# zyang1580/SML

Hardware: AMD Instinct MI355X
Metric: SML retrain-period training triples/s (MF + transfer stages), Yelp-shaped synthetic, d=32 (higher is better)
Workload: dtype f32; 1 GPU; yelp_period: users=60000 items=123000 interactions/period=75000 neg=999 d=32 multi_num=10 MF_batch=1024 TR_batch=256 val_eval=True (the reference's 40 validation evaluations per period: 31 computed on the GPU, 9 memoised because the tables did not change in between -- identical numbers); MF stage: the transfer net runs once per DISTINCT row of a batch (the reference gathers one row per occurrence:; parallelism=single GPU

## Files before the change

### include/sml_hip.h

```cpp
#ifndef SML_HIP_H
#define SML_HIP_H

#include <stdint.h>

#ifdef __cplusplus
extern "C" {
#endif

#define SML_OK 0
#define SML_EINVAL (-1)
#define SML_EHIP (-2)
#define SML_ENOMEM (-3)
#define SML_ESTATE (-4)

#define SML_LOSS_BCE 0
#define SML_LOSS_BPR 1
#define SML_LOSS_BPR_NORM 2
#define SML_LOSS_BPR_UNIT 3

typedef struct sml_ctx sml_ctx;

const char* sml_last_error(void);
int sml_version(void);

int sml_ctx_create(sml_ctx** out, int device, int d, int max_batch);
int sml_ctx_destroy(sml_ctx* ctx);
int sml_ctx_set_variant(sml_ctx* ctx, int variant);
int sml_ctx_set_grad_clip(sml_ctx* ctx, float max_norm);
int sml_ctx_set_adaptive(sml_ctx* ctx, float beta);

int64_t sml_theta_net_size(int d);
int64_t sml_theta_offset(int d, int which);
int sml_theta_pack(sml_ctx* ctx, const float* theta, void* stream);

int sml_comm_load(const char* librccl_path);
int sml_comm_unique_id(void* out128);
int sml_comm_init(sml_ctx* ctx, int world, int rank, const void* id128);
int sml_comm_destroy(sml_ctx* ctx);
int sml_comm_allreduce(sml_ctx* ctx, float* buf, int64_t n, void* stream);
int sml_comm_allgather(sml_ctx* ctx, const float* src, float* dst, int64_t n_per_rank, void* stream);

#define SML_MAX_PEERS 8
int sml_peer_region_bytes(sml_ctx* ctx, int world, int64_t rows_cap, int64_t* inbox_bytes, int64_t* flags_bytes);
int sml_peer_alloc(int device, int64_t bytes, void** ptr);
int sml_peer_free(int device, void* ptr);
int sml_peer_mem_kind(void* ptr);
int sml_peer_read(int device, const void* src, void* dst, int64_t bytes, void* stream);
int sml_peer_export(void* ptr, void* handle64);
int sml_peer_open(int device, const void* handle64, void** ptr);
int sml_peer_close(int device, void* ptr);
int sml_peer_attach(sml_ctx* ctx, int world, int rank, void* const* inbox, void* const* flags, int64_t rows_cap,
                    double timeout_s);
int sml_peer_detach(sml_ctx* ctx);
int sml_peer_status(sml_ctx* ctx, int* timeouts);
int sml_peer_allreduce_check(sml_ctx* ctx, const float* src, float* dst, int64_t n, double timeout_s, void* stream);

int sml_transfer_forward(sml_ctx* ctx, const float* theta, int net, const float* x_t,
                         const float* x_hat, float* out, int64_t n_rows, void* stream);

typedef struct {
    float* w_user;
    float* w_item;
    const float* last_user;
    const float* last_item;
    float* m_user; float* v_user;
    float* m_item; float* v_item;
    int32_t* step_user;
    int32_t* step_item;
    int64_t n_user, n_item;
} sml_mf_tables;

typedef int (*sml_mf_hook)(void* user, int64_t batch_index);
typedef struct {
    int world;
    const uint64_t* key_items;
    const uint32_t* val_items;
    float* dx_local;
    float* dx_items_all;
    sml_mf_hook hook;
    void* hook_user;
    float loss_scale;
    int64_t slot_stride;
    const int64_t* item_off;
    int64_t push_rows;
    int lists_unsorted;
} sml_mf_exchange;
// ... 33 lines not shown
    const int64_t* items_all;
    float* dx_local;
    float* dx_items_all;
    sml_mf_hook hook;
    void* hook_user;
    float loss_scale;
} sml_bare_exchange;

int sml_embed_loss_sgd_prepare(sml_ctx* ctx, const int64_t* triples, int64_t n, int batch,
                               int64_t n_user, int64_t n_item, int slot, const sml_bare_exchange* xchg, void* stream);
int64_t sml_index_lists_read(sml_ctx* ctx, int slot, int which, void* host, int64_t bytes);
int sml_embed_loss_sgd_epoch(sml_ctx* ctx, void* w_user, void* w_item, int64_t n_user,
                             int64_t n_item, int dtype_bytes, const int64_t* triples, int64_t n,
                             int batch, float lr, float lam_user, float lam_item, int loss_kind,
                             float* batch_loss, int prepared_slot, const sml_bare_exchange* xchg, void* stream);

typedef struct {
    int world, rank;
    int64_t head_rows, shard_rows;
    void* const* item_shard;
    void* w_item_head;
    const int64_t* items_all;
    float loss_scale;
} sml_bare_shard;
int sml_embed_loss_sgd_epoch_sharded(sml_ctx* ctx, void* w_user, int64_t n_user, int64_t n_item, int dtype_bytes,
                                     const int64_t* triples, int64_t n, int batch, float lr, float lam_user, float lam_item,
                                     int loss_kind, float* batch_loss, const sml_bare_shard* sh, void* stream);

int sml_embed_loss_adam_epoch(sml_ctx* ctx, const sml_mf_tables* t, const int64_t* triples, int64_t n,
                              int batch, float lr, float lam_user, float lam_item, int loss_kind,
                              int64_t* step, float* batch_loss, void* stream);

int sml_mf_forward(sml_ctx* ctx, const float* w_user, const float* w_item, const int64_t* user,
                   const int64_t* item, int64_t n, int norm, float* uemb, float* iemb, float* score,
                   void* stream);

int sml_eval_ranks(sml_ctx* ctx, const float* w_user, const float* w_item, const int64_t* rows,
                   int64_t n, int n_cols, int32_t* rank, void* stream);
int sml_eval_prepare(sml_ctx* ctx, const int64_t* rows, int64_t n, int n_cols, int64_t n_item,
                     int32_t* rows_b, int32_t* bucket_off, void* stream);
int sml_eval_ranks_blocked(sml_ctx* ctx, const float* w_user, const float* w_item, const int32_t* rows_b,
                           const int32_t* bucket_off, int64_t n, int n_cols, int32_t* rank,
                           int max_workgroups, void* stream);
int sml_eval_sliced_slices(sml_ctx* ctx, int64_t n, int n_cols, int64_t n_item);
int64_t sml_eval_sliced_entries(sml_ctx* ctx, int64_t n, int n_cols, int64_t n_item);
int64_t sml_eval_sliced_work_ints(sml_ctx* ctx, int64_t n, int n_cols, int64_t n_item);
int64_t sml_eval_sliced_scratch_bytes(sml_ctx* ctx, int64_t n, int n_cols, int64_t n_item);
int sml_eval_prepare_sliced(sml_ctx* ctx, const int64_t* rows, int64_t n, int n_cols, int64_t n_item,
                            uint32_t* entries, int32_t* seg_off, int32_t* work, void* stream);
int sml_eval_ranks_sliced(sml_ctx* ctx, const float* w_user, const float* w_item, const int64_t* rows,
                          const uint32_t* entries, const int32_t* seg_off, int64_t n, int n_cols, int64_t n_item,
                          void* scratch, int32_t* rank, int max_workgroups, void* stream);
int sml_copy_tables(int n, void* const* dst, const void* const* src, const int64_t* bytes, void* stream);

int sml_stream_create_cu_range(void** stream, int device, int cu_lo, int cu_hi);
int sml_stream_destroy(void* stream);
int sml_stream_wait_stream(void* waiter, void* signaler);
int sml_flag_set(int32_t* flag, int value, void* stream);
int sml_flag_wait(int32_t* flag, int value, double timeout_s, void* stream);
int sml_eval_metrics(sml_ctx* ctx, const int32_t* rank, int64_t n, int topk, float* out, void* stream);

int sml_full_rank(sml_ctx* ctx, const float* w_user, const float* w_item, int64_t n_item,
                  const int64_t* rows, int64_t n, int n_cols,
                  const int64_t* seen_off, const int32_t* seen_items, int32_t* rank, void* stream);
int64_t sml_topk_scratch_bytes(sml_ctx* ctx, int64_t n, int k, int64_t n_item);
int sml_topk_items(sml_ctx* ctx, const float* w_user, const float* w_item, int64_t n_item,
                   const int64_t* users, int64_t n, int k,
                   const int64_t* seen_off, const int32_t* seen_items,
                   void* scratch, int32_t* items, float* scores, void* stream);
int64_t sml_user_rank_scratch_bytes(sml_ctx* ctx, int64_t n, int64_t n_pos, int64_t n_item);
int sml_user_rank(sml_ctx* ctx, const float* w_user, const float* w_item, int64_t n_item,
                  const int64_t* users, int64_t n, const int64_t* pos_off, const int32_t* pos_items, int64_t n_pos,
                  const int64_t* seen_off, const int32_t* seen_items, void* scratch, int32_t* above, int32_t* pos,
                  void* stream);
int sml_full_rank_f16(sml_ctx* ctx, const void* w_user, const void* w_item, int64_t n_item,
                      const int64_t* rows, int64_t n, int n_cols,
                      const int64_t* seen_off, const int32_t* seen_items, int32_t* rank, void* stream);
int sml_topk_items_f16(sml_ctx* ctx, const void* w_user, const void* w_item, int64_t n_item,
                       const int64_t* users, int64_t n, int k,
                       const int64_t* seen_off, const int32_t* seen_items,
                       void* scratch, int32_t* items, float* scores, void* stream);
int sml_user_rank_f16(sml_ctx* ctx, const void* w_user, const void* w_item, int64_t n_item,
                      const int64_t* users, int64_t n, const int64_t* pos_off, const int32_t* pos_items, int64_t n_pos,
                      const int64_t* seen_off, const int32_t* seen_items, void* scratch, int32_t* above, int32_t* pos,
                      void* stream);
int sml_user_metrics(sml_ctx* ctx, const int32_t* pos, const int64_t* pos_off, int64_t n, const int32_t* ks, int n_k,
                     int32_t* hits, float* dcg, float* ap, int32_t* first, void* stream);

int sml_prof_enable(sml_ctx* ctx, int on);
int sml_debug_timeline(long long* buf);
int sml_prof_reset(sml_ctx* ctx);
int sml_prof_pair_overhead(sml_ctx* ctx, int n, void* stream, double* avg_us);
int sml_prof_classes(void);
const char* sml_prof_name(int cls);
int sml_prof_get(sml_ctx* ctx, int cls, int64_t* count, double* total_ms);

int sml_sample_negatives(sml_ctx* ctx, const int64_t* users, int64_t n, const int64_t* item_all, int64_t pop,
                         const int64_t* user_ptr, int64_t n_users, const int64_t* user_items, uint64_t seed,
                         int64_t* negs, int32_t* failed, void* stream);

int sml_device_epoch(sml_ctx* ctx, const int64_t* ui, const void* mat, int elem_bytes, int64_t row_stride, int64_t col, int64_t n,
                     uint64_t seed, int64_t* out3, void* stream);

int64_t sml_rank_weights_scratch_bytes(sml_ctx* ctx, int64_t n);
int sml_rank_weights(sml_ctx* ctx, const float* w_user, const float* w_item, const int64_t* rows, int64_t n, void* scratch,
                     float* score, int32_t* rank, int32_t* order, float* p, void* stream);
// ... 22 lines not shown
```

### sml_amd/_lib.py

```python
import ctypes
import os

import torch

_HERE = os.path.dirname(os.path.abspath(__file__))
LIB_PATH = os.path.join(_HERE, "libsml_hip.so")

c_f32p = ctypes.POINTER(ctypes.c_float)
c_i64p = ctypes.POINTER(ctypes.c_int64)
c_i32p = ctypes.POINTER(ctypes.c_int32)
c_void = ctypes.c_void_p

GRAD_HOOK = ctypes.CFUNCTYPE(ctypes.c_int, ctypes.c_void_p, ctypes.c_void_p, ctypes.c_int64, ctypes.c_int64)
MF_HOOK = ctypes.CFUNCTYPE(ctypes.c_int, ctypes.c_void_p, ctypes.c_int64)

LOSS_BCE, LOSS_BPR, LOSS_BPR_NORM, LOSS_BPR_UNIT = 0, 1, 2, 3


class MFTables(ctypes.Structure):
    _fields_ = [("w_user", c_void), ("w_item", c_void), ("last_user", c_void), ("last_item", c_void),
                ("m_user", c_void), ("v_user", c_void), ("m_item", c_void), ("v_item", c_void),
                ("step_user", c_void), ("step_item", c_void), ("n_user", ctypes.c_int64), ("n_item", ctypes.c_int64)]


class MFExchange(ctypes.Structure):
    _fields_ = [("world", ctypes.c_int), ("key_items", c_void), ("val_items", c_void), ("dx_local", c_void),
                ("dx_items_all", c_void), ("hook", MF_HOOK), ("hook_user", c_void), ("loss_scale", ctypes.c_float),
                ("slot_stride", ctypes.c_int64), ("item_off", c_void), ("push_rows", ctypes.c_int64), ("lists_unsorted", ctypes.c_int)]


class BareExchange(ctypes.Structure):
    _fields_ = [("world", ctypes.c_int), ("items_all", c_void), ("dx_local", c_void), ("dx_items_all", c_void), ("hook", MF_HOOK),
                ("hook_user", c_void), ("loss_scale", ctypes.c_float)]


class BareShard(ctypes.Structure):
    _fields_ = [("world", ctypes.c_int), ("rank", ctypes.c_int), ("head_rows", ctypes.c_int64), ("shard_rows", ctypes.c_int64),
                ("item_shard", ctypes.POINTER(c_void)), ("w_item_head", c_void), ("items_all", c_void), ("loss_scale", ctypes.c_float)]


class BatchPlan(ctypes.Structure):
    _fields_ = [("n_batches", ctypes.c_int64), ("batch_off", c_void), ("batch_off_dev", c_void), ("loss_scale", c_void)]


class TRTables(ctypes.Structure):
    _fields_ = [("last_user", c_void), ("last_item", c_void), ("hat_user", c_void), ("hat_item", c_void),
                ("n_user", ctypes.c_int64), ("n_item", ctypes.c_int64)]


SIGNATURES = {
    "sml_last_error": (ctypes.c_char_p, []),
    "sml_version": (ctypes.c_int, []),
    "sml_ctx_create": (ctypes.c_int, [ctypes.POINTER(c_void), ctypes.c_int, ctypes.c_int, ctypes.c_int]),
    "sml_ctx_set_variant": (ctypes.c_int, [c_void, ctypes.c_int]),
    "sml_ctx_set_grad_clip": (ctypes.c_int, [c_void, ctypes.c_float]),
    "sml_ctx_set_adaptive": (ctypes.c_int, [c_void, ctypes.c_float]),
    "sml_ctx_destroy": (ctypes.c_int, [c_void]),
    "sml_theta_net_size": (ctypes.c_int64, [ctypes.c_int]),
    "sml_theta_offset": (ctypes.c_int64, [ctypes.c_int, ctypes.c_int]),
    "sml_theta_pack": (ctypes.c_int, [c_void, c_void, c_void]),
    "sml_transfer_forward": (ctypes.c_int, [c_void, c_void, ctypes.c_int, c_void, c_void, c_void, ctypes.c_int64, c_void]),
    "sml_mf_stage_epoch": (ctypes.c_int, [c_void, c_void, ctypes.POINTER(MFTables), c_void, ctypes.c_int64, ctypes.c_int,
                                          ctypes.c_float, ctypes.c_float, ctypes.c_int, ctypes.POINTER(ctypes.c_int64),
                                          c_void, ctypes.POINTER(MFExchange), ctypes.POINTER(BatchPlan), c_void]),
    "sml_mf_adam_flush": (ctypes.c_int, [c_void, ctypes.POINTER(MFTables), ctypes.c_float, ctypes.c_int64, c_void]),
    "sml_tr_stage_epoch": (ctypes.c_int, [c_void, c_void, c_void, c_void, c_void, ctypes.POINTER(TRTables), c_void,
                                          ctypes.c_int64, ctypes.c_int, ctypes.c_float, ctypes.c_float, ctypes.c_int,
                                          ctypes.c_float, ctypes.POINTER(ctypes.c_int64), c_void, GRAD_HOOK, c_void,
                                          ctypes.POINTER(BatchPlan), c_void]),
    "sml_run_mf_grad": (ctypes.c_int, [c_void, c_void, c_void, c_void, c_void, c_void, ctypes.c_int, ctypes.c_int, c_void, c_void, c_void,
                                       c_void, c_void]),
    "sml_embed_loss_sgd_epoch": (ctypes.c_int, [c_void, c_void, c_void, ctypes.c_int64, ctypes.c_int64, ctypes.c_int,
                                                c_void, ctypes.c_int64, ctypes.c_int, ctypes.c_float, ctypes.c_float,
                                                ctypes.c_float, ctypes.c_int, c_void, ctypes.c_int, ctypes.POINTER(BareExchange), c_void]),
    "sml_embed_loss_sgd_epoch_sharded": (ctypes.c_int, [c_void, c_void, ctypes.c_int64, ctypes.c_int64, ctypes.c_int, c_void, ctypes.c_int64,
                                                        ctypes.c_int, ctypes.c_float, ctypes.c_float, ctypes.c_float, ctypes.c_int, c_void,
                                                        ctypes.POINTER(BareShard), c_void]),
    "sml_embed_loss_adam_epoch": (ctypes.c_int, [c_void, c_void, c_void, ctypes.c_int64, ctypes.c_int, ctypes.c_float, ctypes.c_float,
                                                 ctypes.c_float, ctypes.c_int, c_void, c_void, c_void]),
    "sml_index_lists_read": (ctypes.c_int64, [c_void, ctypes.c_int, ctypes.c_int, c_void, ctypes.c_int64]),
    "sml_embed_loss_sgd_prepare": (ctypes.c_int, [c_void, c_void, ctypes.c_int64, ctypes.c_int, ctypes.c_int64, ctypes.c_int64,
                                                  ctypes.c_int, ctypes.POINTER(BareExchange), c_void]),
    "sml_mf_forward": (ctypes.c_int, [c_void, c_void, c_void, c_void, c_void, ctypes.c_int64, ctypes.c_int, c_void,
                                      c_void, c_void, c_void]),
    "sml_eval_ranks": (ctypes.c_int, [c_void, c_void, c_void, c_void, ctypes.c_int64, ctypes.c_int, c_void, c_void]),
    "sml_eval_metrics": (ctypes.c_int, [c_void, c_void, ctypes.c_int64, ctypes.c_int, c_void, c_void]),
    "sml_eval_prepare": (ctypes.c_int, [c_void, c_void, ctypes.c_int64, ctypes.c_int, ctypes.c_int64, c_void, c_void, c_void]),
    "sml_eval_ranks_blocked": (ctypes.c_int, [c_void, c_void, c_void, c_void, c_void, ctypes.c_int64, ctypes.c_int, c_void, ctypes.c_int,
                                              c_void]),
    "sml_eval_sliced_slices": (ctypes.c_int, [c_void, ctypes.c_int64, ctypes.c_int, ctypes.c_int64]),
    "sml_eval_sliced_entries": (ctypes.c_int64, [c_void, ctypes.c_int64, ctypes.c_int, ctypes.c_int64]),
    "sml_eval_sliced_work_ints": (ctypes.c_int64, [c_void, ctypes.c_int64, ctypes.c_int, ctypes.c_int64]),
    "sml_eval_sliced_scratch_bytes": (ctypes.c_int64, [c_void, ctypes.c_int64, ctypes.c_int, ctypes.c_int64]),
    "sml_eval_prepare_sliced": (ctypes.c_int, [c_void, c_void, ctypes.c_int64, ctypes.c_int, ctypes.c_int64, c_void, c_void, c_void, c_void]),
    "sml_eval_ranks_sliced": (ctypes.c_int, [c_void, c_void, c_void, c_void, c_void, c_void, ctypes.c_int64, ctypes.c_int, ctypes.c_int64,
                                             c_void, c_void, ctypes.c_int, c_void]),
    "sml_full_rank": (ctypes.c_int, [c_void, c_void, c_void, ctypes.c_int64, c_void, ctypes.c_int64, ctypes.c_int, c_void, c_void,
                                     c_void, c_void]),
    "sml_topk_scratch_bytes": (ctypes.c_int64, [c_void, ctypes.c_int64, ctypes.c_int, ctypes.c_int64]),
    "sml_topk_items": (ctypes.c_int, [c_void, c_void, c_void, ctypes.c_int64, c_void, ctypes.c_int64, ctypes.c_int, c_void, c_void,
                                      c_void, c_void, c_void, c_void]),
    "sml_user_rank_scratch_bytes": (ctypes.c_int64, [c_void, ctypes.c_int64, ctypes.c_int64, ctypes.c_int64]),
    "sml_user_rank": (ctypes.c_int, [c_void, c_void, c_void, ctypes.c_int64, c_void, ctypes.c_int64, c_void, c_void, ctypes.c_int64,
                                     c_void, c_void, c_void, c_void, c_void, c_void]),
    "sml_full_rank_f16": (ctypes.c_int, [c_void, c_void, c_void, ctypes.c_int64, c_void, ctypes.c_int64, ctypes.c_int, c_void, c_void,
                                         c_void, c_void]),
    "sml_topk_items_f16": (ctypes.c_int, [c_void, c_void, c_void, ctypes.c_int64, c_void, ctypes.c_int64, ctypes.c_int, c_void, c_void,
                                          c_void, c_void, c_void, c_void]),
    "sml_user_rank_f16": (ctypes.c_int, [c_void, c_void, c_void, ctypes.c_int64, c_void, ctypes.c_int64, c_void, c_void, ctypes.c_int64,
                                         c_void, c_void, c_void, c_void, c_void, c_void]),
    "sml_user_metrics": (ctypes.c_int, [c_void, c_void, c_void, ctypes.c_int64, c_void, ctypes.c_int, c_void, c_void, c_void, c_void,
                                        c_void]),
    "sml_stream_create_cu_range": (ctypes.c_int, [ctypes.POINTER(c_void), ctypes.c_int, ctypes.c_int, ctypes.c_int]),
    "sml_stream_destroy": (ctypes.c_int, [c_void]),
    "sml_stream_wait_stream": (ctypes.c_int, [c_void, c_void]),
    "sml_copy_tables": (ctypes.c_int, [ctypes.c_int, ctypes.POINTER(c_void), ctypes.POINTER(c_void), ctypes.POINTER(ctypes.c_int64), c_void]),
    "sml_flag_set": (ctypes.c_int, [c_void, ctypes.c_int, c_void]),
    "sml_flag_wait": (ctypes.c_int, [c_void, ctypes.c_int, ctypes.c_double, c_void]),
    "sml_comm_load": (ctypes.c_int, [ctypes.c_char_p]),
    "sml_comm_unique_id": (ctypes.c_int, [c_void]),
    "sml_comm_init": (ctypes.c_int, [c_void, ctypes.c_int, ctypes.c_int, c_void]),
    "sml_comm_destroy": (ctypes.c_int, [c_void]),
    "sml_comm_allreduce": (ctypes.c_int, [c_void, c_void, ctypes.c_int64, c_void]),
    "sml_comm_allgather": (ctypes.c_int, [c_void, c_void, c_void, ctypes.c_int64, c_void]),
    "sml_peer_region_bytes": (ctypes.c_int, [c_void, ctypes.c_int, ctypes.c_int64, ctypes.POINTER(ctypes.c_int64), ctypes.POINTER(ctypes.c_int64)]),
    "sml_peer_alloc": (ctypes.c_int, [ctypes.c_int, ctypes.c_int64, ctypes.POINTER(c_void)]),
    "sml_peer_free": (ctypes.c_int, [ctypes.c_int, c_void]),
    "sml_device_epoch": (ctypes.c_int, [c_void, c_void, c_void, ctypes.c_int, ctypes.c_int64, ctypes.c_int64, ctypes.c_int64,
                                        ctypes.c_uint64, c_void, c_void]),
    "sml_peer_mem_kind": (ctypes.c_int, [c_void]),
    "sml_peer_read": (ctypes.c_int, [ctypes.c_int, c_void, c_void, ctypes.c_int64, c_void]),
    "sml_peer_export": (ctypes.c_int, [c_void, c_void]),
    "sml_peer_open": (ctypes.c_int, [ctypes.c_int, c_void, ctypes.POINTER(c_void)]),
    "sml_peer_close": (ctypes.c_int, [ctypes.c_int, c_void]),
    "sml_peer_attach": (ctypes.c_int, [c_void, ctypes.c_int, ctypes.c_int, ctypes.POINTER(c_void), ctypes.POINTER(c_void), ctypes.c_int64,
                                       ctypes.c_double]),
    "sml_peer_detach": (ctypes.c_int, [c_void]),
    "sml_peer_status": (ctypes.c_int, [c_void, ctypes.POINTER(ctypes.c_int)]),
    "sml_peer_allreduce_check": (ctypes.c_int, [c_void, c_void, c_void, ctypes.c_int64, ctypes.c_double, c_void]),
    "sml_prof_enable": (ctypes.c_int, [c_void, ctypes.c_int]),
    "sml_debug_timeline": (ctypes.c_int, [c_void]),
    "sml_prof_reset": (ctypes.c_int, [c_void]),
    "sml_prof_pair_overhead": (ctypes.c_int, [c_void, ctypes.c_int, c_void, ctypes.POINTER(ctypes.c_double)]),
    "sml_prof_classes": (ctypes.c_int, []),
    "sml_prof_name": (ctypes.c_char_p, [ctypes.c_int]),
    "sml_prof_get": (ctypes.c_int, [c_void, ctypes.c_int, ctypes.POINTER(ctypes.c_int64), ctypes.POINTER(ctypes.c_double)]),
    "sml_sample_negatives": (ctypes.c_int, [c_void, c_void, ctypes.c_int64, c_void, ctypes.c_int64, c_void, ctypes.c_int64, c_void,
                                            ctypes.c_uint64, c_void, c_void, c_void]),
    "sml_host_resolve_negatives": (ctypes.c_int, [c_void, ctypes.c_int64, c_void, ctypes.c_int64, c_void, ctypes.c_int64,
                                                  ctypes.c_int64, c_void, ctypes.POINTER(ctypes.c_int64),
                                                  ctypes.POINTER(ctypes.c_int64)]),
    "sml_host_gather_pairs": (ctypes.c_int, [c_void, ctypes.c_int64, c_void, ctypes.c_int64, c_void]),
    "sml_host_gather_column": (ctypes.c_int, [c_void, ctypes.c_int64, ctypes.c_int64, ctypes.c_int, ctypes.c_int64, c_void, ctypes.c_int64,
                               c_void, ctypes.c_int]),
    "sml_host_resolve_negatives_csr": (ctypes.c_int, [c_void, ctypes.c_int64, c_void, ctypes.c_int64, c_void, ctypes.c_int64, c_void,
                                                      c_void, c_void, c_void]),
    "sml_rank_weights_scratch_bytes": (ctypes.c_int64, [c_void, ctypes.c_int64]),
    "sml_rank_weights": (ctypes.c_int, [c_void, c_void, c_void, c_void, ctypes.c_int64, c_void, c_void, c_void, c_void, c_void,
                                        c_void]),
    "sml_weighted_epoch": (ctypes.c_int, [c_void, c_void, ctypes.c_int64, c_void, c_void, ctypes.c_int64, c_void, ctypes.c_int64,
                                          c_void, ctypes.c_int64, ctypes.c_uint64, c_void, c_void, c_void]),
    "sml_selftest": (ctypes.c_int, [ctypes.c_int]),
}

_lib = None


def load():
    global _lib
# ... 36 lines not shown
```

### sml_amd/csrc/capi.hip

```cpp
#include <hip/hip_runtime.h>
#ifdef SML_TEST_PREP_REFERENCE
#include <hipcub/hipcub.hpp>
#endif
#include <rccl/rccl.h>
#include <dlfcn.h>

#include <cmath>
#include <cstdio>
#include <cstdlib>
#include <cstring>
#include <map>
#include <mutex>
#include <string>
#include <vector>

#include "../../include/sml_hip.h"
#include "sml_kernels.h"

namespace {

thread_local std::string g_err;

int fail(int code, const char* what, const char* detail) {
    g_err = std::string(what) + ": " + (detail ? detail : "");
// ... 121 lines not shown
    Buf<uint32_t> slot_info;
    int64_t slot_stride = 0;
    int64_t dense_stride = 0;
    Buf<SmlRun> dense_rec; Buf<int> dense_n; Buf<SmlTileHdr> tile_hdr; Buf<uint2> tile_ent, tile_spill; Buf<int> spill_cnt;
    bool dense = false; int tiles_cap = 0;
    Buf<int> off_u, off_i, n_sel;
    Buf<uint32_t> hist_u, hist_i, bko_u, bko_i, bkc_u, bkc_i, large, medium;
    Buf<SmlRun> stage_u, stage_i;
    Buf<int> cnt_u, cnt_i;
    Buf<int> rank_viol;
    bool rank_probed = false;
    bool by_hand = false;
    Buf<char> cub_tmp;
    int key_bytes = 8, row_bits_u = 32, row_bits_i = 32;
    int* viol_host = nullptr;
    hipEvent_t viol_ready = nullptr;
    int* max_len_host = nullptr;
    int* lists_host = nullptr;
    int64_t lists_host_nb = 0, lists_nb = 0;
    hipEvent_t ready = nullptr;
    int64_t n = -1; int batch = 0; const void* triples = nullptr; int world = 1;
    void release() {
        key_u.release(); key_u2.release(); key_i.release(); key_i2.release();
        val_u.release(); val_u2.release(); val_i.release(); val_i2.release();
        rec_u.release(); rec_i.release(); runs_u.release(); runs_i.release();
        hist_u.release(); hist_i.release(); bko_u.release(); bko_i.release(); bkc_u.release(); bkc_i.release(); large.release(); medium.release();
        cnt_u.release(); cnt_i.release(); stage_u.release(); stage_i.release(); rank_viol.release();
        dense_rec.release(); dense_n.release(); tile_hdr.release(); tile_ent.release(); tile_spill.release(); spill_cnt.release();
        uniq.release(); slot_info.release(); heads_u.release(); heads_i.release(); hot_list.release(); hot_count.release(); off_u.release(); off_i.release(); n_sel.release();
        cub_tmp.release();
        if (max_len_host) { g_graveyard.park_host(max_len_host); max_len_host = nullptr; }
        if (viol_host) { g_graveyard.park_host(viol_host); viol_host = nullptr; }
        if (viol_ready) { (void)hipEventDestroy(viol_ready); viol_ready = nullptr; }
        if (lists_host) { g_graveyard.park_host(lists_host); lists_host = nullptr; lists_host_nb = 0; }
        if (ready) { (void)hipEventDestroy(ready); ready = nullptr; }
    }
};

struct SchedRetired { SmlSched* dev; SmlSched* host; hipEvent_t done; };

struct sml_ctx {
    int device = 0, d = 32, max_batch = 0;
    int variant = 0;
    bool side = false;
    float clip_max_norm = 0.0f;
    float adaptive_beta = 0.0f;
    Buf<float> clip_sumsq;
    IndexSet ix[2];
    Buf<float> out, dout, dx, xin, z1, a1, a2, dz1, mrep, vrep;
    Buf<float> pk, grad, convg, loss_part;
    Buf<float> pkx;
    Buf<float> cstate;
    int pk_set = 0;
    Buf<int> arrive;
    Buf<int> run_arrive;
    Buf<SmlSched> sched;
    int sched_len = 0;
    float sched_lr = -1.0f;
    std::vector<SchedRetired> sched_retired;
    hipEvent_t sched_ready = nullptr;
    hipStream_t sched_stream = nullptr;
    Buf<int32_t> dummy;
    Buf<SmlRun> rec_x;
    Buf<int32_t> xoff;
    ncclComm_t comm = nullptr;
    int comm_world = 1, comm_rank = 0;
    struct Peer {
        int world = 0, rank = 0;
        char* inbox[SML_MAX_PEERS] = {nullptr};
        unsigned long long* flags[SML_MAX_PEERS] = {nullptr};
        int64_t theta_slot = 0;
        int64_t rows_cap = 0;
        int64_t tick[3] = {0, 0, 0};
        unsigned long long expect[3][2] = {{0, 0}, {0, 0}, {0, 0}};
        bool done_pending = false;
        SmlPeerPoll done_poll;
        long long timeout = 0;
        int* err = nullptr;
    } peer;
    Buf<int> hot_first;
    Buf<float> hot_part;
    Buf<float> head_part;
    Buf<void*> ptr_tab;
    Prof prof;

    void release_all() {
        prof.release();
        out.release(); dout.release(); dx.release(); xin.release(); z1.release(); a1.release(); a2.release(); dz1.release();
        mrep.release(); vrep.release();
        pk.release(); pkx.release(); grad.release(); convg.release(); loss_part.release(); arrive.release(); run_arrive.release(); cstate.release();
        ix[0].release(); ix[1].release();
        sched.release(); dummy.release(); rec_x.release(); xoff.release();
        for (auto& r : sched_retired) { g_graveyard.park(r.dev); g_graveyard.park_host(r.host); (void)hipEventDestroy(r.done); }
        sched_retired.clear();
        if (sched_ready) { (void)hipEventDestroy(sched_ready); sched_ready = nullptr; }
        hot_first.release(); hot_part.release(); head_part.release(); ptr_tab.release();
        if (peer.err) { g_graveyard.park(peer.err); peer.err = nullptr; }
    }
};

namespace {

SmlSched sched_entry(double lr, int64_t k) {
    SmlSched s;
    if (k <= 0) { s.step_size = 0.f; s.bc2_sqrt = 1.f; return s; }
    const double bc1 = 1.0 - std::pow((double)0.9, (double)k);
// ... 70 lines not shown
    c->sched.p = dnew; c->sched.cap = (size_t)len;
    c->sched_len = (int)len;
    c->sched_lr = lr;
    if (!c->sched_ready) HIPCHK(hipEventCreateWithFlags(&c->sched_ready, hipEventDisableTiming));
    HIPCHK(hipEventRecord(c->sched_ready, st));
    c->sched_stream = st;
    return SML_OK;
}

int tiles_of(int rows) { return (rows + SML_R - 1) / SML_R; }
int wg_tiles(int rows, int mt) { const int r = SML_TM * mt; return (rows + r - 1) / r; }

int env_int(const char* name, int dflt) { const char* v = getenv(name); return v && *v ? atoi(v) : dflt; }
int replay_len(const sml_ctx* c, int64_t to) {
    const int on = env_int("SML_REPLAY_CLOSED", 1), k0 = env_int("SML_REPLAY_K0", SML_RP_K0);
    return (on != 0 && to >= k0 && to - SML_RP_N >= 1 && to + 1 < c->sched_len) ? c->sched_len : 0;
}
int fwd_split(int row_tiles) {
    const int forced = env_int("SML_FWD_NS", 0);
    if (forced == 1 || forced == 2 || forced == 4) return forced;
    return row_tiles <= 64 ? 4 : row_tiles <= 128 ? 2 : 1;
}
int bwd_split(int row_tiles) {
    const int forced = env_int("SML_BWD_SPLIT", -1);
    if (forced == 0 || forced == 1) return forced;
    return row_tiles <= 128 ? 1 : 0;
}

int ensure_transfer_ws(sml_ctx* c, int B, bool tr_stage, hipStream_t st) {
    const size_t slots = (size_t)SML_R * (tiles_of(B) + tiles_of(2 * B)), d = (size_t)c->d;
    HIPCHK(c->out.ensure(slots * d * SML_FWD_NS));
    HIPCHK(c->dout.ensure(slots * d));
    HIPCHK(c->xin.ensure(slots * 3 * d));
    HIPCHK(c->z1.ensure(slots * SML_HID));
    if (tr_stage) {
        HIPCHK(c->a1.ensure(slots * SML_C2 * d));
        HIPCHK(c->a2.ensure(slots * SML_HID));
        HIPCHK(c->dz1.ensure(slots * SML_HID));
        HIPCHK(c->convg.ensure((slots / SML_TM + 4) * (d / 16) * SML_CG));
        HIPCHK(c->grad.ensure((size_t)2 * sml_net_size(c->d)));
        if (!c->arrive.p) { HIPCHK(c->arrive.ensure(4)); HIPCHK(hipMemsetAsync(c->arrive.p, 0, 4 * sizeof(int), st)); }
    } else {
        HIPCHK(c->dx.ensure(slots * d));
        HIPCHK(c->mrep.ensure(slots * d)); HIPCHK(c->vrep.ensure(slots * d));
    }
    return SML_OK;
}

int ensure_pk(sml_ctx* c) {
    HIPCHK(c->pk.ensure((size_t)4 * sml_pk_size(c->d)));
    return SML_OK;
}
float* pk_cur(const sml_ctx* c) { return c->pk.p + (size_t)c->pk_set * 2 * sml_pk_size(c->d); }
float* pk_other(const sml_ctx* c) { return c->pk.p + (size_t)(1 - c->pk_set) * 2 * sml_pk_size(c->d); }

int ceil_log2(int64_t x) { int b = 0; while (((int64_t)1 << b) < x) ++b; return b; }

int64_t peer_theta_slot(int d) { return ((int64_t)2 * sml_net_size(d) + 63) / 64 * 64; }
float* peer_theta_at(const sml_ctx* c, int owner, int parity, int src) {
    return reinterpret_cast<float*>(c->peer.inbox[owner]) + ((int64_t)parity * c->peer.world + src) * c->peer.theta_slot;
}
float* peer_rows_at(const sml_ctx* c, int owner, int parity, int src) {
    float* base = reinterpret_cast<float*>(c->peer.inbox[owner]) + (int64_t)2 * c->peer.world * c->peer.theta_slot;
    return base + ((int64_t)parity * c->peer.world + src) * c->peer.rows_cap * c->d;
}
unsigned long long* peer_flag_at(const sml_ctx* c, int owner, int kind, int parity, int src) {
    return c->peer.flags[owner] + ((int64_t)kind * 2 + parity) * c->peer.world + src;
}
void peer_step(sml_ctx* c, int kind, int incr, SmlPeerPush* push, SmlPeerPoll* poll) {
    const int W = c->peer.world, me = c->peer.rank;
    const int parity = (int)(c->peer.tick[kind] & 1);
    c->peer.tick[kind] += 1;
    c->peer.expect[kind][parity] += (unsigned long long)incr;
    memset(push, 0, sizeof(*push)); memset(poll, 0, sizeof(*poll));
    push->world = W;
    for (int q = 0; q < W; ++q) {
        push->dst[q] = kind == 0 ? peer_theta_at(c, q, parity, me) : kind == 1 ? peer_rows_at(c, q, parity, me) : nullptr;
        push->flag[q] = peer_flag_at(c, q, kind, parity, me);
    }
    poll->world = W;
    poll->slot0 = kind == 0 ? peer_theta_at(c, me, parity, 0) : kind == 1 ? peer_rows_at(c, me, parity, 0) : nullptr;
    poll->slot_stride = kind == 0 ? c->peer.theta_slot : c->peer.rows_cap * c->d;
    poll->flag0 = peer_flag_at(c, me, kind, parity, 0);
    poll->expect = c->peer.expect[kind][parity];
    poll->timeout = c->peer.timeout;
    poll->err = c->peer.err;
}

static bool prep_by_hand() {
    const char* e = getenv("SML_PREP");
    return !(e && !strcmp(e, "cub"));
}

int sort_order_check(IndexSet* c) {
    if (c->viol_host && c->viol_ready && hipEventQuery(c->viol_ready) == hipSuccess && *c->viol_host != 0) {
        char msg[320];
        const int w1 = c->viol_host[1], w2 = c->viol_host[2];
        snprintf(msg, sizeof(msg), "a sorted bucket left out of (row, value) order (%d entries; first: occurrence source %d, table %d, batch %d, %s mode, "
                                   "position %d of a %d-entry bucket): the stable ranking failed on this device (SML_PREP_RANK=ballot selects the ballot ranking)",
                 c->viol_host[0], (w1 >> 28) & 7, (w1 >> 27) & 1, w1 & 0x3ffffff, (w1 >> 26) & 1 ? "records" : "compact / dense", w2 >> 12, w2 & 0xfff);
        return fail(SML_ESTATE, "index preparation", msg);
    }
    return SML_OK;
}
int prep_epoch(IndexSet* c, const int64_t* tri, int64_t n, int batch, int pad_tiles, int64_t n_user, int64_t n_item,
               bool dups, hipStream_t st, const sml_batch_plan* plan, int mode = 0, const sml_bare_exchange* bx = nullptr,
// ... 151 lines not shown
}

int sort_epoch_sharded(IndexSet* A, IndexSet* Bset, const int64_t* tri, int64_t n, int batch, int64_t n_user, const sml_bare_shard* sh,
                       int64_t rows_cap, hipStream_t st) {
    if (prep_by_hand()) {
        int rc = prep_epoch(A, tri, n, batch, 0, n_user, 0, true, st, nullptr, 2, nullptr, sh, rows_cap);
        if (!rc && sh->head_rows > 0) rc = prep_epoch(Bset, tri, n, batch, 0, n_user, 0, true, st, nullptr, 3, nullptr, sh, rows_cap);
        return rc;
    }
#ifdef SML_TEST_PREP_REFERENCE
    return sort_epoch_sharded_reference(A, Bset, tri, n, batch, n_user, sh, rows_cap, st);
#else
    return fail(SML_ESTATE, "index preparation", "SML_PREP=cub: the library-sort reference is test infrastructure (tests/build_reference.py), not in this library");
#endif
}

}

extern "C" {

const char* sml_last_error(void) { return g_err.c_str(); }
int sml_version(void) { return 1; }

int64_t sml_theta_net_size(int d) { return d_ok(d) ? sml_net_size(d) : -1; }
int64_t sml_theta_offset(int d, int which) {
    if (!d_ok(d)) return -1;
    switch (which) {
        case 0: return SML_OFF_C1W;
        case 1: return SML_OFF_C1B;
        case 2: return SML_OFF_C2W;
        case 3: return SML_OFF_C2B;
        case 4: return SML_OFF_F1W;
        case 5: return sml_off_f1b(d);
        case 6: return sml_off_f2w(d);
        case 7: return sml_off_f2b(d);
        default: return -1;
    }
}

int sml_ctx_create(sml_ctx** out, int device, int d, int max_batch) {
    if (!out || !d_ok(d) || max_batch <= 0) return fail(SML_EINVAL, "sml_ctx_create", "d must be 32/64/128, max_batch > 0");
    int n_dev = 0;
    HIPCHK(hipGetDeviceCount(&n_dev));
    if (device < 0 || device >= n_dev) return fail(SML_EINVAL, "sml_ctx_create", "no such device");
    sml_ctx* c = new (std::nothrow) sml_ctx();
    if (!c) return fail(SML_ENOMEM, "sml_ctx_create", "host allocation");
    c->device = device; c->d = d; c->max_batch = max_batch;
    *out = c;
    return SML_OK;
}

int sml_ctx_set_variant(sml_ctx* ctx, int variant) {
    if (!ctx || variant < 0 || variant > 3) return fail(SML_EINVAL, "sml_ctx_set_variant", "variant must be 0 or 1 (+ 2: an evaluation-stream context)");
    ctx->variant = variant & 1; ctx->side = (variant & 2) != 0;
    return SML_OK;
}

int sml_ctx_set_adaptive(sml_ctx* ctx, float beta) {
    if (!ctx || !(beta >= 0.0f)) return fail(SML_EINVAL, "sml_ctx_set_adaptive", "beta must be >= 0 (0: off)");
    ctx->adaptive_beta = beta;
    return SML_OK;
}

int sml_ctx_set_grad_clip(sml_ctx* ctx, float max_norm) {
    if (!ctx || !(max_norm >= 0.0f)) return fail(SML_EINVAL, "sml_ctx_set_grad_clip", "max_norm must be >= 0 (0: off)");
    ctx->clip_max_norm = max_norm;
    return SML_OK;
}

static void ctx_destroy_now(sml_ctx* ctx) {
    (void)sml_comm_destroy(ctx);
    { DevGuard g(ctx->device); ctx->release_all(); }
    delete ctx;
}
int sml_ctx_destroy(sml_ctx* ctx) {
    if (!ctx) return SML_OK;
    (void)sml_peer_detach(ctx);
    if (g_graveyard.defer(ctx)) return SML_OK;
    ctx_destroy_now(ctx);
    for (sml_ctx* z : g_graveyard.take_zombies()) ctx_destroy_now(z);
    g_graveyard.reap();
    return SML_OK;
}

int sml_theta_pack(sml_ctx* ctx, const float* theta, void* stream) {
    if (!ctx || !theta) return fail(SML_EINVAL, "sml_theta_pack", "null argument");
    DevGuard g(ctx->device);
    int rc = ensure_pk(ctx); if (rc) return rc;
    hipStream_t st = (hipStream_t)stream;
    ctx->prof.begin(PC_PACK, st); HIPCHK(sml_launch_theta_pack(ctx->d, theta, pk_cur(ctx), st)); ctx->prof.end(st);
    return SML_OK;
}

int sml_transfer_forward(sml_ctx* ctx, const float* theta, int net, const float* x_t, const float* x_hat, float* out,
                         int64_t n_rows, void* stream) {
    if (n_rows == 0) return SML_OK;
    if (!ctx || !theta || !x_t || !x_hat || !out || (net != 0 && net != 1) || n_rows < 0 || n_rows > 0x7fffffff)
        return fail(SML_EINVAL, "sml_transfer_forward", "bad argument");
    DevGuard g(ctx->device);
    hipStream_t st = (hipStream_t)stream;
    int rc = ensure_pk(ctx); if (rc) return rc;
    const size_t bx3 = n_rows > 8192 && env_int("SML_FWD_BX3", 1) != 0 && env_int("SML_FWD_MT", 0) == 0 ? sml_bx3_bytes(ctx->d) : 0;
    if (bx3) {
        HIPCHK(ctx->pkx.ensure(bx3 / sizeof(float) + 4));
        ctx->prof.begin(PC_PACK, st); HIPCHK(sml_launch_theta_pack_bx3(ctx->d, theta, ctx->pkx.p, st)); ctx->prof.end(st);
        SmlFwdArgs a;
        memset(&a, 0, sizeof(a));
        SmlSeg& s = a.seg[0];
        s.theta = theta + (int64_t)net * sml_net_size(ctx->d);
        s.xt_tab = x_t; s.xh_tab = x_hat; s.n_rows = (int)n_rows; s.out = out;
        a.k2 = ctx->variant == 1; a.unit_rows = (ctx->variant == 1 && net == 0);
        a.tiles0 = wg_tiles((int)n_rows, 2);
        const char* pkx_net = reinterpret_cast<const char*>(ctx->pkx.p) + (size_t)net * (bx3 / 2);
        ctx->prof.begin(ctx->side ? PC_FWD_SIDE : PC_FWD, st);
        HIPCHK(sml_launch_fwd_bx3(ctx->d, a, pkx_net, a.tiles0, st, ctx->side));
        ctx->prof.end(st);
        return SML_OK;
    }
    ctx->prof.begin(PC_PACK, st); HIPCHK(sml_launch_theta_pack(ctx->d, theta, pk_cur(ctx), st)); ctx->prof.end(st);
    SmlFwdArgs a;
    memset(&a, 0, sizeof(a));
    SmlSeg& s = a.seg[0];
    s.theta = theta + (int64_t)net * sml_net_size(ctx->d);
    s.pk = pk_cur(ctx) + (int64_t)net * sml_pk_size(ctx->d);
    s.xt_tab = x_t; s.xh_tab = x_hat; s.n_rows = (int)n_rows; s.out = out;
    a.k2 = ctx->variant == 1; a.unit_rows = (ctx->variant == 1 && net == 0);
    const int mt_env = env_int("SML_FWD_MT", 0);
    const int mt = n_rows > 8192 ? ((mt_env == 3 && ctx->d == 32) ? 3 : 2) : 1;
    a.tiles0 = wg_tiles((int)n_rows, mt);
    a.seg[1] = s; a.seg[1].n_rows = 0;
    const bool side = ctx->side && mt == 2 && (ctx->d == 32 || ctx->d == 64);
    ctx->prof.begin(side ? PC_FWD_SIDE : PC_FWD, st); HIPCHK(sml_launch_fwd(ctx->d, mt, 1, a, a.tiles0, st, side)); ctx->prof.end(st);
    return SML_OK;
}

int sml_mf_stage_epoch(sml_ctx* ctx, const float* theta, const sml_mf_tables* t, const int64_t* triples, int64_t n,
                       int batch, float lr, float l2, int loss_kind, int64_t* step, float* batch_loss,
                       const sml_mf_exchange* xchg, const sml_batch_plan* plan, void* stream) {
    if (!ctx || !theta || !t || !step || !batch_loss || batch <= 0 || (plan ? n < 0 : n <= 0) || (n > 0 && !triples))
        return fail(SML_EINVAL, "sml_mf_stage_epoch", "bad argument");
    if (plan && (plan->n_batches <= 0 || !plan->batch_off || !plan->batch_off_dev || plan->batch_off[0] != 0 || plan->batch_off[plan->n_batches] != n))
        return fail(SML_EINVAL, "sml_mf_stage_epoch", "batch plan does not cover the triples");
    if (batch > ctx->max_batch) return fail(SML_EINVAL, "sml_mf_stage_epoch", "batch exceeds ctx max_batch");
    if (n > 0x3fffffff) return fail(SML_EINVAL, "sml_mf_stage_epoch", "epoch too long");
    if (loss_kind < 0 || loss_kind > 3 || (ctx->variant == 1 ? (loss_kind != SML_LOSS_BPR_UNIT && loss_kind != SML_LOSS_BPR_NORM) : loss_kind == SML_LOSS_BPR_UNIT))
        return fail(SML_EINVAL, "sml_mf_stage_epoch", "loss_kind (variant 1 takes SML_LOSS_BPR_UNIT, or SML_LOSS_BPR_NORM for run_MF(norm=True); SML_LOSS_BPR_UNIT goes with variant 1 only)");
    if (xchg && (xchg->world < 1 || !xchg->key_items || !xchg->val_items || !xchg->dx_local || !xchg->dx_items_all))
        return fail(SML_EINVAL, "sml_mf_stage_epoch", "incomplete exchange descriptor");
    const bool mf_peers = xchg && !xchg->hook && ctx->peer.world > 0;
    if (mf_peers && ctx->peer.world != xchg->world) return fail(SML_ESTATE, "sml_mf_stage_epoch", "peer mappings were attached for another world size");
    if (mf_peers && (xchg->slot_stride > 0 ? xchg->slot_stride : (int64_t)2 * batch) != ctx->peer.rows_cap)
        return fail(SML_EINVAL, "sml_mf_stage_epoch", "on the peer path the exchange's slot_stride must equal the rows_cap the inboxes were attached with");
    if (mf_peers && (xchg->push_rows < 0 || xchg->push_rows > ctx->peer.rows_cap || (xchg->push_rows > 0 && xchg->push_rows < 2 * (int64_t)batch)))
        return fail(SML_EINVAL, "sml_mf_stage_epoch", "push_rows must cover a batch's 2*batch item rows and fit a slot");
    if (xchg && !xchg->hook && !mf_peers && (!ctx->comm || ctx->comm_world != xchg->world))
        return fail(SML_ESTATE, "sml_mf_stage_epoch", "exchange without a hook needs sml_peer_attach or sml_comm_init with the same world size");
    DevGuard g(ctx->device);
    hipStream_t st = (hipStream_t)stream;
    const int d = ctx->d;
    const int64_t nb = plan ? plan->n_batches : (n + batch - 1) / batch;
    if (plan) for (int64_t b = 0; b < nb; ++b)
        if (plan->batch_off[b + 1] < plan->batch_off[b] || plan->batch_off[b + 1] - plan->batch_off[b] > batch)
            return fail(SML_EINVAL, "sml_mf_stage_epoch", "a planned batch is longer than `batch`");
    int rc;
    if ((rc = ensure_pk(ctx))) return rc;
    if ((rc = ensure_transfer_ws(ctx, batch, false, st))) return rc;
    if ((rc = ensure_sched(ctx, lr, *step + nb + 1, st))) return rc;
    const int lstride = (wg_tiles(batch, 1) + wg_tiles(2 * batch, 1)) * (d / 16);
    const int64_t out_pstride = (int64_t)SML_R * (tiles_of(batch) + tiles_of(2 * batch)) * d;
    const int fns = fwd_split(wg_tiles(batch, 1) + wg_tiles(2 * batch, 1)), bsplit = bwd_split(wg_tiles(batch, 1) + wg_tiles(2 * batch, 1));
    HIPCHK(ctx->loss_part.ensure((size_t)nb * lstride));
    ctx->prof.begin(PC_PACK, st); HIPCHK(sml_launch_theta_pack(d, theta, pk_cur(ctx), st)); ctx->prof.end(st);
    const bool mf_bx3 = fns == 1 && sml_bx3_bytes(d) > 0 && env_int("SML_MF_BX3", 1) != 0;
    if (mf_bx3) {
        HIPCHK(ctx->pkx.ensure(sml_bx3_bytes(d) / sizeof(float) + 4));
        ctx->prof.begin(PC_PACK, st); HIPCHK(sml_launch_theta_pack_bx3(d, theta, ctx->pkx.p, st)); ctx->prof.end(st);
    }
    const bool can_fuse = !xchg && !bsplit && d <= 64 && ctx->adaptive_beta <= 0.0f && env_int("SML_MF_FUSED_UPDATE", 1) != 0;
    const bool want_dense = can_fuse && fns == 1 && env_int("SML_MF_DISTINCT", 1) != 0;
    ctx->prof.begin(PC_SORT, st); rc = sort_epoch(&ctx->ix[0], triples, n, batch, 1, t->n_user, t->n_item, false, st, plan, nullptr, want_dense);
    const int64_t x_total = !xchg ? 0 : xchg->item_off ? xchg->item_off[nb] : (int64_t)xchg->world * 2 * n;
    const int64_t x_stride = !xchg ? 0 : xchg->slot_stride > 0 ? xchg->slot_stride : (int64_t)2 * batch;
    const bool x_by_hand = xchg && xchg->lists_unsorted != 0;
    if (!rc && xchg && x_total > 0 && x_by_hand) {
        int64_t x_seg = (int64_t)xchg->world * 2 * batch;
        sml_batch_plan px;
        memset(&px, 0, sizeof(px));
        if (xchg->item_off) {
            std::vector<int32_t> off32((size_t)nb + 1);
            x_seg = 1;
            for (int64_t b = 0; b <= nb; ++b) {
                off32[(size_t)b] = (int32_t)xchg->item_off[b];
                if (b && xchg->item_off[b] - xchg->item_off[b - 1] > x_seg) x_seg = xchg->item_off[b] - xchg->item_off[b - 1];
            }
            HIPCHK(ctx->xoff.ensure((size_t)nb + 1));
            HIPCHK(hipMemcpyAsync(ctx->xoff.p, off32.data(), ((size_t)nb + 1) * sizeof(int32_t), hipMemcpyHostToDevice, st));
            px.n_batches = nb; px.batch_off_dev = ctx->xoff.p;
        }
        if (x_seg > 0x3fffffff) return fail(SML_EINVAL, "sml_mf_stage_epoch", "a batch's job-wide item list is too long");
        rc = prep_epoch(&ctx->ix[1], reinterpret_cast<const int64_t*>(xchg->key_items), x_total, (int)x_seg, 0, 1, t->n_item, false, st,
                        xchg->item_off ? &px : nullptr, 4, nullptr, nullptr, (int64_t)xchg->world * x_stride, false, xchg->val_items);
    } else if (!rc && xchg && x_total > 0) {
        HIPCHK(ctx->rec_x.ensure((size_t)x_total));
        HIPCHK(sml_launch_mark_runs(8, xchg->key_items, xchg->val_items, x_total, 32, ctx->rec_x.p, nullptr, nullptr, 0, 0, st));
    }
    ctx->prof.end(st); if (rc) return rc;
    HIPCHK(hipMemsetAsync(ctx->loss_part.p, 0, (size_t)nb * lstride * sizeof(float), st));
    const int64_t ns = sml_net_size(d), ps = sml_pk_size(d);
    float* dx_buf = xchg ? xchg->dx_local : ctx->dx.p;
    const bool dense = want_dense && ctx->ix[0].by_hand && ctx->ix[0].dense;
    const bool fused = can_fuse && !dense && ctx->ix[0].by_hand && ctx->ix[0].slot_stride > 0;
    if (env_int("SML_TRACE", 0))
        fprintf(stderr, "[sml] mf_stage_epoch: form=%s batches=%lld batch=%d d=%d\n", dense ? "distinct-rows" : fused ? "per-occurrence+fused-update" : "per-occurrence+run-update",
                (long long)nb, batch, d);
    if (fused) {
        HIPCHK(ctx->run_arrive.ensure((size_t)3 * ctx->max_batch + 8));
        HIPCHK(hipMemsetAsync(ctx->run_arrive.p, 0, ((size_t)3 * ctx->max_batch + 8) * sizeof(int), st));
    }
    for (int64_t b = 0; b < nb; ++b) {
        const int64_t off0 = plan ? plan->batch_off[b] : b * batch;
        const int B = plan ? (int)(plan->batch_off[b + 1] - off0) : (int)((n - off0) < batch ? (n - off0) : batch);
        const int64_t* tri = triples + off0 * 3;
        const int cur = (int)(*step + 1 + b);
        SmlFwdArgs f;
        memset(&f, 0, sizeof(f));
        for (int s = 0; s < 2; ++s) {
            SmlSeg& sg = f.seg[s];
            sg.theta = theta + s * ns; sg.pk = pk_cur(ctx) + s * ps;
            sg.xt_tab = s ? t->last_item : t->last_user;
            sg.xh_tab = s ? t->w_item : t->w_user;
            sg.m_tab = s ? t->m_item : t->m_user; sg.v_tab = s ? t->v_item : t->v_user;
            sg.last_tab = s ? t->step_item : t->step_user;
            sg.tri = tri; sg.B = B; sg.is_item = s; sg.n_rows = s ? 2 * B : B;
            const int64_t slot0 = s ? (int64_t)SML_R * tiles_of(B) : 0;
            sg.out = ctx->out.p + slot0 * d; sg.z1 = ctx->z1.p + slot0 * SML_HID; sg.xin = ctx->xin.p + slot0 * 3 * d;
            sg.a1 = nullptr;
            sg.mrep = ctx->mrep.p + slot0 * d; sg.vrep = ctx->vrep.p + slot0 * d;
            if (dense) {
                sg.n_rows = SML_TM * wg_tiles(sg.n_rows, 1);
                sg.drec = ctx->ix[0].dense_rec.p + b * ctx->ix[0].dense_stride + slot0;
                sg.hdr = ctx->ix[0].tile_hdr.p + b * ctx->ix[0].tiles_cap + (s ? wg_tiles(B, 1) : 0);
            }
        }
        f.tiles0 = wg_tiles(B, 1); f.cur_step = cur; f.sched = ctx->sched.p; f.out_pstride = out_pstride; f.k2 = ctx->variant == 1;
        f.sched_len = replay_len(ctx, cur - 1);
        const int tiles = f.tiles0 + wg_tiles(2 * B, 1);
        f.tiles_total = tiles;
        ctx->prof.begin(PC_FWD, st);
        if (mf_bx3) HIPCHK(sml_launch_mf_fwd_bx3(d, f, ctx->pkx.p, tiles, st));
        else HIPCHK(sml_launch_fwd(d, 1, fns, f, tiles, st));
        ctx->prof.end(st);
        SmlBwdArgs w;
        memset(&w, 0, sizeof(w));
        for (int s = 0; s < 2; ++s) {
            SmlBwdSeg& sg = w.seg[s];
            const int64_t slot0 = s ? (int64_t)SML_R * tiles_of(B) : 0;
            sg.theta = theta + s * ns; sg.pk = pk_cur(ctx) + s * ps;
            sg.dout = ctx->dout.p + slot0 * d; sg.is_item = s; sg.z1 = ctx->z1.p + slot0 * SML_HID; sg.xin = ctx->xin.p + slot0 * 3 * d;
            sg.dx = dx_buf + slot0 * d; sg.dz1 = nullptr; sg.n_rows = s ? 2 * B : B;
        }
// ... 27 lines not shown
        int bwd_grid = tiles;
        if (push_fused) {
            bwd_grid = wg_tiles(batch, 1) + wg_tiles(2 * batch, 1);
            if (bwd_grid < tiles) bwd_grid = tiles;
            peer_step(ctx, 1, bwd_grid, &push_f, &poll_f);
            w.push = push_f; w.tiles_live = tiles;
        }
        ctx->prof.begin(PC_BWD, st); HIPCHK(sml_launch_bwd(d, bsplit, w, bwd_grid, st)); ctx->prof.end(st);
        if (fused || dense) continue;
        if (ctx->adaptive_beta > 0.0f) {
            ctx->prof.begin(PC_MISC, st);
            HIPCHK(sml_launch_adaptive_users(d, ctx->xin.p, dx_buf, B, ctx->adaptive_beta, w.loss_part, st));
            ctx->prof.end(st);
        }
        SmlRunArgs u;
        memset(&u, 0, sizeof(u));
        u.run_u = ctx->ix[0].rec_u.p + off0; u.n_u = B; u.val_u = ctx->ix[0].val_u2.p;
        u.run_i = ctx->ix[0].rec_i.p + 2 * off0; u.n_i = 2 * B; u.val_i = ctx->ix[0].val_i2.p;
        u.dx = dx_buf; u.dx_i = dx_buf; u.w_user = t->w_user; u.w_item = t->w_item;
        if (xchg) {
            const float* gathered = xchg->dx_items_all;
            if (xchg->hook) {
                if (xchg->hook(xchg->hook_user, b) != 0) return fail(SML_ESTATE, "sml_mf_stage_epoch", "exchange hook failed");
            } else if (mf_peers) {
                const int64_t ioff = (int64_t)SML_R * tiles_of(B);
                SmlPeerPush push; SmlPeerPoll poll;
                const int64_t x_push = xchg->push_rows > 0 ? xchg->push_rows : x_stride;
                ctx->prof.begin(PC_MISC, st);
                if (push_fused) poll = poll_f;
                else {
                    peer_step(ctx, 1, sml_peer_push_blocks(x_push * d), &push, &poll);
                    HIPCHK(sml_launch_peer_push(dx_buf + ioff * d, x_push * d, push, st));
                }
                if (env_int("SML_PEER_WAIT_LAUNCH", 0)) HIPCHK(sml_launch_peer_wait(poll, st));
                else u.wait = poll;
                ctx->prof.end(st);
                gathered = poll.slot0;
            } else {
                const int64_t ioff = (int64_t)SML_R * tiles_of(B);
                NCCLCHK(g_rccl.AllGather(dx_buf + ioff * d, xchg->dx_items_all, (size_t)x_stride * d, ncclFloat, ctx->comm, st));
            }
            const int64_t x0 = xchg->item_off ? xchg->item_off[b] : (int64_t)xchg->world * 2 * b * batch;
            u.run_i = (x_by_hand ? ctx->ix[1].rec_i.p : ctx->rec_x.p) + x0;
            u.val_i = x_by_hand ? ctx->ix[1].val_i2.p : xchg->val_items;
            u.n_i = xchg->item_off ? (int)(xchg->item_off[b + 1] - x0) : xchg->world * 2 * B;
            u.dx_i = gathered;
        }
        u.m_user = t->m_user; u.v_user = t->v_user; u.m_item = t->m_item; u.v_item = t->v_item;
        u.last_user = t->step_user; u.last_item = t->step_item; u.sched = ctx->sched.p; u.cur_step = cur; u.lr = lr; u.sched_len = replay_len(ctx, cur - 1);
        u.rep_x = ctx->xin.p; u.rep_m = ctx->mrep.p; u.rep_v = ctx->vrep.p; u.rep_u = 1; u.rep_i = xchg ? 0 : 1;
        u.rep_x_stride = 3 * d; u.rep_x_off = d;
        ctx->prof.begin(PC_SEG_ADAM, st); HIPCHK(sml_launch_run_adam(d, u, (int64_t)u.n_u + u.n_i, st)); ctx->prof.end(st);
    }
    ctx->prof.begin(PC_MISC, st); HIPCHK(sml_launch_loss_finalize(ctx->loss_part.p, (int)nb, lstride, nullptr, batch_loss, st)); ctx->prof.end(st);
    *step += nb;
    return SML_OK;
}

int sml_mf_adam_flush(sml_ctx* ctx, const sml_mf_tables* t, float lr, int64_t step, void* stream) {
    if (!ctx || !t || step < 0) return fail(SML_EINVAL, "sml_mf_adam_flush", "bad argument");
    if (step == 0) return SML_OK;
    DevGuard g(ctx->device);
    hipStream_t st = (hipStream_t)stream;
    int rc;
    if ((rc = ensure_sched(ctx, lr, step + 1, st))) return rc;
    ctx->prof.begin(PC_FLUSH, st); HIPCHK(sml_launch_adam_flush(ctx->d, t->w_user, t->m_user, t->v_user, t->step_user, t->n_user, ctx->sched.p, (int)step, replay_len(ctx, step), st));
    HIPCHK(sml_launch_adam_flush(ctx->d, t->w_item, t->m_item, t->v_item, t->step_item, t->n_item, ctx->sched.p, (int)step, replay_len(ctx, step), st)); ctx->prof.end(st);
    return SML_OK;
}

int sml_tr_stage_epoch(sml_ctx* ctx, float* theta, float* adam_m, float* adam_v, float* theta_grad,
                       const sml_tr_tables* t, const int64_t* triples, int64_t n, int batch, float lr,
                       float weight_decay, int loss_kind, float loss_scale, int64_t* step, float* batch_loss,
                       sml_grad_hook grad_hook, void* hook_user, const sml_batch_plan* plan, void* stream) {
    if (!ctx || !theta || !adam_m || !adam_v || !t || !step || !batch_loss || batch <= 0 || (plan ? n < 0 : n <= 0) || (n > 0 && !triples))
        return fail(SML_EINVAL, "sml_tr_stage_epoch", "bad argument");
    if (plan && (plan->n_batches <= 0 || !plan->batch_off || plan->batch_off[0] != 0 || plan->batch_off[plan->n_batches] != n))
        return fail(SML_EINVAL, "sml_tr_stage_epoch", "batch plan does not cover the triples");
    if (batch > ctx->max_batch) return fail(SML_EINVAL, "sml_tr_stage_epoch", "batch exceeds ctx max_batch");
    if (loss_kind < 0 || loss_kind > 3 || (ctx->variant == 1 ? (loss_kind != SML_LOSS_BPR_UNIT && loss_kind != SML_LOSS_BPR_NORM) : loss_kind == SML_LOSS_BPR_UNIT))
        return fail(SML_EINVAL, "sml_tr_stage_epoch", "loss_kind (variant 1 takes SML_LOSS_BPR_UNIT, or SML_LOSS_BPR_NORM for run_MF(norm=True); SML_LOSS_BPR_UNIT goes with variant 1 only)");
    DevGuard g(ctx->device);
    hipStream_t st = (hipStream_t)stream;
    const int d = ctx->d;
    const int64_t nb = plan ? plan->n_batches : (n + batch - 1) / batch;
    if (plan) for (int64_t b = 0; b < nb; ++b)
        if (plan->batch_off[b + 1] < plan->batch_off[b] || plan->batch_off[b + 1] - plan->batch_off[b] > batch)
            return fail(SML_EINVAL, "sml_tr_stage_epoch", "a planned batch is longer than `batch`");
    int rc;
    if ((rc = ensure_pk(ctx))) return rc;
    if ((rc = ensure_transfer_ws(ctx, batch, true, st))) return rc;
    const bool clip = ctx->clip_max_norm > 0.0f;
    if (clip) HIPCHK(ctx->clip_sumsq.ensure(4));
    float* grad = theta_grad ? theta_grad : ctx->grad.p;
    const int fns = fwd_split(wg_tiles(batch, 1) + wg_tiles(2 * batch, 1)), bsplit = bwd_split(wg_tiles(batch, 1) + wg_tiles(2 * batch, 1));
    const int cs = bsplit ? d / 16 : 1;
    const bool v2 = env_int("SML_TR_V2", 1) != 0;
    const int lstride = (wg_tiles(batch, 1) + wg_tiles(2 * batch, 1)) * (d / 16 > 4 ? d / 16 : 4);
    const int64_t out_pstride = (int64_t)SML_R * (tiles_of(batch) + tiles_of(2 * batch)) * d;
    HIPCHK(ctx->loss_part.ensure((size_t)nb * lstride));
    ctx->prof.begin(PC_PACK, st); HIPCHK(sml_launch_theta_pack(d, theta, pk_cur(ctx), st)); ctx->prof.end(st);
    HIPCHK(hipMemsetAsync(ctx->loss_part.p, 0, (size_t)nb * lstride * sizeof(float), st));
    HIPCHK(hipMemsetAsync(grad, 0, (size_t)2 * sml_net_size(d) * sizeof(float), st));
    const int64_t ns = sml_net_size(d), ps = sml_pk_size(d);
    const bool fused_path = !clip && !grad_hook && ctx->peer.world <= 0 && ctx->comm == nullptr;
    const bool defer = v2 && fns == 4 && fused_path && !plan && nb > 1 && env_int("SML_TR_DEFER", 1) != 0;
    const bool a2_recompute = v2 && env_int("SML_TR_A2_RECOMPUTE", 1) != 0;
    int prev_split = 0, prev_total = 0;
    if (defer) {
        HIPCHK(ctx->cstate.ensure((size_t)2 * 2 * 3 * SML_CG));
        HIPCHK(sml_launch_conv_state_init(d, theta, adam_m, adam_v, ctx->cstate.p, st));
    }
    for (int64_t b = 0; b < nb; ++b) {
        const int64_t off0 = plan ? plan->batch_off[b] : b * batch;
        const int B = plan ? (int)(plan->batch_off[b + 1] - off0) : (int)((n - off0) < batch ? (n - off0) : batch);
        const int64_t* tri = triples + off0 * 3;
        SmlFwdArgs f;
        memset(&f, 0, sizeof(f));
        if (defer) {
            const SmlSched scp = sched_entry((double)lr, *step + b);
            f.cg_part = b > 0 ? ctx->convg.p : nullptr; f.cg_split = prev_split; f.cg_total = prev_total;
            f.cs_in = ctx->cstate.p + (size_t)(b & 1) * 2 * 3 * SML_CG; f.cs_out = ctx->cstate.p + (size_t)((b + 1) & 1) * 2 * 3 * SML_CG;
            f.cs_theta = theta; f.cs_m = adam_m; f.cs_v = adam_v;
            f.cs_wd = weight_decay; f.cs_step_size = scp.step_size; f.cs_bc2_sqrt = scp.bc2_sqrt;
        }
        for (int s = 0; s < 2; ++s) {
            SmlSeg& sg = f.seg[s];
            sg.theta = theta + s * ns; sg.pk = pk_cur(ctx) + s * ps;
            sg.xt_tab = s ? t->last_item : t->last_user;
            sg.xh_tab = s ? t->hat_item : t->hat_user;
            sg.tri = tri; sg.B = B; sg.is_item = s; sg.n_rows = s ? 2 * B : B;
            const int64_t slot0 = s ? (int64_t)SML_R * tiles_of(B) : 0;
            sg.out = ctx->out.p + slot0 * d; sg.z1 = ctx->z1.p + slot0 * SML_HID; sg.xin = ctx->xin.p + slot0 * 3 * d;
            sg.a1 = ctx->a1.p + slot0 * SML_C2 * d; sg.a2 = a2_recompute ? nullptr : ctx->a2.p + slot0 * SML_HID;
        }
        f.tiles0 = wg_tiles(B, 1); f.cur_step = 0; f.sched = nullptr; f.out_pstride = out_pstride; f.k2 = ctx->variant == 1;
        const int tiles = f.tiles0 + wg_tiles(2 * B, 1);
        f.tiles_total = tiles;
        ctx->prof.begin(PC_FWD, st); HIPCHK(sml_launch_fwd(d, 1, fns, f, tiles, st)); ctx->prof.end(st);
        SmlBwdArgs w;
        memset(&w, 0, sizeof(w));
        SmlWgArgs wg;
        memset(&wg, 0, sizeof(wg));
        for (int s = 0; s < 2; ++s) {
            SmlBwdSeg& sg = w.seg[s];
            const int64_t slot0 = s ? (int64_t)SML_R * tiles_of(B) : 0;
            sg.theta = theta + s * ns; sg.pk = pk_cur(ctx) + s * ps;
            sg.dout = ctx->dout.p + slot0 * d; sg.is_item = s; sg.z1 = ctx->z1.p + slot0 * SML_HID; sg.xin = ctx->xin.p + slot0 * 3 * d;
            sg.dx = nullptr; sg.dz1 = ctx->dz1.p + slot0 * SML_HID; sg.n_rows = s ? 2 * B : B;
            SmlWgSeg& q = wg.seg[s];
            q.dz1 = sg.dz1; q.a1 = ctx->a1.p + slot0 * SML_C2 * d; q.dout = sg.dout; q.a2 = a2_recompute ? sg.z1 : ctx->a2.p + slot0 * SML_HID;
            const bool fused_only = !clip && !grad_hook && (ctx->comm == nullptr || ctx->peer.world > 0) && theta_grad == nullptr;
            q.grad = fused_only ? nullptr : grad + s * ns; q.n_rows = sg.n_rows;
            q.theta_net = sg.theta; q.pk_net = sg.pk; q.xin = sg.xin;
        }
        w.tiles0 = f.tiles0; w.l2 = 0.0f; w.convg_part = ctx->convg.p;
        w.out_all = ctx->out.p; w.B = B; w.ioff = SML_R * tiles_of(B); w.kind = loss_kind;
        w.scale = (plan && plan->loss_scale) ? plan->loss_scale[b] : loss_scale; w.loss_part = ctx->loss_part.p + b * lstride;
// ... 2 lines not shown
        if (v2) HIPCHK(sml_launch_tr_bwd_head(d, w, tiles, st)); else HIPCHK(sml_launch_bwd(d, bsplit, w, tiles, st));
        ctx->prof.end(st);
        const SmlSched sc = sched_entry((double)lr, *step + 1 + b);
        const int wcs = v2 ? 1 : cs;
        auto launch_wgrad = [&](const SmlWgArgs& g) { return v2 ? sml_launch_tr_wgrad2(d, g, st) : sml_launch_wgrad(d, g, st); };
        wg.convg_part = ctx->convg.p; wg.tiles0 = f.tiles0 * wcs; wg.tiles_total = tiles * wcs;
        wg.n_tail = tiles * (d / 16) > 0 ? tiles * (d / 16) : 1; wg.convg_out = ctx->convg.p; wg.arrive = ctx->arrive.p;
        wg.defer_conv = (defer && b + 1 < nb) ? 1 : 0; wg.gelu_b = a2_recompute ? 1 : 0;
        prev_split = f.tiles0 * (d / 16); prev_total = tiles * (d / 16);
        const bool peers = !grad_hook && ctx->peer.world > 0;
        const bool native = !grad_hook && !peers && ctx->comm != nullptr;
        if (peers) {
            SmlThetaAdamArgs ad;
            memset(&ad, 0, sizeof(ad));
            peer_step(ctx, 0, v2 ? sml_wgrad2_pushers(d) : sml_wgrad_grid(d), &wg.peer, &ad.peer);
            ctx->prof.begin(PC_WGRAD, st); HIPCHK(launch_wgrad(wg)); ctx->prof.end(st);
            ad.theta = theta; ad.m = adam_m; ad.v = adam_v; ad.grad = grad; ad.pk = pk_cur(ctx);
            ad.weight_decay = weight_decay; ad.step_size = sc.step_size; ad.bc2_sqrt = sc.bc2_sqrt;
            static const bool poll_in_adam = env_int("SML_PEER_POLL_IN_ADAM", 1) != 0;
            ctx->prof.begin(PC_THETA_ADAM, st);
            if (clip) {
                HIPCHK(sml_launch_peer_sum(grad, 2 * ns, ad.peer, st, (int)ns));
                HIPCHK(sml_launch_grad_sumsq(grad, 2 * ns, ctx->clip_sumsq.p, st));
                ad.peer.world = 0;
                ad.clip_sumsq = ctx->clip_sumsq.p; ad.clip_max_norm = ctx->clip_max_norm;
            } else if (!poll_in_adam) { HIPCHK(sml_launch_peer_wait(ad.peer, st)); ad.peer.waited = 1; }
            HIPCHK(sml_launch_theta_adam(d, ad, st));
            ctx->prof.end(st);
        } else if (!grad_hook && !native && !clip) {
            wg.theta = theta; wg.m = adam_m; wg.v = adam_v; wg.pk = v2 ? pk_other(ctx) : pk_cur(ctx);
            wg.weight_decay = weight_decay; wg.step_size = sc.step_size; wg.bc2_sqrt = sc.bc2_sqrt;
            ctx->prof.begin(PC_WGRAD, st); HIPCHK(launch_wgrad(wg)); ctx->prof.end(st);
            if (v2) ctx->pk_set ^= 1;
        } else {
            ctx->prof.begin(PC_WGRAD, st); HIPCHK(launch_wgrad(wg)); ctx->prof.end(st);
            SmlThetaAdamArgs ad;
            memset(&ad, 0, sizeof(ad));
            ad.theta = theta; ad.m = adam_m; ad.v = adam_v; ad.grad = grad; ad.pk = pk_cur(ctx);
            ad.weight_decay = weight_decay; ad.step_size = sc.step_size; ad.bc2_sqrt = sc.bc2_sqrt;
            if (native) {
                NCCLCHK(g_rccl.AllReduce(grad, grad, (size_t)(2 * ns), ncclFloat, ncclSum, ctx->comm, st));
            } else if (grad_hook) {
                const int hr = grad_hook(hook_user, grad, 2 * ns, b);
                if (hr != 0) return fail(SML_ESTATE, "sml_tr_stage_epoch", "grad_hook failed");
            }
            ctx->prof.begin(PC_THETA_ADAM, st);
            if (clip) {
                HIPCHK(sml_launch_grad_sumsq(grad, 2 * ns, ctx->clip_sumsq.p, st));
                ad.clip_sumsq = ctx->clip_sumsq.p; ad.clip_max_norm = ctx->clip_max_norm;
            }
            HIPCHK(sml_launch_theta_adam(d, ad, st)); ctx->prof.end(st);
        }
    }
    ctx->prof.begin(PC_MISC, st); HIPCHK(sml_launch_loss_finalize(ctx->loss_part.p, (int)nb, lstride, nullptr, batch_loss, st)); ctx->prof.end(st);
    *step += nb;
    return SML_OK;
}

int sml_run_mf_grad(sml_ctx* ctx, const float* theta, const float* user_last, const float* user_hat, const float* item_last,
                    const float* item_hat, int B, int loss_kind, float* loss, float* d_user_hat, float* d_item_hat,
                    float* theta_grad, void* stream) {
    if (!ctx || !theta || !user_last || !user_hat || !item_last || !item_hat || !loss || B <= 0)
        return fail(SML_EINVAL, "sml_run_mf_grad", "bad argument");
    if (B > ctx->max_batch) return fail(SML_EINVAL, "sml_run_mf_grad", "batch exceeds ctx max_batch");
    if (loss_kind < 0 || loss_kind > 3 || (ctx->variant == 1 ? (loss_kind != SML_LOSS_BPR_UNIT && loss_kind != SML_LOSS_BPR_NORM) : loss_kind == SML_LOSS_BPR_UNIT))
        return fail(SML_EINVAL, "sml_run_mf_grad", "loss_kind (variant 1 takes SML_LOSS_BPR_UNIT, or SML_LOSS_BPR_NORM for run_MF(norm=True); SML_LOSS_BPR_UNIT goes with variant 1 only)");
    DevGuard g(ctx->device);
    hipStream_t st = (hipStream_t)stream;
    const int d = ctx->d;
    int rc;
    if ((rc = ensure_pk(ctx))) return rc;
    if ((rc = ensure_transfer_ws(ctx, B, true, st))) return rc;
    if ((rc = ensure_transfer_ws(ctx, B, false, st))) return rc;
    const int64_t ns = sml_net_size(d), ps = sml_pk_size(d);
    const int tiles0 = wg_tiles(B, 1), tiles = tiles0 + wg_tiles(2 * B, 1);
    const int fns = fwd_split(tiles);
    const int lstride = tiles * (d / 16 > 4 ? d / 16 : 4);
    const int64_t out_pstride = (int64_t)SML_R * (tiles_of(B) + tiles_of(2 * B)) * d;
    HIPCHK(ctx->loss_part.ensure((size_t)2 * lstride));
    HIPCHK(hipMemsetAsync(ctx->loss_part.p, 0, (size_t)2 * lstride * sizeof(float), st));
    HIPCHK(sml_launch_theta_pack(d, theta, pk_cur(ctx), st));
    SmlFwdArgs f;
    memset(&f, 0, sizeof(f));
    SmlBwdArgs w;
    memset(&w, 0, sizeof(w));
    SmlWgArgs wg;
    memset(&wg, 0, sizeof(wg));
    float* grad = theta_grad ? theta_grad : ctx->grad.p;
    for (int s = 0; s < 2; ++s) {
        const int64_t slot0 = s ? (int64_t)SML_R * tiles_of(B) : 0;
        SmlSeg& sg = f.seg[s];
        sg.theta = theta + s * ns; sg.pk = pk_cur(ctx) + s * ps;
        sg.xt_tab = s ? item_last : user_last; sg.xh_tab = s ? item_hat : user_hat;
        sg.tri = nullptr; sg.B = B; sg.is_item = s; sg.n_rows = s ? 2 * B : B;
        sg.out = ctx->out.p + slot0 * d; sg.z1 = ctx->z1.p + slot0 * SML_HID; sg.xin = ctx->xin.p + slot0 * 3 * d;
        sg.a1 = ctx->a1.p + slot0 * SML_C2 * d; sg.a2 = ctx->a2.p + slot0 * SML_HID;
        SmlBwdSeg& bg = w.seg[s];
        bg.theta = sg.theta; bg.pk = sg.pk; bg.dout = ctx->dout.p + slot0 * d; bg.is_item = s; bg.z1 = sg.z1; bg.xin = sg.xin;
        bg.dx = ctx->dx.p + slot0 * d; bg.dz1 = ctx->dz1.p + slot0 * SML_HID; bg.n_rows = sg.n_rows;
        SmlWgSeg& q = wg.seg[s];
        q.dz1 = bg.dz1; q.a1 = sg.a1; q.dout = bg.dout; q.a2 = sg.a2; q.grad = grad + s * ns; q.n_rows = sg.n_rows;
        q.theta_net = sg.theta; q.pk_net = sg.pk; q.xin = sg.xin;
    }
    f.tiles0 = tiles0; f.out_pstride = out_pstride; f.k2 = ctx->variant == 1; f.tiles_total = tiles;
    HIPCHK(sml_launch_fwd(d, 1, fns, f, tiles, st));
    w.tiles0 = tiles0; w.l2 = 0.0f; w.out_all = ctx->out.p; w.B = B; w.ioff = SML_R * tiles_of(B); w.kind = loss_kind; w.scale = 1.0f;
    w.out_np = fns; w.out_pstride = out_pstride; w.tiles_total = tiles;
    if (d_user_hat || d_item_hat || !theta_grad) {
        w.convg_part = nullptr; w.loss_part = ctx->loss_part.p;
        SmlBwdArgs wx = w;
        wx.seg[0].dz1 = nullptr; wx.seg[1].dz1 = nullptr;
        HIPCHK(sml_launch_bwd(d, bwd_split(tiles), wx, tiles, st));
        if (d_user_hat) HIPCHK(hipMemcpyAsync(d_user_hat, ctx->dx.p, (size_t)B * d * sizeof(float), hipMemcpyDeviceToDevice, st));
        if (d_item_hat) HIPCHK(hipMemcpyAsync(d_item_hat, ctx->dx.p + (size_t)SML_R * tiles_of(B) * d, (size_t)2 * B * d * sizeof(float),
                                              hipMemcpyDeviceToDevice, st));
        HIPCHK(sml_launch_loss_finalize(ctx->loss_part.p, 1, lstride, nullptr, loss, st));
    }
    if (theta_grad) {
        w.convg_part = ctx->convg.p; w.loss_part = ctx->loss_part.p + lstride;
        w.seg[0].dx = nullptr; w.seg[1].dx = nullptr;
        HIPCHK(sml_launch_tr_bwd_head(d, w, tiles, st));
        wg.convg_part = ctx->convg.p; wg.tiles0 = tiles0; wg.tiles_total = tiles;
        wg.n_tail = tiles * (d / 16); wg.convg_out = ctx->convg.p; wg.arrive = ctx->arrive.p;
        HIPCHK(hipMemsetAsync(grad, 0, (size_t)2 * ns * sizeof(float), st));
        HIPCHK(sml_launch_tr_wgrad2(d, wg, st));
        if (!(d_user_hat || d_item_hat)) HIPCHK(sml_launch_loss_finalize(ctx->loss_part.p + lstride, 1, lstride, nullptr, loss, st));
    }
    return SML_OK;
}

int sml_embed_loss_sgd_prepare(sml_ctx* ctx, const int64_t* triples, int64_t n, int batch, int64_t n_user,
                               int64_t n_item, int slot, const sml_bare_exchange* xchg, void* stream) {
    if (!ctx || !triples || n <= 0 || batch <= 0 || (slot != 0 && slot != 1))
        return fail(SML_EINVAL, "sml_embed_loss_sgd_prepare", "bad argument");
// ... 19 lines not shown
        case 4: case 5: {
            if (!X->by_hand) return 0;
            std::vector<int> raw((size_t)nb * SML_PREP_CNT_STRIDE), cnt((size_t)nb);
            HIPCHK(hipMemcpy(raw.data(), which == 4 ? X->cnt_u.p : X->cnt_i.p, raw.size() * sizeof(int), hipMemcpyDeviceToHost));
            for (int64_t b = 0; b < nb; ++b) cnt[(size_t)b] = raw[(size_t)b * SML_PREP_CNT_STRIDE];
            const int64_t nbytes = nb * 4 < bytes ? nb * 4 : bytes;
            memcpy(host, cnt.data(), (size_t)nbytes);
            return nbytes;
        }
        case 6: src = X->val_u2.p; have = X->n * 4; break;
        case 7: src = X->val_i2.p; have = 2 * X->n * 4; break;
        case 8: src = X->uniq.p; have = 3 * nb * X->batch; break;
        case 9: src = X->hot_list.p; have = X->hot_cap ? nb * X->hot_cap * 12 : 0; break;
        case 10: src = X->hot_count.p; have = X->hot_cap ? nb * 4 : 0; break;
        case 11: HIPCHK(hipMemcpy(two, X->n_sel.p + 2, 4, hipMemcpyDeviceToHost)); memcpy(host, two, bytes < 8 ? bytes : 8); return bytes < 8 ? bytes : 8;
        default: return fail(SML_EINVAL, "sml_index_lists_read", "which");
    }
    const int64_t nbytes = have < bytes ? have : bytes;
    if (nbytes > 0 && src) HIPCHK(hipMemcpy(host, src, (size_t)nbytes, hipMemcpyDeviceToHost));
    return src ? nbytes : 0;
}

int sml_embed_loss_sgd_epoch(sml_ctx* ctx, void* w_user, void* w_item, int64_t n_user, int64_t n_item, int dtype_bytes,
                             const int64_t* triples, int64_t n, int batch, float lr, float lam_user, float lam_item,
                             int loss_kind, float* batch_loss, int prepared_slot, const sml_bare_exchange* xchg, void* stream) {
    if (!ctx || !w_user || !w_item || !triples || !batch_loss || n <= 0 || batch <= 0 || n_user <= 0 || n_item <= 0)
        return fail(SML_EINVAL, "sml_embed_loss_sgd_epoch", "bad argument");
    if (xchg && (xchg->world < 1 || !xchg->items_all || !xchg->dx_items_all || !xchg->dx_local))
        return fail(SML_EINVAL, "sml_embed_loss_sgd_epoch", "incomplete exchange descriptor");
    if (xchg && !xchg->hook && (!ctx->comm || ctx->comm_world != xchg->world))
        return fail(SML_ESTATE, "sml_embed_loss_sgd_epoch", "exchange without a hook needs sml_comm_init with the same world size");
    if (dtype_bytes != 4 && dtype_bytes != 2) return fail(SML_EINVAL, "sml_embed_loss_sgd_epoch", "dtype_bytes must be 4 or 2");
    if (loss_kind != SML_LOSS_BCE && loss_kind != SML_LOSS_BPR) return fail(SML_EINVAL, "sml_embed_loss_sgd_epoch", "loss_kind");
    if (batch > ctx->max_batch) return fail(SML_EINVAL, "sml_embed_loss_sgd_epoch", "batch exceeds ctx max_batch");
    if (n > 0x3fffffff) return fail(SML_EINVAL, "sml_embed_loss_sgd_epoch", "epoch too long");
    if (prepared_slot < -1 || prepared_slot > 1) return fail(SML_EINVAL, "sml_embed_loss_sgd_epoch", "prepared_slot");
    DevGuard g(ctx->device);
    hipStream_t st = (hipStream_t)stream;
    const int d = ctx->d;
    const int64_t nb = (n + batch - 1) / batch;
    int rc;
    HIPCHK(ctx->dx.ensure((size_t)3 * batch * d));
    float* const dxb = xchg ? xchg->dx_local : ctx->dx.p;
    const int lpr = d * dtype_bytes / 16;
    const int lstride = (int)(((int64_t)batch * lpr + 255) / 256);
    HIPCHK(ctx->loss_part.ensure((size_t)nb * lstride));
    IndexSet* X = &ctx->ix[prepared_slot < 0 ? 0 : prepared_slot];
    if (prepared_slot < 0) {
        ctx->prof.begin(PC_SORT, st); rc = sort_epoch(X, triples, n, batch, 0, n_user, n_item, true, st, nullptr, xchg); ctx->prof.end(st);
        if (rc) return rc;
    } else if (X->n != n || X->batch != batch || X->triples != triples || X->world != (xchg ? xchg->world : 1)) {
        return fail(SML_ESTATE, "sml_embed_loss_sgd_epoch", "index set was prepared for other triples");
    }
    HIPCHK(hipMemsetAsync(ctx->loss_part.p, 0, (size_t)nb * lstride * sizeof(float), st));
    const int hot_cap = X->hot_cap;
    const bool known = hipEventQuery(X->ready) == hipSuccess;
    if ((rc = sort_order_check(X))) return rc;
    const bool hot = hot_cap > 0 && (!known || *X->max_len_host > SML_HOT);
    const int world = xchg ? xchg->world : 1;
    const int hot_chunks = (int)(((int64_t)batch + (int64_t)world * 2 * batch) / SML_HOT_CHUNK) + hot_cap;
    if (hot) {
        HIPCHK(ctx->hot_first.ensure((size_t)hot_cap));
        HIPCHK(ctx->hot_part.ensure((size_t)hot_chunks * d));
    }
    for (int64_t b = 0; b < nb; ++b) {
        const int B = (int)((n - b * batch) < batch ? (n - b * batch) : batch);
        SmlBareArgs a;
        memset(&a, 0, sizeof(a));
        a.w_user = w_user; a.w_item = w_item; a.tri = triples + b * batch * 3; a.B = B; a.dx = dxb;
        a.loss_part = ctx->loss_part.p + b * lstride; a.kind = loss_kind; a.lam_user = lam_user; a.lam_item = lam_item;
        a.uniq = X->uniq.p + (size_t)3 * b * batch; a.lr = lr; a.scale = xchg ? xchg->loss_scale : 1.0f;
        ctx->prof.begin(PC_BARE_GRAD, st); HIPCHK(sml_launch_bare_grad(d, dtype_bytes, a, nullptr, st)); ctx->prof.end(st);
        if (xchg) {
            if (xchg->hook) {
                if (xchg->hook(xchg->hook_user, b) != 0) return fail(SML_ESTATE, "sml_embed_loss_sgd_epoch", "exchange hook failed");
            } else {
                NCCLCHK(g_rccl.AllGather(dxb + (size_t)B * d, xchg->dx_items_all, (size_t)2 * batch * d, ncclFloat, ctx->comm, st));
            }
        }
        SmlRunArgs u;
        memset(&u, 0, sizeof(u));
        u.run_u = X->runs_u.p; u.run_i = X->runs_i.p; u.off_u = X->off_u.p; u.off_i = X->off_i.p; u.batch_index = (int)b;
        u.val_u = X->val_u2.p; u.val_i = X->val_i2.p;
        if (X->by_hand) { u.cnt_u = X->cnt_u.p; u.cnt_i = X->cnt_i.p; }
        int64_t max_rec = xchg ? (int64_t)B / 2 + (int64_t)world * 2 * B : (int64_t)3 * B / 2;
        if (known && X->by_hand && !xchg && X->lists_nb == nb && env_int("SML_A3_KNOWN_LISTS", 1)) {
            const int* h = X->lists_host;
            const int ou = h[b], oi = h[(nb + 1) + b];
            const int cu = h[2 * (nb + 1) + b * SML_PREP_CNT_STRIDE], ci = h[2 * (nb + 1) + nb * SML_PREP_CNT_STRIDE + b * SML_PREP_CNT_STRIDE];
            u.run_u = X->runs_u.p + ou; u.n_u = cu; u.run_i = X->runs_i.p + oi; u.n_i = ci;
            u.off_u = u.off_i = nullptr; u.cnt_u = u.cnt_i = nullptr; u.known = 1;
            max_rec = (int64_t)cu + ci;
        }
        u.dx = dxb; u.dx_i = xchg ? xchg->dx_items_all : dxb; u.w_user = w_user; u.w_item = w_item; u.lr = lr;
        if (hot) {
            u.hot_list = X->hot_list.p + (size_t)b * hot_cap * 3; u.hot_count = X->hot_count.p + b; u.hot_first = ctx->hot_first.p;
            u.hot_part = ctx->hot_part.p; u.hot_cap = hot_cap; u.hot_blocks = hot_chunks < 512 ? hot_chunks : 512;
        }
        ctx->prof.begin(PC_SEG_SGD, st); HIPCHK(sml_launch_run_sgd(d, dtype_bytes, u, max_rec, st)); ctx->prof.end(st);
        if (hot) { ctx->prof.begin(PC_PAIR_LOSS, st); HIPCHK(sml_launch_hot_apply(d, dtype_bytes, u, st)); ctx->prof.end(st); }
    }
    ctx->prof.begin(PC_MISC, st); HIPCHK(sml_launch_loss_finalize(ctx->loss_part.p, (int)nb, lstride, nullptr, batch_loss, st)); ctx->prof.end(st);
    return SML_OK;
}

int sml_embed_loss_sgd_epoch_sharded(sml_ctx* ctx, void* w_user, int64_t n_user, int64_t n_item, int dtype_bytes,
                                     const int64_t* triples, int64_t n, int batch, float lr, float lam_user, float lam_item,
                                     int loss_kind, float* batch_loss, const sml_bare_shard* sh, void* stream) {
    if (!ctx || !w_user || !triples || !batch_loss || !sh || n <= 0 || batch <= 0 || n_user <= 0 || n_item <= 0)
        return fail(SML_EINVAL, "sml_embed_loss_sgd_epoch_sharded", "bad argument");
    if (dtype_bytes != 4 && dtype_bytes != 2) return fail(SML_EINVAL, "sml_embed_loss_sgd_epoch_sharded", "dtype_bytes must be 4 or 2");
    if (loss_kind != SML_LOSS_BCE && loss_kind != SML_LOSS_BPR) return fail(SML_EINVAL, "sml_embed_loss_sgd_epoch_sharded", "loss_kind");
    if (batch > ctx->max_batch) return fail(SML_EINVAL, "sml_embed_loss_sgd_epoch_sharded", "batch exceeds ctx max_batch");
    const int W = sh->world;
    if (ctx->peer.world <= 0 || ctx->peer.world != W || ctx->peer.rank != sh->rank)
        return fail(SML_ESTATE, "sml_embed_loss_sgd_epoch_sharded", "needs sml_peer_attach with the same world / rank");
    if (!sh->item_shard || !sh->items_all || sh->head_rows < 0 || sh->shard_rows <= 0 || (sh->head_rows > 0 && !sh->w_item_head))
        return fail(SML_EINVAL, "sml_embed_loss_sgd_epoch_sharded", "incomplete shard descriptor");
    for (int q = 0; q < W; ++q) if (!sh->item_shard[q]) return fail(SML_EINVAL, "sml_embed_loss_sgd_epoch_sharded", "every rank's shard pointer is needed");
    if (sh->head_rows + (int64_t)W * sh->shard_rows < n_item) return fail(SML_EINVAL, "sml_embed_loss_sgd_epoch_sharded", "head + shards do not cover the item table");
    if (ctx->peer.rows_cap < 2 * (int64_t)batch) return fail(SML_EINVAL, "sml_embed_loss_sgd_epoch_sharded", "the inboxes' rows_cap must hold a batch's 2*batch gradient rows");
    if (sh->head_rows * ctx->d > 2 * (int64_t)sml_net_size(ctx->d) || (sh->head_rows * ctx->d) % 4)
        return fail(SML_EINVAL, "sml_embed_loss_sgd_epoch_sharded", "the dense head partial must fit a theta slot (head_rows * d <= 2 * net size)");
    DevGuard g(ctx->device);
    hipStream_t st = (hipStream_t)stream;
    const int d = ctx->d, me = sh->rank;
    const int64_t nb = (n + batch - 1) / batch, H = sh->head_rows;
    int rc;
    HIPCHK(ctx->dx.ensure((size_t)3 * batch * d));
    const int lpr = d * dtype_bytes / 16;
    const int lstride = (int)(((int64_t)batch * lpr + 255) / 256);
    HIPCHK(ctx->loss_part.ensure((size_t)nb * lstride));
    if (H > 0) HIPCHK(ctx->head_part.ensure((size_t)H * d));
    HIPCHK(ctx->ptr_tab.ensure(16));
    ctx->prof.begin(PC_SORT, st);
    rc = sort_epoch_sharded(&ctx->ix[0], &ctx->ix[1], triples, n, batch, n_user, sh, ctx->peer.rows_cap, st);
    ctx->prof.end(st);
    if (rc) return rc;
    void* inboxes[8];
    for (int q = 0; q < 8; ++q) inboxes[q] = q < W ? ctx->peer.inbox[q] : nullptr;
    HIPCHK(sml_launch_set_ptr_tab(ctx->ptr_tab.p, sh->item_shard, W, st));
    HIPCHK(sml_launch_set_ptr_tab(ctx->ptr_tab.p + 8, inboxes, W, st));
    HIPCHK(hipMemsetAsync(ctx->loss_part.p, 0, (size_t)nb * lstride * sizeof(float), st));
    IndexSet* A = &ctx->ix[0];
    IndexSet* Bs = &ctx->ix[1];
    for (int64_t b = 0; b < nb; ++b) {
        const int B = (int)((n - b * batch) < batch ? (n - b * batch) : batch);
        if (ctx->peer.done_pending) { ctx->prof.begin(PC_MISC, st); HIPCHK(sml_launch_peer_wait(ctx->peer.done_poll, st)); ctx->prof.end(st); }
        SmlBareArgs a;
        memset(&a, 0, sizeof(a));
        SmlPeerPoll rows_poll;
        int n_blocks = (int)(((int64_t)B * lpr + 255) / 256);
        peer_step(ctx, 1, n_blocks, &a.peer, &rows_poll);
        a.w_user = w_user; a.w_item = sh->w_item_head; a.tri = triples + b * batch * 3; a.B = B; a.dx = ctx->dx.p;
        a.loss_part = ctx->loss_part.p + b * lstride; a.kind = loss_kind; a.lam_user = lam_user; a.lam_item = lam_item;
        a.uniq = A->uniq.p + (size_t)3 * b * batch; a.lr = lr; a.scale = sh->loss_scale;
        a.shard_tab = reinterpret_cast<const void* const*>(ctx->ptr_tab.p);
        a.inbox_tab = reinterpret_cast<float* const*>(ctx->ptr_tab.p + 8);
        a.head_rows = H; a.shard_rows = sh->shard_rows;
        a.push_off = (long long)(a.peer.dst[me] - reinterpret_cast<float*>(ctx->peer.inbox[me]));
        ctx->prof.begin(PC_BARE_GRAD, st); HIPCHK(sml_launch_bare_grad(d, dtype_bytes, a, nullptr, st)); ctx->prof.end(st);
        ctx->prof.begin(PC_MISC, st); HIPCHK(sml_launch_peer_wait(rows_poll, st)); ctx->prof.end(st);
        SmlRunArgs u;
        memset(&u, 0, sizeof(u));
        u.run_u = A->runs_u.p; u.run_i = A->runs_i.p; u.off_u = A->off_u.p; u.off_i = A->off_i.p; u.batch_index = (int)b;
        u.val_u = A->val_u2.p; u.val_i = A->val_i2.p;
        if (A->by_hand) { u.cnt_u = A->cnt_u.p; u.cnt_i = A->cnt_i.p; }
        u.dx = ctx->dx.p; u.dx_i = rows_poll.slot0; u.w_user = w_user; u.w_item = sh->item_shard[me]; u.lr = lr;
        ctx->prof.begin(PC_SEG_SGD, st); HIPCHK(sml_launch_run_sgd(d, dtype_bytes, u, (int64_t)B / 2 + (int64_t)W * 2 * B, st)); ctx->prof.end(st);
        {
            SmlPeerPush done_push;
            peer_step(ctx, 2, 1, &done_push, &ctx->peer.done_poll);
            ctx->peer.done_pending = true;
            ctx->prof.begin(PC_MISC, st); HIPCHK(sml_launch_peer_signal(done_push, st)); ctx->prof.end(st);
        }
        if (H > 0) {
            HIPCHK(hipMemsetAsync(ctx->head_part.p, 0, (size_t)H * d * sizeof(float), st));
            SmlRunArgs hgt;
            memset(&hgt, 0, sizeof(hgt));
            hgt.run_u = Bs->runs_i.p; hgt.run_i = Bs->runs_i.p; hgt.off_u = Bs->off_u.p; hgt.off_i = Bs->off_i.p; hgt.batch_index = (int)b;
            hgt.val_u = Bs->val_i2.p; hgt.val_i = Bs->val_i2.p;
            if (Bs->by_hand) { hgt.cnt_u = Bs->cnt_u.p; hgt.cnt_i = Bs->cnt_i.p; }
            hgt.dx = ctx->dx.p; hgt.dx_i = ctx->dx.p; hgt.w_user = ctx->head_part.p; hgt.w_item = ctx->head_part.p;
            hgt.lr = -1.0f;
            ctx->prof.begin(PC_SEG_SGD, st); HIPCHK(sml_launch_run_sgd(d, 4, hgt, (int64_t)2 * B, st)); ctx->prof.end(st);
            SmlPeerPush hp; SmlPeerPoll hq;
            peer_step(ctx, 0, sml_peer_push_blocks(H * d), &hp, &hq);
            ctx->prof.begin(PC_MISC, st);
            HIPCHK(sml_launch_peer_push(ctx->head_part.p, H * d, hp, st));
            HIPCHK(sml_launch_head_apply(d, dtype_bytes, sh->w_item_head, H, lr, hq, st));
            ctx->prof.end(st);
        }
    }
    ctx->prof.begin(PC_MISC, st); HIPCHK(sml_launch_loss_finalize(ctx->loss_part.p, (int)nb, lstride, nullptr, batch_loss, st)); ctx->prof.end(st);
    return SML_OK;
}

int sml_embed_loss_adam_epoch(sml_ctx* ctx, const sml_mf_tables* t, const int64_t* triples, int64_t n, int batch, float lr,
                              float lam_user, float lam_item, int loss_kind, int64_t* step, float* batch_loss, void* stream) {
    if (!ctx || !t || !t->w_user || !t->w_item || !t->m_user || !t->v_user || !t->m_item || !t->v_item || !t->step_user ||
        !t->step_item || !triples || !step || !batch_loss || n <= 0 || batch <= 0)
        return fail(SML_EINVAL, "sml_embed_loss_adam_epoch", "bad argument");
    if (loss_kind != SML_LOSS_BCE && loss_kind != SML_LOSS_BPR) return fail(SML_EINVAL, "sml_embed_loss_adam_epoch", "loss_kind");
    if (batch > ctx->max_batch) return fail(SML_EINVAL, "sml_embed_loss_adam_epoch", "batch exceeds ctx max_batch");
    if (n > 0x3fffffff) return fail(SML_EINVAL, "sml_embed_loss_adam_epoch", "epoch too long");
    DevGuard g(ctx->device);
    hipStream_t st = (hipStream_t)stream;
    const int d = ctx->d;
    const int64_t nb = (n + batch - 1) / batch;
    int rc;
    if ((rc = ensure_sched(ctx, lr, *step + nb + 1, st))) return rc;
    HIPCHK(ctx->dx.ensure((size_t)3 * batch * d));
    HIPCHK(ctx->xin.ensure((size_t)3 * batch * d)); HIPCHK(ctx->mrep.ensure((size_t)3 * batch * d)); HIPCHK(ctx->vrep.ensure((size_t)3 * batch * d));
    const int lstride = (int)(((int64_t)batch * (d / 4) + 255) / 256);
    HIPCHK(ctx->loss_part.ensure((size_t)nb * lstride));
    ctx->prof.begin(PC_SORT, st); rc = sort_epoch(&ctx->ix[0], triples, n, batch, 0, t->n_user, t->n_item, false, st); ctx->prof.end(st);
    if (rc) return rc;
    HIPCHK(hipMemsetAsync(ctx->loss_part.p, 0, (size_t)nb * lstride * sizeof(float), st));
    for (int64_t b = 0; b < nb; ++b) {
        const int B = (int)((n - b * batch) < batch ? (n - b * batch) : batch);
        const int cur = (int)(*step + 1 + b);
        SmlBareArgs a;
        memset(&a, 0, sizeof(a));
        a.w_user = t->w_user; a.w_item = t->w_item; a.tri = triples + b * batch * 3; a.B = B; a.dx = ctx->dx.p;
        a.loss_part = ctx->loss_part.p + b * lstride; a.kind = loss_kind; a.lam_user = lam_user; a.lam_item = lam_item;
        a.m_user = t->m_user; a.v_user = t->v_user; a.m_item = t->m_item; a.v_item = t->v_item;
        a.last_user = t->step_user; a.last_item = t->step_item; a.sched = ctx->sched.p; a.cur_step = cur;
        a.xrep = ctx->xin.p; a.mrep = ctx->mrep.p; a.vrep = ctx->vrep.p; a.scale = 1.0f;
        ctx->prof.begin(PC_BARE_GRAD, st); HIPCHK(sml_launch_bare_grad(d, 4, a, nullptr, st)); ctx->prof.end(st);
        SmlRunArgs u;
        memset(&u, 0, sizeof(u));
        u.run_u = ctx->ix[0].rec_u.p + b * batch; u.n_u = B; u.val_u = ctx->ix[0].val_u2.p;
        u.run_i = ctx->ix[0].rec_i.p + 2 * b * batch; u.n_i = 2 * B; u.val_i = ctx->ix[0].val_i2.p;
        u.dx = ctx->dx.p; u.dx_i = ctx->dx.p; u.w_user = t->w_user; u.w_item = t->w_item;
        u.m_user = t->m_user; u.v_user = t->v_user; u.m_item = t->m_item; u.v_item = t->v_item;
        u.last_user = t->step_user; u.last_item = t->step_item; u.sched = ctx->sched.p; u.cur_step = cur; u.lr = lr; u.sched_len = replay_len(ctx, cur - 1);
        u.rep_x = ctx->xin.p; u.rep_m = ctx->mrep.p; u.rep_v = ctx->vrep.p; u.rep_u = 1; u.rep_i = 1; u.rep_x_stride = d; u.rep_x_off = 0;
        ctx->prof.begin(PC_SEG_ADAM, st); HIPCHK(sml_launch_run_adam(d, u, (int64_t)3 * B, st)); ctx->prof.end(st);
    }
    ctx->prof.begin(PC_MISC, st); HIPCHK(sml_launch_loss_finalize(ctx->loss_part.p, (int)nb, lstride, nullptr, batch_loss, st)); ctx->prof.end(st);
    *step += nb;
    return SML_OK;
}

int sml_mf_forward(sml_ctx* ctx, const float* w_user, const float* w_item, const int64_t* user, const int64_t* item,
                   int64_t n, int norm, float* uemb, float* iemb, float* score, void* stream) {
    if (!ctx || !w_user || !w_item || !user || !item || !uemb || !iemb || !score || n < 0)
        return fail(SML_EINVAL, "sml_mf_forward", "bad argument");
    if (n == 0) return SML_OK;
    DevGuard g(ctx->device);
    HIPCHK(sml_launch_mf_forward(ctx->d, w_user, w_item, user, item, n, norm, uemb, iemb, score, (hipStream_t)stream));
    return SML_OK;
}

int sml_eval_ranks(sml_ctx* ctx, const float* w_user, const float* w_item, const int64_t* rows, int64_t n, int n_cols,
                   int32_t* rank, void* stream) {
    if (ctx && n == 0) return SML_OK;
    if (!ctx || !w_user || !w_item || !rows || !rank || n < 0 || n_cols < 2)
        return fail(SML_EINVAL, "sml_eval_ranks", "bad argument");
    DevGuard g(ctx->device);
    hipStream_t st = (hipStream_t)stream;
    ctx->prof.begin(PC_EVAL_RANKS, st); HIPCHK(sml_launch_eval_ranks(ctx->d, w_user, w_item, rows, n, n_cols, rank, st)); ctx->prof.end(st);
    return SML_OK;
}

int sml_eval_prepare(sml_ctx* ctx, const int64_t* rows, int64_t n, int n_cols, int64_t n_item, int32_t* rows_b,
                     int32_t* bucket_off, void* stream) {
    if (ctx && n == 0 && n_cols >= 2 && n_item > 0) return SML_OK;
    if (!ctx || !rows || !rows_b || !bucket_off || n < 0 || n_cols < 2 || n_item <= 0 || n_item > 0x7fffffff)
        return fail(SML_EINVAL, "sml_eval_prepare", "bad argument");
    if ((uint64_t)n_item * (uint64_t)ctx->d * 4ull > 0x100000000ull)
// ... 530 lines not shown
    return SML_OK;
}

int sml_host_gather_pairs(const int64_t* ui, int64_t n_rows, const int64_t* order, int64_t n, int64_t* out3) {
    if (!ui || !order || !out3 || n < 0 || n_rows < 0) return fail(SML_EINVAL, "sml_host_gather_pairs", "bad argument");
    for (int64_t e = 0; e < n; ++e) {
        if (e + 16 < n) __builtin_prefetch(ui + 2 * order[e + 16]);
        const int64_t r = order[e];
        if (r < 0 || r >= n_rows) return fail(SML_EINVAL, "sml_host_gather_pairs", "index outside the data");
        out3[3 * e] = ui[2 * r]; out3[3 * e + 1] = ui[2 * r + 1];
    }
    return SML_OK;
}
int sml_host_gather_column(const void* mat, int64_t n_rows, int64_t row_stride_bytes, int elem_bytes, int64_t col,
                           const int64_t* order, int64_t n, int64_t* out3, int out_col) {
    if (!mat || !order || !out3 || n < 0 || (elem_bytes != 4 && elem_bytes != 8) || out_col < 0 || out_col > 2 || col < 0)
        return fail(SML_EINVAL, "sml_host_gather_column", "bad argument");
    const char* base = reinterpret_cast<const char*>(mat) + col * elem_bytes;
    for (int64_t e = 0; e < n; ++e) {
        if (e + 16 < n) __builtin_prefetch(base + order[e + 16] * row_stride_bytes);
        const int64_t r = order[e];
        if (r < 0 || r >= n_rows) return fail(SML_EINVAL, "sml_host_gather_column", "index outside the data");
        const char* p = base + r * row_stride_bytes;
        out3[3 * e + out_col] = elem_bytes == 8 ? *reinterpret_cast<const int64_t*>(p) : (int64_t)*reinterpret_cast<const int32_t*>(p);
    }
    return SML_OK;
}

int sml_stream_create_cu_range(void** stream, int device, int cu_lo, int cu_hi) {
    if (!stream) return fail(SML_EINVAL, "sml_stream_create_cu_range", "null stream pointer");
    DevGuard g(device);
    hipDeviceProp_t prop;
    HIPCHK(hipGetDeviceProperties(&prop, device));
    const int n_cu = prop.multiProcessorCount;
    if (cu_lo < 0 || cu_hi > n_cu || cu_lo >= cu_hi) return fail(SML_EINVAL, "sml_stream_create_cu_range", "range outside the device's CUs");
    std::vector<uint32_t> mask((size_t)(n_cu + 31) / 32, 0u);
    for (int b = cu_lo; b < cu_hi; ++b) mask[(size_t)b / 32] |= 1u << (b % 32);
    hipStream_t st = nullptr;
    HIPCHK(hipExtStreamCreateWithCUMask(&st, (uint32_t)mask.size(), mask.data()));
    *stream = st;
    return SML_OK;
}
int sml_stream_wait_stream(void* waiter, void* signaler) {
    static const unsigned flags = getenv("SML_EVENT_FLAGS") ? (unsigned)strtoul(getenv("SML_EVENT_FLAGS"), nullptr, 0)
                                                            : (hipEventDisableTiming | hipEventDisableSystemFence);
    hipEvent_t ev;
    HIPCHK(hipEventCreateWithFlags(&ev, flags));
    hipError_t e = hipEventRecord(ev, (hipStream_t)signaler);
    if (e == hipSuccess) e = hipStreamWaitEvent((hipStream_t)waiter, ev, 0);
    (void)hipEventDestroy(ev);
    if (e != hipSuccess) return fail(SML_EHIP, "sml_stream_wait_stream", hipGetErrorString(e));
    return SML_OK;
}
int sml_copy_tables(int n, void* const* dst, const void* const* src, const int64_t* bytes, void* stream) {
    if (n < 0 || n > 4 || (n && (!dst || !src || !bytes))) return fail(SML_EINVAL, "sml_copy_tables", "1..4 copies per call");
    long long b[4] = {0, 0, 0, 0};
    for (int q = 0; q < n; ++q) {
        if (bytes[q] == 0) continue;
        if (!dst[q] || !src[q] || bytes[q] < 0 || bytes[q] % 16 || ((uintptr_t)dst[q] | (uintptr_t)src[q]) % 16)
            return fail(SML_EINVAL, "sml_copy_tables", "pointers and sizes must be multiples of 16 bytes");
        b[q] = bytes[q];
    }
    HIPCHK(sml_launch_copy_tables(n, dst, src, b, (hipStream_t)stream));
    return SML_OK;
}
int sml_debug_timeline(long long* buf) { return sml_debug_set_timeline(buf) == hipSuccess ? 0 : -1; }
int sml_flag_set(int32_t* flag, int value, void* stream) {
    if (!flag || value < 0) return fail(SML_EINVAL, "sml_flag_set", "bad argument");
    HIPCHK(sml_launch_flag_set(flag, value, (hipStream_t)stream));
    return SML_OK;
}
int sml_flag_wait(int32_t* flag, int value, double timeout_s, void* stream) {
    if (!flag || value < 0 || !(timeout_s > 0)) return fail(SML_EINVAL, "sml_flag_wait", "bad argument");
    HIPCHK(sml_launch_flag_wait(flag, value, (long long)(timeout_s * 1e8), (hipStream_t)stream));
    return SML_OK;
}
int sml_stream_destroy(void* stream) {
    if (stream) HIPCHK(hipStreamDestroy((hipStream_t)stream));
    return SML_OK;
}

int sml_selftest(int device) {
    DevGuard g(device);
    const int M = 16, K = 32;
    std::vector<float> A(M * K), W(M * K), ref(M * M, 0.f), got(M * M, 0.f);
    for (int i = 0; i < M * K; ++i) {
        A[i] = (float)((i * 37 + 11) % 23) - 11.0f;
        W[i] = (float)((i * 53 + 5) % 19) - 9.0f + (float)(i / K);
    }
    for (int r = 0; r < M; ++r)
        for (int c = 0; c < M; ++c) {
            float s = 0.f;
            for (int k = 0; k < K; ++k) s += A[r * K + k] * W[c * K + k];
            ref[r * M + c] = s;
        }
    float *dA = nullptr, *dW = nullptr, *dP = nullptr, *dO = nullptr;
    HIPCHK(hipMalloc((void**)&dA, A.size() * 4)); HIPCHK(hipMalloc((void**)&dW, W.size() * 4));
    HIPCHK(hipMalloc((void**)&dP, 512 * 4)); HIPCHK(hipMalloc((void**)&dO, got.size() * 4));
    HIPCHK(hipMemcpy(dA, A.data(), A.size() * 4, hipMemcpyHostToDevice));
    HIPCHK(hipMemcpy(dW, W.data(), W.size() * 4, hipMemcpyHostToDevice));
    HIPCHK(sml_launch_selftest(dA, dW, dP, dO, nullptr));
    HIPCHK(hipDeviceSynchronize());
    HIPCHK(hipMemcpy(got.data(), dO, got.size() * 4, hipMemcpyDeviceToHost));
    (void)hipFree(dA); (void)hipFree(dW); (void)hipFree(dP); (void)hipFree(dO);
    for (int i = 0; i < M * M; ++i)
        if (got[i] != ref[i]) {
            char buf[128];
            snprintf(buf, sizeof(buf), "element (%d,%d): got %g want %g", i / M, i % M, got[i], ref[i]);
            return fail(SML_ESTATE, "sml_selftest: MFMA lane map mismatch", buf);
        }
    return SML_OK;
}

}
```

### sml_amd/csrc/mf_kernels.hip

```cpp
#include <hip/hip_fp16.h>
#include "sml_dev.h"
#include "sml_kernels.h"
#include "../../include/sml_hip.h"

#ifndef SML_NT
#define SML_NT 7
#endif
namespace {

template <typename T> struct RowVec;
template <> struct RowVec<float> {
    static constexpr int VEC = 4;
    __device__ static void load(const float* p, float (&x)[4]) {
        const f32x4 v = *reinterpret_cast<const f32x4*>(p);
        x[0] = v[0]; x[1] = v[1]; x[2] = v[2]; x[3] = v[3];
    }
    __device__ static void store(float* p, const float (&x)[4]) {
        f32x4 v; v[0] = x[0]; v[1] = x[1]; v[2] = x[2]; v[3] = x[3];
        *reinterpret_cast<f32x4*>(p) = v;
    }
    __device__ static void load_nt(const float* p, float (&x)[4]) {
        const f32x4 v = __builtin_nontemporal_load(reinterpret_cast<const f32x4*>(p));
        x[0] = v[0]; x[1] = v[1]; x[2] = v[2]; x[3] = v[3];
    }
// ... 68 lines not shown
    }
}
template <int LPR>
__device__ __forceinline__ float eval8_reduce(float (&a)[8], int sub) {
    static_assert(LPR == 8 || LPR == 16, "eight-at-a-time path: d = 32 or 64");
    butterfly_split<LPR / 2, 8>(a, sub);
    butterfly_split<LPR / 4, 4>(a, sub);
    butterfly_split<LPR / 8, 2>(a, sub);
    float v = a[0];
    if constexpr (LPR == 16) v += lane_xor<1>(v);
    return v;
}
template <int LPR>
__device__ __forceinline__ int eval8_index(int sub) {
    return ((sub & (LPR / 2)) ? 4 : 0) + ((sub & (LPR / 4)) ? 2 : 0) + ((sub & (LPR / 8)) ? 1 : 0);
}

__device__ __forceinline__ float dot4(const float (&a)[4], const float (&b)[4]) {
    return __fmaf_rn(a[3], b[3], __fmaf_rn(a[2], b[2], __fmaf_rn(a[1], b[1], __fmul_rn(a[0], b[0]))));
}

__device__ __forceinline__ float block_sum256(float v, float* sh4) {
#pragma unroll
    for (int off = 32; off >= 1; off >>= 1) v += __shfl_xor(v, off, 64);
    if ((threadIdx.x & 63) == 0) sh4[threadIdx.x >> 6] = v;
    __syncthreads();
    return sh4[0] + sh4[1] + sh4[2] + sh4[3];
}

template <int D>
__global__ __launch_bounds__(1024) void k_adaptive_users(const float* __restrict__ xin, float* __restrict__ dx, int B, float beta,
                                                         float* __restrict__ loss_slot) {
    constexpr int LPR = D / 4;
    __shared__ float part[16];
    const int grp = threadIdx.x / LPR, sub = threadIdx.x % LPR;
    float acc = 0.0f;
    for (int t = grp; t < B; t += 1024 / LPR) {
        float x[4], g[4];
        RowVec<float>::load(xin + ((int64_t)t * 3 + 1) * D + sub * 4, x);
        const float nrm = sqrtf(group_sum<LPR>(x[0] * x[0] + x[1] * x[1] + x[2] * x[2] + x[3] * x[3]));
        RowVec<float>::load(dx + (int64_t)t * D + sub * 4, g);
#pragma unroll
        for (int e = 0; e < 4; ++e) g[e] += 2.0f * beta * x[e] / nrm;
        RowVec<float>::store(dx + (int64_t)t * D + sub * 4, g);
        if (sub == 0) acc += beta * nrm;
    }
#pragma unroll
    for (int off = 32; off > 0; off >>= 1) acc += __shfl_xor(acc, off, 64);
    if ((threadIdx.x & 63) == 0) part[threadIdx.x >> 6] = acc;
    __syncthreads();
    if (threadIdx.x == 0) { float s2 = 0.0f; for (int w = 0; w < 16; ++w) s2 += part[w]; *loss_slot += s2; }
}

__global__ __launch_bounds__(256) void k_loss_finalize(const float* __restrict__ part, int n_batches, int stride,
                                                      float* __restrict__ out) {
    __shared__ float sh4[4];
    const int b = blockIdx.x;
    if (b >= n_batches) return;
    const float* p = part + (int64_t)b * stride;
    float s = 0.0f;
    int i = threadIdx.x;
    for (; i + 7 * 256 < stride; i += 8 * 256) {
        float x[8];
#pragma unroll
        for (int u = 0; u < 8; ++u) x[u] = p[i + u * 256];
#pragma unroll
        for (int u = 0; u < 8; ++u) s += x[u];
    }
    for (; i < stride; i += 256) s += p[i];
    const float tot = block_sum256(s, sh4);
    if (threadIdx.x == 0) out[b] = tot;
}

template <int D, typename T, bool LAZY, bool SH = false>
__global__ __launch_bounds__(256) void k_bare_grad(const int64_t* __restrict__ p_tri, const uint8_t* __restrict__ p_uniq, int p_B, SmlBareArgs a) {
    constexpr int VEC = RowVec<T>::VEC;
    constexpr int LPR = D / VEC;
    __shared__ float sh4[4];
    __shared__ SmlSched swin[LAZY ? SML_SW : 1];
    if constexpr (LAZY) {
        sched_window_load(swin, a.sched, a.cur_step - 1, threadIdx.x);
        __syncthreads();
    }
    const int gid = blockIdx.x * 256 + threadIdx.x;
    const int t = gid / LPR, sub = gid % LPR;
    float contrib = 0.0f;
    if (t < p_B) {
        const int64_t iu = p_tri[(int64_t)t * 3], ii = p_tri[(int64_t)t * 3 + 1], in = p_tri[(int64_t)t * 3 + 2];
        uint8_t mk_u = 0, mk_i = 0, mk_n = 0;
        if (!LAZY && p_uniq != nullptr) { mk_u = p_uniq[t]; mk_i = p_uniq[p_B + t]; mk_n = p_uniq[2 * p_B + t]; }
        __builtin_amdgcn_sched_barrier(0);
        float u[VEC], it[VEC], ng[VEC];
        if (SML_NT & 1) RowVec<T>::load_nt(reinterpret_cast<const T*>(a.w_user) + iu * D + sub * VEC, u);
        else RowVec<T>::load(reinterpret_cast<const T*>(a.w_user) + iu * D + sub * VEC, u);
        int qi = -1, qn = -1;
        auto item_row = [&](int64_t row, int& q) -> const T* {
            if constexpr (SH) {
                if (row >= a.head_rows) {
                    const int64_t r = row - a.head_rows;
                    q = (int)(r / a.shard_rows);
                    return reinterpret_cast<const T*>(a.shard_tab[q]) + (r - (int64_t)q * a.shard_rows) * D;
                }
            }
            return reinterpret_cast<const T*>(a.w_item) + row * D;
        };
        if constexpr (SH) {
            f32x4 raw[2];
            peer_load16x2(raw, reinterpret_cast<const float*>(item_row(ii, qi) + sub * VEC), reinterpret_cast<const float*>(item_row(in, qn) + sub * VEC));
            RowVec<T>::decode(raw[0], it);
            RowVec<T>::decode(raw[1], ng);
        } else {
            RowVec<T>::load(item_row(ii, qi) + sub * VEC, it);
            RowVec<T>::load(item_row(in, qn) + sub * VEC, ng);
        }
        if constexpr (LAZY) {
            static_assert(!LAZY || VEC == 4, "lazy Adam runs on fp32 tables");
            float m[3][4], v[3][4];
            RowVec<float>::load(a.m_user + iu * D + sub * 4, m[0]); RowVec<float>::load(a.v_user + iu * D + sub * 4, v[0]);
            RowVec<float>::load(a.m_item + ii * D + sub * 4, m[1]); RowVec<float>::load(a.v_item + ii * D + sub * 4, v[1]);
            RowVec<float>::load(a.m_item + in * D + sub * 4, m[2]); RowVec<float>::load(a.v_item + in * D + sub * 4, v[2]);
            const int fu = a.last_user[iu], fi = a.last_item[ii], fn = a.last_item[in];
#pragma unroll
// ... 400 lines not shown
            RowVec<float>::store((is_item ? a.m_item : a.m_user) + row * D + sub * 4, m);
            RowVec<float>::store((is_item ? a.v_item : a.v_user) + row * D + sub * 4, v);
            if (sub == 0) (is_item ? a.last_item : a.last_user)[row] = a.cur_step;
        }
    }
}

template <int D, typename T>
__global__ __launch_bounds__(256) void k_hot_apply(SmlRunArgs a) {
    constexpr int VEC = RowVec<T>::VEC;
    constexpr int LPR = D / VEC;
    constexpr int G = 64 / LPR;
    const int lane = threadIdx.x & 63, grp = lane / LPR, sub = lane % LPR;
    const int h = (blockIdx.x * 256 + threadIdx.x) >> 6;
    const int nh = min(*a.hot_count, a.hot_cap);
    if (h >= nh) return;
    const uint32_t packed = a.hot_list[3 * h];
    const int is_item = packed >> 31, len = (int)a.hot_list[3 * h + 1];
    const int first = a.hot_first[h], nchunks = (len + SML_HOT_CHUNK - 1) / SML_HOT_CHUNK;
    const int64_t row = a.hot_list[3 * h + 2];
    T* w = reinterpret_cast<T*>(is_item ? a.w_item : a.w_user);
    float p[VEC];
    if (grp == 0) RowVec<T>::load(w + row * D + sub * VEC, p);
    float g[VEC];
#pragma unroll
    for (int k = 0; k < VEC; ++k) g[k] = 0.0f;
    for (int c0 = grp; c0 < nchunks; c0 += 8 * G) {
        float x[8][VEC];
#pragma unroll
        for (int j = 0; j < 8; ++j)
            if (c0 + j * G < nchunks) {
                const float* src = a.hot_part + (int64_t)(first + c0 + j * G) * D + sub * VEC;
#pragma unroll
                for (int hh = 0; hh < VEC / 4; ++hh) RowVec<float>::load(src + hh * 4, reinterpret_cast<float(&)[4]>(x[j][hh * 4]));
            }
#pragma unroll
        for (int j = 0; j < 8; ++j)
            if (c0 + j * G < nchunks) {
#pragma unroll
                for (int k = 0; k < VEC; ++k) g[k] += x[j][k];
            }
    }
#pragma unroll
    for (int off = LPR; off < 64; off <<= 1)
#pragma unroll
        for (int k = 0; k < VEC; ++k) g[k] += __shfl_xor(g[k], off, 64);
    if (grp != 0) return;
#pragma unroll
    for (int k = 0; k < VEC; ++k) p[k] -= a.lr * g[k];
    RowVec<T>::store(w + row * D + sub * VEC, p);
}

template <int D>
__global__ __launch_bounds__(256) void k_adam_flush(float* __restrict__ w, float* __restrict__ mt, float* __restrict__ vt,
                                                    int32_t* __restrict__ last, int64_t rows,
                                                    const SmlSched* __restrict__ sched, int cur_step, int sched_len) {
    constexpr int LPR = D / 4;
    __shared__ SmlSched swin[SML_SW];
    __shared__ SmlReplayEnt rtab[SML_RP_N];
    sched_window_load(swin, sched, cur_step, threadIdx.x);
    const bool closed = sched_len > 0;
    if (closed) replay_table_build(rtab, sched, sched_len, cur_step, threadIdx.x);
    __syncthreads();
    const SmlReplayEnt* tab = closed ? rtab : nullptr;
    const int64_t total = rows * LPR;
    for (int64_t gid = (int64_t)blockIdx.x * 256 + threadIdx.x; gid < total; gid += (int64_t)gridDim.x * 256) {
        const int64_t row = gid / LPR;
        const int sub = (int)(gid % LPR);
        const int from = last[row];
        if (from < 0 || from >= cur_step) continue;
        float p[4], m[4], v[4];
        RowVec<float>::load(w + row * D + sub * 4, p);
        RowVec<float>::load(mt + row * D + sub * 4, m);
        RowVec<float>::load(vt + row * D + sub * 4, v);
        adam_replay_t4(p, m, v, from, cur_step, sched, swin, cur_step, tab);
        RowVec<float>::store(w + row * D + sub * 4, p);
        RowVec<float>::store(mt + row * D + sub * 4, m);
        RowVec<float>::store(vt + row * D + sub * 4, v);
        if (sub == 0) last[row] = cur_step;
    }
}

template <int D>
__global__ __launch_bounds__(256) void k_mf_forward(const float* __restrict__ wu, const float* __restrict__ wi,
                                                    const int64_t* __restrict__ user, const int64_t* __restrict__ item,
                                                    int64_t n, int norm, float* __restrict__ uemb,
                                                    float* __restrict__ iemb, float* __restrict__ score) {
    constexpr int LPR = D / 4;
    const int64_t gid = (int64_t)blockIdx.x * 256 + threadIdx.x;
    const int64_t t = gid / LPR;
    const int sub = (int)(gid % LPR);
    if (t >= n) return;
    float u[4], it[4];
    RowVec<float>::load(wu + user[t] * D + sub * 4, u);
    RowVec<float>::load(wi + item[t] * D + sub * 4, it);
    float s = mf_dot<LPR>(u, it), uu = 0.f;
#pragma unroll
    for (int k = 0; k < 4; ++k) uu += u[k] * u[k];
    if (norm) s = s / sqrtf(group_sum<LPR>(uu));
    RowVec<float>::store(uemb + t * D + sub * 4, u);
    RowVec<float>::store(iemb + t * D + sub * 4, it);
    if (sub == 0) score[t] = s;
}

template <int D>
__global__ __launch_bounds__(256) void k_eval_ranks(const float* __restrict__ wu, const float* __restrict__ wi,
                                                    const int64_t* __restrict__ rows, int64_t n, int n_cols,
                                                    int32_t* __restrict__ rank) {
    constexpr int LPR = D / 4;
    constexpr int G = 64 / LPR;
    const int lane = threadIdx.x & 63;
    const int64_t r = (int64_t)blockIdx.x * 4 + (threadIdx.x >> 6);
    if (r >= n) return;
    const int grp = lane / LPR, sub = lane % LPR;
    const int64_t* R = rows + r * n_cols;
    float u[4], x[4];
    RowVec<float>::load(wu + R[0] * D + sub * 4, u);
    RowVec<float>::load(wi + R[1] * D + sub * 4, x);
    const float s0 = eval_group_sum<LPR>(dot4(u, x));
    int cnt = 0;
    int c = 2;
    if constexpr (LPR <= 16) {
        for (; c + 8 * G <= n_cols; c += 8 * G) {
            const int cb = c + grp * 8;
            float y[8][4], a[8];
#pragma unroll
            for (int e = 0; e < 8; ++e) RowVec<float>::load(wi + R[cb + e] * D + sub * 4, y[e]);
#pragma unroll
            for (int e = 0; e < 8; ++e) a[e] = dot4(u, y[e]);
            const float sc = eval8_reduce<LPR>(a, sub);
            cnt += ((sub & (LPR / 8 - 1)) == 0 && sc > s0) ? 1 : 0;
        }
    }
// ... 402 lines not shown
    } while (x >= n);
    return x;
}
template <typename E>
__global__ __launch_bounds__(256) void k_device_epoch(const int64_t* __restrict__ ui, const E* __restrict__ mat, int64_t stride, int64_t col,
                                                      int64_t n, int hb, uint64_t seed, int64_t* __restrict__ out3) {
    const int64_t e = (int64_t)blockIdx.x * 256 + threadIdx.x;
    if (e >= n) return;
    const int64_t r = (int64_t)feistel_perm((uint64_t)e, (uint64_t)n, hb, seed);
    out3[3 * e] = ui[2 * r];
    out3[3 * e + 1] = ui[2 * r + 1];
    if (mat != nullptr) out3[3 * e + 2] = (int64_t)mat[r * stride + col];
}
__global__ __launch_bounds__(1024) void k_eval_metrics(const int32_t* __restrict__ rank, int64_t n, int topk,
                                                       float* __restrict__ out) {
    __shared__ float sh[2][16];
    float hits = 0.f, nd = 0.f;
    for (int64_t i = threadIdx.x; i < n; i += 1024) {
        const int rk = rank[i];
        if (rk < topk) { hits += 1.0f; nd += 1.0f / log2f((float)rk + 2.0f); }
    }
#pragma unroll
    for (int off = 32; off >= 1; off >>= 1) { hits += __shfl_xor(hits, off, 64); nd += __shfl_xor(nd, off, 64); }
    if ((threadIdx.x & 63) == 0) { sh[0][threadIdx.x >> 6] = hits; sh[1][threadIdx.x >> 6] = nd; }
    __syncthreads();
    if (threadIdx.x == 0) {
        float h = 0.f, d = 0.f;
        for (int w = 0; w < 16; ++w) { h += sh[0][w]; d += sh[1][w]; }
        out[0] = h; out[1] = d;
    }
}

#ifdef SML_TEST_PREP_REFERENCE
#define SML_PREP_REF_DEVICE_PART
#include "../../tests/csrc/prep_cub_kernels.inc"
#undef SML_PREP_REF_DEVICE_PART
#endif
}

#define SML_DISPATCH_D(d, ...)              \
    switch (d) {                             \
        case 32: { constexpr int DD = 32; __VA_ARGS__; } break;   \
        case 64: { constexpr int DD = 64; __VA_ARGS__; } break;   \
        case 128: { constexpr int DD = 128; __VA_ARGS__; } break; \
        default: return hipErrorInvalidValue; \
    }

hipError_t sml_launch_adaptive_users(int d, const float* xin, float* dx, int B, float beta, float* loss_slot, hipStream_t st) {
    if (B <= 0) return hipSuccess;
    SML_DISPATCH_D(d, k_adaptive_users<DD><<<dim3(1), dim3(1024), 0, st>>>(xin, dx, B, beta, loss_slot));
    return hipGetLastError();
}
hipError_t sml_launch_loss_finalize(const float* part, int n_batches, int stride, const int*, float* out, hipStream_t st) {
    k_loss_finalize<<<dim3(n_batches), dim3(256), 0, st>>>(part, n_batches, stride, out);
    return hipGetLastError();
}
hipError_t sml_launch_bare_grad(int d, int dtype_bytes, const SmlBareArgs& a, int* n_blocks, hipStream_t st) {
    const int lpr = d * dtype_bytes / 16;
    const int nb = (int)(((int64_t)a.B * lpr + 255) / 256);
    if (n_blocks) *n_blocks = nb;
    if (a.sched != nullptr) {
        if (dtype_bytes != 4) return hipErrorInvalidValue;
        SML_DISPATCH_D(d, k_bare_grad<DD, float, true><<<dim3(nb), dim3(256), 0, st>>>(a.tri, a.uniq, a.B, a));
    } else if (a.shard_tab != nullptr) {
        if (dtype_bytes == 4) { SML_DISPATCH_D(d, k_bare_grad<DD, float, false, true><<<dim3(nb), dim3(256), 0, st>>>(a.tri, a.uniq, a.B, a)); }
        else if (dtype_bytes == 2) { SML_DISPATCH_D(d, k_bare_grad<DD, __half, false, true><<<dim3(nb), dim3(256), 0, st>>>(a.tri, a.uniq, a.B, a)); }
        else return hipErrorInvalidValue;
    } else if (dtype_bytes == 4) {
        SML_DISPATCH_D(d, k_bare_grad<DD, float, false><<<dim3(nb), dim3(256), 0, st>>>(a.tri, a.uniq, a.B, a));
    } else if (dtype_bytes == 2) {
        SML_DISPATCH_D(d, k_bare_grad<DD, __half, false><<<dim3(nb), dim3(256), 0, st>>>(a.tri, a.uniq, a.B, a));
    } else return hipErrorInvalidValue;
    return hipGetLastError();
}
hipError_t sml_launch_head_apply(int d, int dtype_bytes, void* w_head, long long head_rows, float lr, const SmlPeerPoll& p, hipStream_t st) {
    if (head_rows <= 0) return hipSuccess;
    const int lpr = d * dtype_bytes / 16;
    const unsigned nb = (unsigned)((head_rows * lpr + 255) / 256);
    if (dtype_bytes == 4) { SML_DISPATCH_D(d, k_head_apply<DD, float><<<dim3(nb), dim3(256), 0, st>>>((float*)w_head, head_rows, lr, p)); }
    else if (dtype_bytes == 2) { SML_DISPATCH_D(d, k_head_apply<DD, __half><<<dim3(nb), dim3(256), 0, st>>>((__half*)w_head, head_rows, lr, p)); }
    else return hipErrorInvalidValue;
    return hipGetLastError();
}
struct SmlPtr8 { void* p[8]; };
__global__ void k_set_ptr_tab(void** dst, SmlPtr8 v) { if (threadIdx.x < 8) dst[threadIdx.x] = v.p[threadIdx.x]; }
hipError_t sml_launch_set_ptr_tab(void** dst, void* const* src, int n, hipStream_t st) {
    SmlPtr8 v;
    for (int q = 0; q < 8; ++q) v.p[q] = q < n ? src[q] : nullptr;
    k_set_ptr_tab<<<dim3(1), dim3(64), 0, st>>>(dst, v);
    return hipGetLastError();
}
hipError_t sml_launch_peer_signal(const SmlPeerPush& p, hipStream_t st) {
    k_peer_signal<<<dim3(1), dim3(64), 0, st>>>(p);
    return hipGetLastError();
}
hipError_t sml_launch_mark_runs(int key_bytes, const void* keys, const uint32_t* vals, int64_t n, int row_bits, SmlRun* rec,
                                uint8_t* flag_dup, uint8_t* uniq, int64_t uniq_stride, int64_t uniq_item_base, hipStream_t st) {
    if (n <= 0) return hipSuccess;
    const dim3 grid((unsigned)((n + 255) / 256));
    if (key_bytes == 4) k_mark_runs<uint32_t><<<grid, dim3(256), 0, st>>>((const uint32_t*)keys, vals, n, row_bits, rec, flag_dup, uniq, uniq_stride, uniq_item_base);
    else k_mark_runs<uint64_t><<<grid, dim3(256), 0, st>>>((const uint64_t*)keys, vals, n, row_bits, rec, flag_dup, uniq, uniq_stride, uniq_item_base);
    return hipGetLastError();
}
static int run_grid(int64_t records, int lpr, int cap_blocks) {
    int64_t nb = (records * lpr + 255) / 256;
    if (nb < 1) nb = 1;
    return (int)(nb > cap_blocks ? cap_blocks : nb);
}
hipError_t sml_launch_run_adam(int d, const SmlRunArgs& a, int64_t max_records, hipStream_t st) {
    const int nb = run_grid(max_records, d / 4, 4096);
    SML_DISPATCH_D(d, k_run_update<DD, float, 1, false><<<dim3(nb), dim3(256), 0, st>>>(a.run_u, a.run_i, a.off_u, a.off_i, a.n_u, a.n_i, a.batch_index, a.known, a.hot_blocks, a));
    return hipGetLastError();
}
hipError_t sml_launch_run_sgd(int d, int dtype_bytes, const SmlRunArgs& a, int64_t max_records, hipStream_t st) {
    const int nb = run_grid(max_records, d * dtype_bytes / 16, 4096) + a.hot_blocks;
    const bool hotb = a.hot_blocks > 0;
    if (dtype_bytes == 4) {
        if (hotb) { SML_DISPATCH_D(d, k_run_update<DD, float, 0, true><<<dim3(nb), dim3(256), 0, st>>>(a.run_u, a.run_i, a.off_u, a.off_i, a.n_u, a.n_i, a.batch_index, a.known, a.hot_blocks, a)); }
        else { SML_DISPATCH_D(d, k_run_update<DD, float, 0, false><<<dim3(nb), dim3(256), 0, st>>>(a.run_u, a.run_i, a.off_u, a.off_i, a.n_u, a.n_i, a.batch_index, a.known, a.hot_blocks, a)); }
    } else if (dtype_bytes == 2) {
        if (hotb) { SML_DISPATCH_D(d, k_run_update<DD, __half, 0, true><<<dim3(nb), dim3(256), 0, st>>>(a.run_u, a.run_i, a.off_u, a.off_i, a.n_u, a.n_i, a.batch_index, a.known, a.hot_blocks, a)); }
        else { SML_DISPATCH_D(d, k_run_update<DD, __half, 0, false><<<dim3(nb), dim3(256), 0, st>>>(a.run_u, a.run_i, a.off_u, a.off_i, a.n_u, a.n_i, a.batch_index, a.known, a.hot_blocks, a)); }
    } else return hipErrorInvalidValue;
    return hipGetLastError();
}
hipError_t sml_launch_hot_apply(int d, int dtype_bytes, const SmlRunArgs& a, hipStream_t st) {
    const int nb_apply = (a.hot_cap + 3) / 4;
    if (dtype_bytes == 4) {
        SML_DISPATCH_D(d, k_hot_apply<DD, float><<<dim3(nb_apply), dim3(256), 0, st>>>(a));
    } else if (dtype_bytes == 2) {
        SML_DISPATCH_D(d, k_hot_apply<DD, __half><<<dim3(nb_apply), dim3(256), 0, st>>>(a));
    } else return hipErrorInvalidValue;
    return hipGetLastError();
}
hipError_t sml_launch_adam_flush(int d, float* w, float* m, float* v, int32_t* last, int64_t rows,
                                 const SmlSched* sched, int cur_step, int sched_len, hipStream_t st) {
    const int lpr = d / 4;
    int64_t nb = (rows * lpr + 255) / 256;
    if (sched_len > 0 && nb > 2048) nb = 2048;
    SML_DISPATCH_D(d, k_adam_flush<DD><<<dim3((unsigned)nb), dim3(256), 0, st>>>(w, m, v, last, rows, sched, cur_step, sched_len));
    return hipGetLastError();
}
hipError_t sml_launch_mf_forward(int d, const float* wu, const float* wi, const int64_t* user, const int64_t* item,
                                 int64_t n, int norm, float* uemb, float* iemb, float* score, hipStream_t st) {
    const int lpr = d / 4;
    const int64_t nb = (n * lpr + 255) / 256;
    SML_DISPATCH_D(d, k_mf_forward<DD><<<dim3((unsigned)nb), dim3(256), 0, st>>>(wu, wi, user, item, n, norm, uemb, iemb, score));
    return hipGetLastError();
}
hipError_t sml_launch_eval_ranks(int d, const float* wu, const float* wi, const int64_t* rows, int64_t n, int n_cols,
                                 int32_t* rank, hipStream_t st) {
    const int64_t nb = (n + 3) / 4;
    SML_DISPATCH_D(d, k_eval_ranks<DD><<<dim3((unsigned)nb), dim3(256), 0, st>>>(wu, wi, rows, n, n_cols, rank));
    return hipGetLastError();
}
hipError_t sml_launch_eval_bucketize(const int64_t* rows, int64_t n, int n_cols, int64_t n_item, int32_t* rows_out,
                                     int32_t* bucket_off, hipStream_t st) {
    k_eval_bucketize<<<dim3((unsigned)((n + 3) / 4)), dim3(256), 0, st>>>(rows, n, n_cols, n_item, rows_out, bucket_off);
    return hipGetLastError();
}
struct SmlCopyJobs { f32x4* dst[4]; const f32x4* src[4]; long long n16[4]; int n_jobs; };
__global__ __launch_bounds__(256) void k_copy_tables(SmlCopyJobs j) {
    const long long stride = (long long)gridDim.x * 256;
    for (int q = 0; q < j.n_jobs; ++q) {
        f32x4* __restrict__ d = j.dst[q];
        const f32x4* __restrict__ s = j.src[q];
        for (long long i = (long long)blockIdx.x * 256 + threadIdx.x; i < j.n16[q]; i += stride)
            __builtin_nontemporal_store(__builtin_nontemporal_load(s + i), d + i);
    }
}
hipError_t sml_launch_copy_tables(int n_jobs, void* const* dst, const void* const* src, const long long* bytes, hipStream_t st) {
    SmlCopyJobs j;
    long long most = 0;
    j.n_jobs = n_jobs;
    for (int q = 0; q < 4; ++q) {
        j.dst[q] = q < n_jobs ? reinterpret_cast<f32x4*>(dst[q]) : nullptr;
        j.src[q] = q < n_jobs ? reinterpret_cast<const f32x4*>(src[q]) : nullptr;
        j.n16[q] = q < n_jobs ? bytes[q] / 16 : 0;
        if (j.n16[q] > most) most = j.n16[q];
    }
    if (most == 0) return hipSuccess;
    long long nb = (most + 1023) / 1024;
    if (nb > 4096) nb = 4096;
    k_copy_tables<<<dim3((unsigned)nb), dim3(256), 0, st>>>(j);
    return hipGetLastError();
}

__global__ void k_flag_set(int* flag, int value) {
    __hip_atomic_store(flag, value, __ATOMIC_RELAXED, __HIP_MEMORY_SCOPE_SYSTEM);
}
__global__ void k_flag_wait(int* flag, int value, long long timeout) {
    if (threadIdx.x != 0) return;
    const long long t0 = wall_clock64();
    for (;;) {
        const int v = __hip_atomic_load(flag, __ATOMIC_RELAXED, __HIP_MEMORY_SCOPE_SYSTEM);
        if (v >= value) return;
        if (wall_clock64() - t0 > timeout) { __hip_atomic_fetch_add(flag + 1, 1, __ATOMIC_RELAXED, __HIP_MEMORY_SCOPE_SYSTEM); return; }
        __builtin_amdgcn_s_sleep(32);
    }
}
__global__ __launch_bounds__(256) void k_peer_push(const f32x4* __restrict__ src, long long n16, SmlPeerPush p) {
    const long long stride = (long long)gridDim.x * 256;
    for (long long i = (long long)blockIdx.x * 256 + threadIdx.x; i < n16; i += stride) {
        const f32x4 v = src[i];
        for (int q = 0; q < p.world; ++q) peer_store16(p.dst[q] + 4 * i, v);
    }
    peer_signal(p);
}
__global__ __launch_bounds__(64) void k_peer_wait(SmlPeerPoll p) { peer_wait(p); }
__global__ __launch_bounds__(256) void k_peer_sum(float* __restrict__ dst, long long n, SmlPeerPoll p, int theta_net) {
    peer_wait(p);
    const long long i = (long long)blockIdx.x * 256 + threadIdx.x;
    if (i >= n) return;
    float g = peer_load(p.slot0 + i);
    for (int q = 1; q < p.world; ++q) g += peer_load(p.slot0 + q * p.slot_stride + i);
    if (theta_net > 0) { const int off = (int)(i % theta_net); if (off < SML_OFF_F1W && !conv_slot_used_host(off)) g = 0.0f; }
    dst[i] = g;
}
__global__ __launch_bounds__(256) void k_peer_read(const float* __restrict__ src, f32x4* __restrict__ dst, long long n16) {
    const long long stride = (long long)gridDim.x * 256 * 2;
    for (long long i = ((long long)blockIdx.x * 256 + threadIdx.x) * 2; i < n16; i += stride) {
        f32x4 v[2];
        const long long j = i + 1 < n16 ? i + 1 : i;
        peer_load16x2(v, src + 4 * i, src + 4 * j);
        dst[i] = v[0];
        if (j != i) dst[j] = v[1];
    }
}
hipError_t sml_launch_peer_read(const void* src, void* dst, long long n16, hipStream_t st) {
    long long nb = (n16 + 511) / 512;
    nb = nb < 1 ? 1 : nb > 1024 ? 1024 : nb;
    k_peer_read<<<dim3((unsigned)nb), dim3(256), 0, st>>>(reinterpret_cast<const float*>(src), reinterpret_cast<f32x4*>(dst), n16);
    return hipGetLastError();
}
int sml_peer_push_blocks(long long n_floats) {
    long long nb = (n_floats / 4 + 1023) / 1024;
    return (int)(nb < 1 ? 1 : nb > 256 ? 256 : nb);
// ... 96 lines not shown
```

### sml_amd/csrc/sml_kernels.h

```cpp
#pragma once
#include <hip/hip_runtime.h>
#include <stdint.h>
#include "sml_dev.h"

#define SML_RUN_INL 4
struct __attribute__((aligned(16))) SmlRun { uint32_t row, pos, len, pad; uint32_t slot[SML_RUN_INL]; };

#define SML_TILE_ENT 256
struct __attribute__((aligned(16))) SmlTileHdr {
    uint32_t count;
    uint32_t nrows;
    uint32_t spill;
    uint32_t pad;
    unsigned short len[16];
};

struct SmlSeg {
    const float* theta;
    const float* pk;
    const float* xt_tab;
    const float* xh_tab;
    const float* m_tab;
    const float* v_tab;
    const int32_t* last_tab;
// ... 84 lines not shown
struct SmlWgSeg {
    const float* dz1; const float* a1; const float* dout; const float* a2;
    float* grad;
    int n_rows;
    const float* theta_net; const float* pk_net; const float* xin;
};
struct SmlWgArgs {
    SmlWgSeg seg[2];
    float* theta; float* m; float* v; float* pk;
    const float* convg_part; int tiles0, tiles_total;
    float weight_decay, step_size, bc2_sqrt;
    SmlPeerPush peer;
    int n_tail; float* convg_out; int* arrive;
    int defer_conv;
    int gelu_b;
};

struct SmlThetaAdamArgs {
    float* theta; float* m; float* v; float* grad; float* pk;
    float weight_decay, step_size, bc2_sqrt;
    SmlPeerPoll peer;
    const float* clip_sumsq; float clip_max_norm;
};
hipError_t sml_launch_grad_sumsq(const float* grad, int64_t n, float* out, hipStream_t st);
hipError_t sml_launch_conv_state_init(int d, const float* theta, const float* m, const float* v, float* cs, hipStream_t st);

hipError_t sml_launch_fwd(int d, int mt, int ns, const SmlFwdArgs& a, int tiles_total, hipStream_t st, bool side = false);
hipError_t sml_launch_bwd(int d, int split, const SmlBwdArgs& a, int tiles_total, hipStream_t st);
hipError_t sml_launch_wgrad(int d, const SmlWgArgs& a, hipStream_t st);
hipError_t sml_launch_tr_bwd_head(int d, const SmlBwdArgs& a, int tiles_total, hipStream_t st);
hipError_t sml_launch_tr_wgrad2(int d, const SmlWgArgs& a, hipStream_t st);
int sml_wgrad2_pushers(int d);
hipError_t sml_launch_theta_adam(int d, const SmlThetaAdamArgs& a, hipStream_t st);
hipError_t sml_launch_theta_pack(int d, const float* theta, float* pk, hipStream_t st);
size_t sml_bx3_bytes(int d);
hipError_t sml_launch_theta_pack_bx3(int d, const float* theta, void* pkx, hipStream_t st);
hipError_t sml_launch_mf_fwd_bx3(int d, const SmlFwdArgs& a, const void* pkx, int tiles, hipStream_t st);
hipError_t sml_launch_fwd_bx3(int d, const SmlFwdArgs& a, const void* pkx_net, int tiles, hipStream_t st, bool side);
int sml_wgrad_grid(int d);
int sml_peer_push_blocks(long long n_floats);
hipError_t sml_launch_peer_push(const float* src, long long n_floats, const SmlPeerPush& p, hipStream_t st);
hipError_t sml_launch_peer_wait(const SmlPeerPoll& p, hipStream_t st);
hipError_t sml_launch_peer_sum(float* dst, long long n_floats, const SmlPeerPoll& p, hipStream_t st, int theta_net = 0);
hipError_t sml_launch_peer_read(const void* src, void* dst, long long n16, hipStream_t st);
hipError_t sml_launch_selftest(const float* A, const float* W, float* pk, float* out, hipStream_t st);

struct SmlShardKeys {
    int mode;
    int rank; long long head_rows, shard_rows, rows_cap;
};
hipError_t sml_launch_adaptive_users(int d, const float* xin, float* dx, int B, float beta, float* loss_slot, hipStream_t st);
hipError_t sml_launch_loss_finalize(const float* part, int n_batches, int stride, const int* counts,
                                    float* out, hipStream_t st);


struct SmlRunArgs {
    const SmlRun* run_u; int n_u;
    const SmlRun* run_i; int n_i;
    const int* off_u; const int* off_i; int batch_index;
    const int* cnt_u; const int* cnt_i;
    int known;
    const uint32_t* val_u; const uint32_t* val_i;
    const float* dx;
    const float* dx_i;
    void* w_user; void* w_item;
    float* m_user; float* v_user; float* m_item; float* v_item;
    int32_t* last_user; int32_t* last_item;
    const SmlSched* sched; int cur_step;
    int sched_len;
    const float* rep_x; const float* rep_m; const float* rep_v; int rep_u, rep_i;
    int rep_x_stride, rep_x_off;
    float lr;
    SmlPeerPoll wait;
    const uint32_t* hot_list;
    const int* hot_count;
    int hot_blocks;
    int* hot_first;
    float* hot_part;
    int hot_cap;
};
#define SML_HOT 128
#define SML_HOT_CHUNK 512
#define SML_HOT_MAXCAP 8192
#define SML_PREP_CNT_STRIDE 32
#define SML_PREP_IPT 4
#define SML_PREP_TT (1024 * SML_PREP_IPT)
#define SML_PREP_MAXBK 1024
#define SML_PREP_CG 8
#define SML_PREP_SMALL 2048
#define SML_PREP_CROWS 2048
#define SML_PREP_CCAP 1536
#define SML_PREP_CDUP 1024
struct SmlPrepTable {
    int nbk, lb;
    int hb;
    int vb;
    int npass, pbits;
    int wave;
    int ntile;
    int lmul;
    int allruns;
    int rshift;
    void* ent; void* ent2;
    uint32_t* hist;
    uint2* bk;
    uint32_t* brc;
    SmlRun* runs_tmp;
    uint32_t* vals;
    SmlRun* runs;
    int* run_off; int* run_cnt;
};
struct SmlPrepArgs {
    const int64_t* tri; int64_t n; int batch; int nb; int tpb;
    const int* boff;
    int pad_tiles;
    int records;
    int mode, has_users, nis;
    const int64_t* items_all; int64_t val_q;
    const uint64_t* x_keys; const uint32_t* x_vals;
    int64_t head_rows, shard_rows; int shard_rank;
    SmlPrepTable t[2];
    uint8_t* uniq; int64_t uniq_stride;
    uint32_t* slot_info; int64_t slot_stride;
    int dense; SmlRun* dense_rec; int* dense_n; int64_t dense_stride;
    SmlTileHdr* tile_hdr; uint2* tile_ent; uint2* tile_spill; int* spill_cnt; int tiles_cap;
    uint32_t* hot_list; int* hot_count; int hot_cap; int* max_len;
    uint32_t* medium; int* n_medium;
    uint32_t* large; int* n_large; int large_cap;
    const int* rank_viol;
    int* order_viol;
    int vals_ascend;
};
hipError_t sml_launch_rank_probe(int* viol, hipStream_t st);
hipError_t sml_launch_prep(const SmlPrepArgs& a, int ent_bytes, hipStream_t st);
hipError_t sml_launch_hot_apply(int d, int dtype_bytes, const SmlRunArgs& a, hipStream_t st);
hipError_t sml_launch_run_adam(int d, const SmlRunArgs& a, int64_t max_records, hipStream_t st);
hipError_t sml_launch_run_sgd(int d, int dtype_bytes, const SmlRunArgs& a, int64_t max_records, hipStream_t st);
hipError_t sml_launch_adam_flush(int d, float* w, float* m, float* v, int32_t* last, int64_t rows,
                                 const SmlSched* sched, int cur_step, int sched_len, hipStream_t st);
hipError_t sml_launch_mark_runs(int key_bytes, const void* keys, const uint32_t* vals, int64_t n, int row_bits, SmlRun* rec,
                                uint8_t* flag_dup, uint8_t* uniq, int64_t uniq_stride, int64_t uniq_item_base, hipStream_t st);
hipError_t sml_launch_mark_unique(int key_bytes, const void* keys, const uint32_t* vals, int64_t n, int row_bits, uint8_t* uniq,
                                  int64_t uniq_stride, hipStream_t st);
hipError_t sml_launch_make_runs(int key_bytes, const void* keys, const uint32_t* vals, int64_t n, int row_bits, const uint32_t* heads,
                                const int* n_heads, int64_t max_heads, SmlRun* runs, int* max_len, int64_t seg, int is_item,
                                uint32_t* hot_list, int* hot_count, int hot_cap, hipStream_t st);
hipError_t sml_launch_batch_offsets(const SmlRun* runs, const int* n_sel, int nb, int64_t seg, int* off, hipStream_t st);
hipError_t sml_launch_build_item_keys_x(int key_bytes, const int64_t* items_all, int world, int64_t n, int batch, int row_bits_i,
                                        void* key_i, uint32_t* val_i, hipStream_t st);
hipError_t sml_launch_build_item_keys_sh(int key_bytes, const int64_t* items_all, int world, int64_t n, int batch, int row_bits_i,
                                         const SmlShardKeys& sk, void* key_i, uint32_t* val_i, hipStream_t st);
hipError_t sml_launch_head_apply(int d, int dtype_bytes, void* w_head, long long head_rows, float lr, const SmlPeerPoll& p, hipStream_t st);
hipError_t sml_launch_peer_signal(const SmlPeerPush& p, hipStream_t st);
hipError_t sml_launch_set_ptr_tab(void** dst, void* const* src, int n, hipStream_t st);
hipError_t sml_launch_zero_item_marks(uint8_t* uniq, int64_t n, int batch, hipStream_t st);
hipError_t sml_launch_build_keys(int key_bytes, const int64_t* tri, int64_t n, int batch, int pad_tiles, int row_bits_u,
                                 int row_bits_i, void* key_u, uint32_t* val_u, void* key_i, uint32_t* val_i, const int* boff,
                                 int nb, hipStream_t st);

struct SmlBareArgs {
    void* w_user; void* w_item;
    const uint8_t* uniq;
    float lr;
    const int64_t* tri; int B;
    float* dx;
    float* loss_part;
    int kind; float lam_user, lam_item;
    float scale;
    const float* m_user; const float* v_user; const float* m_item; const float* v_item;
    const int32_t* last_user; const int32_t* last_item;
    const SmlSched* sched; int cur_step;
    float* xrep; float* mrep; float* vrep;
    const void* const* shard_tab; float* const* inbox_tab;
    long long head_rows, shard_rows, push_off;
    SmlPeerPush peer;
};

hipError_t sml_launch_bare_grad(int d, int dtype_bytes, const SmlBareArgs& a, int* n_blocks, hipStream_t st);
hipError_t sml_launch_mf_forward(int d, const float* wu, const float* wi, const int64_t* user, const int64_t* item,
                                 int64_t n, int norm, float* uemb, float* iemb, float* score, hipStream_t st);
hipError_t sml_launch_eval_ranks(int d, const float* wu, const float* wi, const int64_t* rows, int64_t n,
                                 int n_cols, int32_t* rank, hipStream_t st);
hipError_t sml_launch_eval_bucketize(const int64_t* rows, int64_t n, int n_cols, int64_t n_item, int32_t* rows_out,
                                     int32_t* bucket_off, hipStream_t st);
hipError_t sml_launch_copy_tables(int n_jobs, void* const* dst, const void* const* src, const long long* bytes, hipStream_t st);
hipError_t sml_debug_set_timeline(long long* buf);
hipError_t sml_launch_flag_set(int* flag, int value, hipStream_t st);
hipError_t sml_launch_flag_wait(int* flag, int value, long long timeout_ticks, hipStream_t st);
hipError_t sml_launch_eval_ranks_bucketed(int d, const float* wu, const float* wi, const int32_t* rows_b,
                                          const int32_t* bucket_off, int64_t n, int n_cols, int32_t* rank, int max_blocks,
                                          hipStream_t st);
int sml_evs_slices(int d, int64_t n_item);
hipError_t sml_launch_evs_prepare(const int64_t* rows, int64_t n, int n_cols, int ns, int32_t* whist, int32_t* mbcnt, int32_t* seg_off,
                                  uint32_t* entries, hipStream_t st);
hipError_t sml_launch_evs_ranks(int d, const float* wu, const float* wi, const int64_t* rows, const uint32_t* entries, const int32_t* seg_off,
                                int64_t n, int n_cols, int64_t n_item, int ns, float* ug, float* s0, uint16_t* partial, int32_t* rank,
                                int max_blocks, hipStream_t st);
hipError_t sml_launch_sample_negatives(const int64_t* users, int64_t n, const int64_t* item_all, int64_t pop, const int64_t* user_ptr,
                                       int64_t n_users, const int64_t* user_items, uint64_t seed, int64_t* negs, int* failed,
                                       hipStream_t st);
hipError_t sml_launch_device_epoch(const int64_t* ui, const void* mat, int elem_bytes, int64_t stride, int64_t col, int64_t n, uint64_t seed,
                                   int64_t* out3, hipStream_t st);
hipError_t sml_launch_eval_metrics(const int32_t* rank, int64_t n, int topk, float* out, hipStream_t st);
bool sml_retrieval_supports(int d, int elem_bytes);
hipError_t sml_launch_full_rank(int d, int elem_bytes, const void* wu, const void* wi, int64_t n_item, const int64_t* rows, int64_t n,
                                int n_cols, const int64_t* seen_off, const int32_t* seen_items, int32_t* rank, hipStream_t st);
int64_t sml_topk_scratch_size(int64_t n, int k, int64_t n_item);
hipError_t sml_launch_topk(int d, int elem_bytes, const void* wu, const void* wi, int64_t n_item, const int64_t* users, int64_t n,
                           int k, const int64_t* seen_off, const int32_t* seen_items, void* scratch, int32_t* items, float* scores,
                           hipStream_t st);
int64_t sml_user_rank_scratch_size(int64_t n_pos);
hipError_t sml_launch_user_rank(int d, int elem_bytes, const void* wu, const void* wi, int64_t n_item, const int64_t* users, int64_t n,
                                const int64_t* pos_off, const int32_t* pos_items, int64_t n_pos, const int64_t* seen_off,
                                const int32_t* seen_items, void* scratch, int32_t* above, int32_t* pos, hipStream_t st);
hipError_t sml_launch_user_metrics(const int32_t* pos, const int64_t* pos_off, int64_t n, const int32_t* ks, int n_k,
                                   int32_t* hits, float* dcg, float* ap, int32_t* first, hipStream_t st);
int64_t sml_rank_weights_scratch_size(int64_t n);
hipError_t sml_launch_rank_weights(int d, const float* wu, const float* wi, const int64_t* rows, int64_t n, void* scratch,
                                   float* score, int32_t* rank, int32_t* order, float* p, hipStream_t st);
hipError_t sml_launch_weighted_epoch(const int64_t* rows, int64_t n, const int32_t* order, const int64_t* item_all, int64_t pop,
                                     const int64_t* user_ptr, int64_t n_users, const int64_t* user_items, int64_t n_out,
                                     uint64_t seed, int64_t* out3, int* failed, hipStream_t st);
```

### sml_amd/engine.py

```python
import ctypes

import numpy as np
import torch

from . import _lib
from ._lib import check

NET_PARAM_ORDER = ("conv1.weight", "conv1.bias", "conv2.weight", "conv2.bias",
                   "fc1.weight", "fc1.bias", "fc2.weight", "fc2.bias")


def _ptr(t):
    return ctypes.c_void_p(t.data_ptr()) if t is not None else ctypes.c_void_p(0)


class HipEngine(object):
    def __init__(self, device, d, max_batch=4096, lib=None):
        self.lib = _lib.load() if lib is None else lib
        if not torch.cuda.is_available():
            raise RuntimeError("HipEngine needs a GPU (torch.cuda.is_available() is False); there is no CPU path")
        self.device = torch.device(device)
        if self.device.type != "cuda":
            raise RuntimeError("HipEngine device must be a cuda (HIP) device, got %s" % device)
        if self.device.index is None:
# ... 37 lines not shown
                self.lib.sml_peer_close(self.device.index, ctypes.c_void_p(p))

    def __del__(self):
        try:
            self.close()
        except Exception:
            pass

    def _stream(self):
        return ctypes.c_void_p(torch.cuda.current_stream(self.device).cuda_stream)

    def _dev(self, t, dtype):
        if isinstance(t, np.ndarray):
            t = torch.from_numpy(np.ascontiguousarray(t))
            if t.dtype != dtype:
                t = t.to(dtype)
            return t.pin_memory().to(device=self.device, non_blocking=True)
        t = t.to(device=self.device, dtype=dtype)
        return t if t.is_contiguous() else t.contiguous()

    def _table(self, t):
        if t.device != self.device or t.dtype != torch.float32 or not t.is_contiguous() or t.shape[-1] != self.d:
            raise ValueError("expected a contiguous fp32 [rows,%d] tensor on %s, got %s %s on %s"
                             % (self.d, self.device, tuple(t.shape), t.dtype, t.device))
        return t

    def adopt(self, transfer):
        key = id(transfer)
        ent = self._flat.get(key)
        if ent is not None and ent[2] is transfer:
            flat, views = ent[0], ent[1]
            if all(p.data_ptr() == flat.data_ptr() + 4 * off for (p, off, _) in views):
                return flat
        flat = torch.zeros(2 * self.net_size, device=self.device, dtype=torch.float32)
        views = []
        for ni, net in enumerate((transfer.user_transfer, transfer.item_transfer)):
            named = dict(net.named_parameters())
            for w, name in enumerate(NET_PARAM_ORDER):
                p = named[name]
                off = ni * self.net_size + self.offsets[w]
                n = p.numel()
                if name == "conv1.weight" and p.shape[2] == 2:
                    block = flat[off:off + 30].view(10, 3)
                    block[:, :2].copy_(p.data.reshape(10, 2).to(self.device, torch.float32))
                    p.data = block[:, :2].view(10, 1, 2, 1)
                    views.append((p, off, n))
                    continue
                flat[off:off + n].copy_(p.data.reshape(-1).to(self.device, torch.float32))
                p.data = flat[off:off + n].view(p.shape)
                views.append((p, off, n))
        if len(self._flat) >= 8:
            self._flat.pop(next(iter(self._flat)))
        self._flat[key] = (flat, views, transfer)
        return flat

    def load_optimizer_state(self, mfbase=None, mf_state=None, transfer=None, tr_state=None):
        if mf_state is not None:
            self._mf_tables(mfbase, None, None)
            s = self.mf_state
            for key, src in (("m_u", "m_user"), ("v_u", "v_user"), ("m_i", "m_item"), ("v_i", "v_item")):
                s[key].copy_(torch.as_tensor(mf_state[src]).to(self.device, torch.float32))
            self.mf_step = int(mf_state["step"])
            s["s_u"].fill_(self.mf_step)
            s["s_i"].fill_(self.mf_step)
        if tr_state is not None:
            theta = self._select(transfer)
            if self.tr_state is None or self.tr_state[0].shape != theta.shape:
                self.tr_state = (torch.zeros_like(theta), torch.zeros_like(theta), torch.zeros_like(theta))
            names = {id(p): n for n, p in transfer.named_parameters()}
            for flat, src in ((self.tr_state[0], tr_state["m"]), (self.tr_state[1], tr_state["v"])):
                flat.zero_()
                for p, off, n in self._flat[id(transfer)][1]:
                    t = torch.as_tensor(src[names[id(p)]]).to(self.device, torch.float32)
                    if p.dim() == 4 and p.shape[2] == 2 and p.shape[0] == 10:
                        flat[off:off + 30].view(10, 3)[:, :2].copy_(t.reshape(10, 2))
                    else:
                        flat[off:off + n].copy_(t.reshape(-1))
            self.tr_step = int(tr_state["step"])

    def _select(self, transfer):
        variant = 1 if int(getattr(transfer.user_transfer, "kernel", 3)) == 2 else 0
        if variant != getattr(self, "_variant", 0):
            check(self.lib.sml_ctx_set_variant(self._ctx, variant), "sml_ctx_set_variant")
            self._variant = variant
        return self.adopt(transfer)

    def transfer_forward(self, transfer, x_t, x_hat, which):
        net = {"user": 0, "item": 1}.get(which)
        if net is None:
            raise TypeError("convtransfer has not this type")
        theta = self._select(transfer)
        x_t = self._table(self._dev(x_t, torch.float32))
        x_hat = self._table(self._dev(x_hat.detach(), torch.float32))
        out = torch.empty_like(x_t)
        check(self.lib.sml_transfer_forward(self._ctx, _ptr(theta), net, _ptr(x_t), _ptr(x_hat), _ptr(out),
                                            x_t.shape[0], self._stream()), "sml_transfer_forward")
        return out

    def updata(self, transfer, last_user, hat_user, last_item, hat_item, out_user, out_item):
        theta = self._select(transfer)
        for net, (xt, xh, out) in enumerate(((last_user, hat_user, out_user), (last_item, hat_item, out_item))):
            xt, xh, out = self._table(xt), self._table(xh), self._table(out)
            if out.data_ptr() in (xt.data_ptr(), xh.data_ptr()):
                raise ValueError("updata output may not alias its inputs")
            check(self.lib.sml_transfer_forward(self._ctx, _ptr(theta), net, _ptr(xt), _ptr(xh), _ptr(out),
                                                xt.shape[0], self._stream()), "sml_transfer_forward")

# ... 576 lines not shown
        st = HipEngine._MASKED.get(key)
        if st is None:
            h = ctypes.c_void_p()
            check(self.lib.sml_stream_create_cu_range(ctypes.byref(h), key[0], key[1], key[2]), "sml_stream_create_cu_range")
            st = HipEngine._MASKED[key] = torch.cuda.ExternalStream(h.value, device=self.device)
        return st

    def training_stream(self):
        if self._side_cus() <= 0:
            return None
        if getattr(self, "_train", None) is None:
            self._train = self._masked_stream(0, self._n_cus() - self._side_cus())
        return self._train

    def partition(self):
        import contextlib, os

        @contextlib.contextmanager
        def scope():
            ts = self.training_stream() if os.environ.get("SML_TRAIN_PARTITION", "1") != "0" else None
            if ts is None:
                yield
                return
            outer = torch.cuda.current_stream(self.device)
            ts.wait_stream(outer)
            with torch.cuda.stream(ts):
                yield
            outer.wait_stream(ts)
        return scope()

    def _side_eval_cap(self):
        if self.SIDE_EVAL_WORKGROUPS > 0:
            return self.SIDE_EVAL_WORKGROUPS
        return 4 * self._side_cus() if self._side_cus() > 0 else 256

    def _side_stream(self):
        if getattr(self, "_side", None) is None:
            if self._side_cus() > 0:
                n = self._n_cus()
                self._side = self._masked_stream(n - self._side_cus(), n)
                return self._side
            prio = 0
            try:
                lo, _hi = torch.cuda.Stream.priority_range()
                prio = int(lo)
            except Exception:
                prio = 0
            try:
                self._side = torch.cuda.Stream(device=self.device, priority=prio)
            except Exception:
                self._side = torch.cuda.Stream(device=self.device)
        return self._side

    def copy_tables(self, pairs):
        pairs = list(pairs)
        for k in range(0, len(pairs), 4):
            chunk = pairs[k:k + 4]
            n = len(chunk)
            dst, src, nbytes = (ctypes.c_void_p * n)(), (ctypes.c_void_p * n)(), (ctypes.c_int64 * n)()
            for q, (d, s) in enumerate(chunk):
                if d.shape != s.shape or d.dtype != s.dtype or not (d.is_contiguous() and s.is_contiguous()) \
                        or (d.numel() * d.element_size()) % 16 or d.data_ptr() % 16 or s.data_ptr() % 16 or d.numel() == 0:
                    d.copy_(s)
                    dst[q], src[q], nbytes[q] = None, None, 0
                    continue
                dst[q], src[q], nbytes[q] = d.data_ptr(), s.data_ptr(), d.numel() * d.element_size()
            check(self.lib.sml_copy_tables(n, dst, src, nbytes, self._stream()), "sml_copy_tables")

    def _snap_slot(self, cur):
        ring = self.__dict__.setdefault("_snap", [])
        k = self.__dict__.get("_snap_next", 0) % self.SNAPSHOTS
        self._snap_next = k + 1
        while len(ring) <= k:
            ring.append(dict(ev=None))
        slot = ring[k]
        if slot["ev"] is not None:
            cur.wait_event(slot["ev"])
        return slot

    @staticmethod
    def _snap_buf(slot, key, like):
        if slot.get(key) is None or slot[key].shape != like.shape:
            slot[key] = torch.empty_like(like)
        return slot[key]

    def _side_order(self, cur, side):
        mode = __import__("os").environ.get("SML_SIDE_SYNC", "flag")
        if mode == "event":
            check(self.lib.sml_stream_wait_stream(ctypes.c_void_p(side.cuda_stream), ctypes.c_void_p(cur.cuda_stream)),
                  "sml_stream_wait_stream")
            return
        if getattr(self, "_sync_flag", None) is None:
            self._sync_flag = torch.zeros(2, device=self.device, dtype=torch.int32)
            self._sync_seq = 0
            self._sync_seen = 0
        self._sync_seq += 1
        check(self.lib.sml_flag_set(_ptr(self._sync_flag), self._sync_seq, ctypes.c_void_p(cur.cuda_stream)), "sml_flag_set")
        check(self.lib.sml_flag_wait(_ptr(self._sync_flag), self._sync_seq, self._flag_timeout(),
                                     ctypes.c_void_p(side.cuda_stream)), "sml_flag_wait")

    def eval_submit(self, user_tab, item_tab, rows):
        wu, wi = self._table(user_tab), self._table(item_tab)
        rows = self._dev(rows, torch.int64)
        side = self._side_stream()
        cur = torch.cuda.current_stream(self.device)
        slot = self._snap_slot(cur)
        su, si = self._snap_buf(slot, "u", wu), self._snap_buf(slot, "i", wi)
        self.copy_tables([(su, wu), (si, wi)])
        self._side_order(cur, side)
        with torch.cuda.stream(side):
            ranks = self.eval_ranks(su, si, rows, max_workgroups=self._side_eval_cap())
            ev = torch.cuda.Event()
            ev.record(side)
        slot["ev"] = ev
        rows.record_stream(side)
        return dict(ranks=ranks, event=ev, n=rows.shape[0])

    TRANSFERRED_MAX_BYTES = int(__import__("os").environ.get("SML_TRANSFERRED_MAX_BYTES", str(24 << 30)))

    def can_submit_transferred(self, user_tab, item_tab):
        if __import__("os").environ.get("SML_EVAL_TRANSFERRED", "1") == "0":
            return False
        per_slot = 3 * (user_tab.numel() + item_tab.numel()) * 4
        return per_slot * self.SNAPSHOTS <= self.TRANSFERRED_MAX_BYTES

    def _side_ctx(self):
        if getattr(self, "_side_ctx_h", None) is None:
            h = ctypes.c_void_p()
            check(self.lib.sml_ctx_create(ctypes.byref(h), self.device.index or 0, self.d, 1024), "sml_ctx_create")
            self._side_ctx_h, self._side_variant = h, -1
        if self._side_variant != getattr(self, "_variant", 0):
            check(self.lib.sml_ctx_set_variant(self._side_ctx_h, getattr(self, "_variant", 0) | 2), "sml_ctx_set_variant")
            self._side_variant = getattr(self, "_variant", 0)
        return self._side_ctx_h

    def eval_submit_transferred(self, transfer, last_user, hat_user, last_item, hat_item, rows):
        theta = self._select(transfer)
        tabs = [self._table(t) for t in (last_user, hat_user, last_item, hat_item)]
        rows = self._dev(rows, torch.int64)
        side = self._side_stream()
        cur = torch.cuda.current_stream(self.device)
        slot = self._snap_slot(cur)
        snaps = [self._snap_buf(slot, k, t) for k, t in zip(("lu", "hu", "li", "hi"), tabs)]
        su, si = self._snap_buf(slot, "u", tabs[0]), self._snap_buf(slot, "i", tabs[2])
        sth = self._snap_buf(slot, "theta", theta)
        self.copy_tables(list(zip(snaps, tabs)))
        sth.copy_(theta)
        self._side_order(cur, side)
        ctx = self._side_ctx()
        with torch.cuda.stream(side):
            for net, (xt, xh, out) in enumerate(((snaps[0], snaps[1], su), (snaps[2], snaps[3], si))):
                check(self.lib.sml_transfer_forward(ctx, _ptr(sth), net, _ptr(xt), _ptr(xh), _ptr(out), xt.shape[0],
                                                    self._stream()), "sml_transfer_forward")
            ranks = self.eval_ranks(su, si, rows, max_workgroups=self._side_eval_cap())
            ev = torch.cuda.Event()
            ev.record(side)
        slot["ev"] = ev
        rows.record_stream(side)
        return dict(ranks=ranks, event=ev, n=rows.shape[0])

    def eval_metrics_submit(self, handle, topk):
        side = self._side_stream()
        with torch.cuda.stream(side):
            out = torch.empty(2, device=self.device, dtype=torch.float32)
            check(self.lib.sml_eval_metrics(self._ctx, _ptr(handle["ranks"]), handle["n"], int(topk), _ptr(out),
                                            self._stream()), "sml_eval_metrics")
            ev = torch.cuda.Event()
            ev.record(side)
        return (out, ev)

    @staticmethod
    def _flag_timeout():
        import os
        return float(os.environ.get("SML_FLAG_TIMEOUT_S", "300"))

    def side_sync_check(self, block=True):
        flag = getattr(self, "_sync_flag", None)
        if flag is None:
            return
        side = self._side_stream()
        if block:
            with torch.cuda.stream(side):
                n = int(flag[1].item())
        else:
            n = self._sync_seen
            pend = getattr(self, "_sync_pending", None)
            if pend is not None and pend[1].query():
                n = int(pend[0][0])
                self._sync_pending = pend = None
            if pend is None:
                host = getattr(self, "_sync_host", None)
                if host is None:
                    host = self._sync_host = torch.zeros(1, dtype=torch.int32).pin_memory()
                with torch.cuda.stream(side):
                    host.copy_(flag[1:2], non_blocking=True)
                    ev = torch.cuda.Event()
                    ev.record(side)
                self._sync_pending = (host, ev)
        if n > self._sync_seen:
            new, self._sync_seen = n - self._sync_seen, n
            raise RuntimeError("%d side-stream evaluation(s) gave up waiting for their table snapshot (sml_flag_wait "
                               "timeout, SML_FLAG_TIMEOUT_S=%g): their results are not trustworthy" % (new, self._flag_timeout()))

    def eval_result(self, pending, check=True):
        out, ev = pending[0], pending[1]
        ev.synchronize()
# ... 194 lines not shown
```

### sml_amd/period.py

```python
import numpy as np
import torch

from . import synth


class Hyper(object):

    def __init__(self, **kw):
        self.multi_num = 10
        self.MF_epochs = 1
        self.TR_epochs = 1
        self.MF_batch_size = 1024
        self.TR_batch_size = 256
        self.MF_lr = 0.01
        self.l2 = 1e-6
        self.TR_lr = 0.001
        self.TR_l2 = 1e-4
        self.topK = 20
        self.__dict__.update(kw)


class PeriodState(object):

    def __init__(self, mfbase, transfer):
        self.MFbase = mfbase
        self.transfer = transfer
        wu, wi = mfbase.user_laten.weight.data, mfbase.item_laten.weight.data
        self.last_user, self.last_item = torch.zeros_like(wu), torch.zeros_like(wi)
        self.hat_user, self.hat_item = wu.clone(), wi.clone()
        self.prev_hat_user, self.prev_hat_item = wu.clone(), wi.clone()


class PeriodPlan(object):

    def __init__(self, val_rows, mf_triples, tr_triples):
        self.val_rows = val_rows
        self.mf_triples = mf_triples
        self.tr_triples = tr_triples

    def n_train_triples(self):
        return sum(t.shape[0] for ph in self.mf_triples for t in ph) + \
               sum(t.shape[0] for ph in self.tr_triples for t in ph)


def synth_plan(seed, n_inter, n_user, n_item, neg, hp, device, user_lo=0, user_hi=None, with_val=True):
    rng = np.random.RandomState(seed)
    user_hi = n_user if user_hi is None else user_hi
    span = user_hi - user_lo

    def period(n):
        train, test = synth.sample_period(rng, n, span, n_item, neg=neg)
        train[:, 0] += user_lo
        test[:, 0] += user_lo
        return train, test

    _, set_t = period(n_inter)
    set_tt, val = period(n_inter)
    mf, tr = [], []
    for ph in range(hp.multi_num):
        eps = []
        for ep in range(hp.MF_epochs):
            order = rng.permutation(n_inter)
            col = 2 + rng.randint(0, neg)
            eps.append(torch.from_numpy(np.ascontiguousarray(set_t[order][:, [0, 1, col]])).to(device))
        mf.append(eps)
        eps = []
        items = np.unique(set_tt[:, 1])
        for ep in range(hp.TR_epochs):
            order = rng.permutation(n_inter)
            negs = items[rng.randint(0, items.shape[0], size=n_inter)]
            tri = np.concatenate([set_tt[order], negs[:, None]], axis=1)
            eps.append(torch.from_numpy(np.ascontiguousarray(tri)).to(device))
        tr.append(eps)
    val_rows = torch.from_numpy(val).to(device) if with_val else None
    return PeriodPlan(val_rows, mf, tr)


class RoutedEpoch(object):

    def __init__(self, route, d, device, with_exchange):
        self.local_tri = torch.from_numpy(route.local_tri).to(device)
        self.cap, self.plan = route.cap, route.plan
        self.exchange = route.exchange(d) if with_exchange else None
        self.n_global = route.n


def route_plan(dctx, plan, hp, n_user_global, d, device, mean_loss=True):
    mf = [[RoutedEpoch(dctx.route_epoch(t.cpu().numpy(), hp.MF_batch_size, n_user_global, mean_loss), d, device, True) for t in ph]
          for ph in plan.mf_triples]
    tr = [[RoutedEpoch(dctx.route_epoch(t.cpu().numpy(), hp.TR_batch_size, n_user_global, mean_loss), d, device, False) for t in ph]
          for ph in plan.tr_triples]
    val = None
    if plan.val_rows is not None:
        val = torch.from_numpy(dctx.route_rows(plan.val_rows.cpu().numpy(), n_user_global)).to(device)
    out = PeriodPlan(val, mf, tr)
    out.n_global_triples = sum(e.n_global for ph in mf for e in ph) + sum(e.n_global for ph in tr for e in ph)
    return out


def run_period(engine, st, plan, hp, record=None, overlap=True, exchanges=None):
    mf, net = st.MFbase, st.transfer
    wu, wi = mf.user_laten.weight.data, mf.item_laten.weight.data
    state = {"version": 0, "cached": None}
    notes = []

    def evaluate(tag):
        if plan.val_rows is None:
            return
        if state["cached"] is None or state["cached"][0] != state["version"]:
            if overlap and hasattr(engine, "eval_submit"):
                pending = engine.eval_metrics_submit(engine.eval_submit(wu, wi, plan.val_rows), hp.topK)
                box = {}

                def res(pending=pending, box=box):
                    if "v" not in box:
                        box["v"] = engine.eval_result(pending)
                    return box["v"]
            else:
                val = engine.eval_metrics(engine.eval_ranks(wu, wi, plan.val_rows), hp.topK)

                def res(val=val):
                    return val
            state["cached"] = (state["version"], res)
        notes.append((tag, state["cached"][1]))

    def updata():
        engine.updata(net, st.last_user, st.hat_user, st.last_item, st.hat_item, wu, wi)
        state["version"] += 1

    transferred_ok = (overlap and plan.val_rows is not None and hasattr(engine, "eval_submit_transferred")
                      and engine.can_submit_transferred(wu, wi))

    def evaluate_transferred(tag):
        pending = engine.eval_metrics_submit(
            engine.eval_submit_transferred(net, st.last_user, st.hat_user, st.last_item, st.hat_item, plan.val_rows), hp.topK)
        box = {}

        def res(pending=pending, box=box):
            if "v" not in box:
                box["v"] = engine.eval_result(pending)
            return box["v"]
        notes.append((tag, res))

    copy = engine.copy_tables if hasattr(engine, "copy_tables") else (lambda pairs: [d.copy_(s) for d, s in pairs])
    copy([(st.last_user, wu), (st.last_item, wi)])
    mf_loss = tr_loss = None
    for ph in range(hp.multi_num):
        evaluate("before MF")
        for tri in plan.mf_triples[ph]:
            if isinstance(tri, RoutedEpoch):
                mf_loss = engine.mf_stage_epoch(mf, net, st.last_user, st.last_item, tri.local_tri, tri.cap,
                                                hp.MF_lr, hp.l2, norm=False, bce=True, plan=tri.plan, exchange=tri.exchange)
            else:
                ex = exchanges.get(id(tri)) if exchanges else None
                mf_loss = engine.mf_stage_epoch(mf, net, st.last_user, st.last_item, tri, hp.MF_batch_size,
                                                hp.MF_lr, hp.l2, norm=False, bce=True, exchange=ex)
            engine.mf_flush(mf)
            state["version"] += 1
            evaluate("MF epoch")
        copy([(st.prev_hat_user, st.hat_user), (st.prev_hat_item, st.hat_item)])
        copy([(st.hat_user, wu), (st.hat_item, wi)])
        n_tr = len(plan.tr_triples[ph])
        if transferred_ok and n_tr > 0:
            evaluate_transferred("before TR")
        else:
            updata()
            evaluate("before TR")
        for k_tr, tri in enumerate(plan.tr_triples[ph]):
            if isinstance(tri, RoutedEpoch):
                tr_loss = engine.tr_stage_epoch(net, st.last_user, st.last_item, st.hat_user, st.hat_item, tri.local_tri,
                                                tri.cap, hp.TR_lr, hp.TR_l2, bce=True, plan=tri.plan)
            else:
                tr_loss = engine.tr_stage_epoch(net, st.last_user, st.last_item, st.hat_user, st.hat_item, tri,
                                                hp.TR_batch_size, hp.TR_lr, hp.TR_l2, bce=True)
            if plan.val_rows is not None:
                if transferred_ok and k_tr + 1 < n_tr:
                    evaluate_transferred("TR epoch")
                else:
                    updata()
                    evaluate("TR epoch")
    updata()
    if record is not None and plan.val_rows is not None:
        n = plan.val_rows.shape[0]
        for tag, res in notes:
            hits, ndcg = res()
            record.append((tag, hits / n, ndcg / n))
    elif plan.val_rows is not None and overlap and hasattr(engine, "side_sync_check"):
        engine.side_sync_check(block=False)
    return mf_loss, tr_loss
```

Measured before the change: 16.05 million triples/s.

## Cut per-epoch launches: cache theta packs, fold loss zeroing, merge flush and copies

Adds a theta-version scope so repeated theta_pack and bx3 pack launches are skipped while theta is unchanged within a period. The loss-partial buffer is now zeroed by the finalize kernel instead of a separate memset, and the TR grad memset is skipped on the fused path. Other merges: the two Adam flushes become one two-table kernel, the two hat-table copy calls become one launch of four copies, and copy_tables can signal a flag from the copy kernel (off by default). The aim is fewer small kernel launches and memsets per epoch. The risks are stale packs if a theta write misses the version bump, and a read/write hazard in the merged copy, where hat_user is both a source and a destination.

```diff
diff --git a/include/sml_hip.h b/include/sml_hip.h
--- a/include/sml_hip.h
+++ b/include/sml_hip.h
@@ -32,6 +32,7 @@
 int64_t sml_theta_net_size(int d);
 int64_t sml_theta_offset(int d, int which);
 int sml_theta_pack(sml_ctx* ctx, const float* theta, void* stream);
+int sml_ctx_theta_scope(sml_ctx* ctx, int on);
 
 int sml_comm_load(const char* librccl_path);
 int sml_comm_unique_id(void* out128);
@@ -171,6 +172,8 @@
                           const uint32_t* entries, const int32_t* seg_off, int64_t n, int n_cols, int64_t n_item,
                           void* scratch, int32_t* rank, int max_workgroups, void* stream);
 int sml_copy_tables(int n, void* const* dst, const void* const* src, const int64_t* bytes, void* stream);
+int sml_copy_tables_signal(int n, void* const* dst, const void* const* src, const int64_t* bytes, int32_t* flag, int value,
+                           void* stream);
 
 int sml_stream_create_cu_range(void** stream, int device, int cu_lo, int cu_hi);
 int sml_stream_destroy(void* stream);
diff --git a/sml_amd/_lib.py b/sml_amd/_lib.py
--- a/sml_amd/_lib.py
+++ b/sml_amd/_lib.py
@@ -59,6 +59,7 @@
     "sml_theta_net_size": (ctypes.c_int64, [ctypes.c_int]),
     "sml_theta_offset": (ctypes.c_int64, [ctypes.c_int, ctypes.c_int]),
     "sml_theta_pack": (ctypes.c_int, [c_void, c_void, c_void]),
+    "sml_ctx_theta_scope": (ctypes.c_int, [c_void, ctypes.c_int]),
     "sml_transfer_forward": (ctypes.c_int, [c_void, c_void, ctypes.c_int, c_void, c_void, c_void, ctypes.c_int64, c_void]),
     "sml_mf_stage_epoch": (ctypes.c_int, [c_void, c_void, ctypes.POINTER(MFTables), c_void, ctypes.c_int64, ctypes.c_int,
                                           ctypes.c_float, ctypes.c_float, ctypes.c_int, ctypes.POINTER(ctypes.c_int64),
@@ -115,6 +116,8 @@
     "sml_stream_destroy": (ctypes.c_int, [c_void]),
     "sml_stream_wait_stream": (ctypes.c_int, [c_void, c_void]),
     "sml_copy_tables": (ctypes.c_int, [ctypes.c_int, ctypes.POINTER(c_void), ctypes.POINTER(c_void), ctypes.POINTER(ctypes.c_int64), c_void]),
+    "sml_copy_tables_signal": (ctypes.c_int, [ctypes.c_int, ctypes.POINTER(c_void), ctypes.POINTER(c_void), ctypes.POINTER(ctypes.c_int64), c_void,
+                                              ctypes.c_int, c_void]),
     "sml_flag_set": (ctypes.c_int, [c_void, ctypes.c_int, c_void]),
     "sml_flag_wait": (ctypes.c_int, [c_void, ctypes.c_int, ctypes.c_double, c_void]),
     "sml_comm_load": (ctypes.c_int, [ctypes.c_char_p]),
diff --git a/sml_amd/csrc/capi.hip b/sml_amd/csrc/capi.hip
--- a/sml_amd/csrc/capi.hip
+++ b/sml_amd/csrc/capi.hip
@@ -197,6 +197,11 @@
     Buf<float> pkx;
     Buf<float> cstate;
     int pk_set = 0;
+    bool theta_scope = false;
+    uint64_t theta_ver = 1;
+    const float* pk_theta = nullptr;  uint64_t pk_ver = 0;
+    const float* pkx_theta = nullptr; uint64_t pkx_ver = 0;
+    const float* loss_clean_p = nullptr; size_t loss_clean_cap = 0;
     Buf<int> arrive;
     Buf<int> run_arrive;
     Buf<SmlSched> sched;
@@ -373,6 +378,36 @@
     return SML_OK;
 }
 float* pk_cur(const sml_ctx* c) { return c->pk.p + (size_t)c->pk_set * 2 * sml_pk_size(c->d); }
+bool hk_on(const char* name) { return env_int(name, 1) != 0; }
+int pack_pk(sml_ctx* c, const float* theta, hipStream_t st, bool force = false) {
+    if (!force && c->theta_scope && hk_on("SML_HK_PACK_ONCE") && c->pk_theta == theta && c->pk_ver == c->theta_ver) return SML_OK;
+    c->prof.begin(PC_PACK, st); HIPCHK(sml_launch_theta_pack(c->d, theta, pk_cur(c), st)); c->prof.end(st);
+    c->pk_theta = theta; c->pk_ver = c->theta_ver;
+    return SML_OK;
+}
+int pack_pkx(sml_ctx* c, const float* theta, hipStream_t st) {
+    const size_t had = c->pkx.cap;
+    HIPCHK(c->pkx.ensure(sml_bx3_bytes(c->d) / sizeof(float) + 4));
+    if (had == c->pkx.cap && c->theta_scope && hk_on("SML_HK_PACK_ONCE") && c->pkx_theta == theta && c->pkx_ver == c->theta_ver) return SML_OK;
+    c->prof.begin(PC_PACK, st); HIPCHK(sml_launch_theta_pack_bx3(c->d, theta, c->pkx.p, st)); c->prof.end(st);
+    c->pkx_theta = theta; c->pkx_ver = c->theta_ver;
+    return SML_OK;
+}
+int loss_part_begin(sml_ctx* c, size_t need, bool fold, hipStream_t st) {
+    HIPCHK(c->loss_part.ensure(need));
+    const bool clean = fold && c->loss_clean_p == c->loss_part.p && c->loss_clean_cap == c->loss_part.cap;
+    c->loss_clean_p = nullptr;
+    if (!clean) HIPCHK(hipMemsetAsync(c->loss_part.p, 0, (fold ? c->loss_part.cap : need) * sizeof(float), st));
+    return SML_OK;
+}
+int loss_part_end(sml_ctx* c, int nb, int lstride, bool fold, float* batch_loss, hipStream_t st) {
+    c->prof.begin(PC_MISC, st);
+    if (fold) HIPCHK(sml_launch_loss_finalize_zero(c->loss_part.p, nb, lstride, batch_loss, st));
+    else HIPCHK(sml_launch_loss_finalize(c->loss_part.p, nb, lstride, nullptr, batch_loss, st));
+    c->prof.end(st);
+    if (fold) { c->loss_clean_p = c->loss_part.p; c->loss_clean_cap = c->loss_part.cap; }
+    return SML_OK;
+}
 float* pk_other(const sml_ctx* c) { return c->pk.p + (size_t)(1 - c->pk_set) * 2 * sml_pk_size(c->d); }
 
 int ceil_log2(int64_t x) { int b = 0; while (((int64_t)1 << b) < x) ++b; return b; }
@@ -630,6 +665,7 @@
 
 int sml_ctx_set_variant(sml_ctx* ctx, int variant) {
     if (!ctx || variant < 0 || variant > 3) return fail(SML_EINVAL, "sml_ctx_set_variant", "variant must be 0 or 1 (+ 2: an evaluation-stream context)");
+    if (ctx->variant != (variant & 1)) ctx->theta_ver++;
     ctx->variant = variant & 1; ctx->side = (variant & 2) != 0;
     return SML_OK;
 }
@@ -666,7 +702,14 @@
     DevGuard g(ctx->device);
     int rc = ensure_pk(ctx); if (rc) return rc;
     hipStream_t st = (hipStream_t)stream;
-    ctx->prof.begin(PC_PACK, st); HIPCHK(sml_launch_theta_pack(ctx->d, theta, pk_cur(ctx), st)); ctx->prof.end(st);
+    if ((rc = pack_pk(ctx, theta, st, true))) return rc;
+    return SML_OK;
+}
+
+int sml_ctx_theta_scope(sml_ctx* ctx, int on) {
+    if (!ctx || (on != 0 && on != 1)) return fail(SML_EINVAL, "sml_ctx_theta_scope", "bad argument");
+    ctx->theta_scope = on == 1;
+    ctx->theta_ver++;
     return SML_OK;
 }
 
@@ -680,8 +723,7 @@
     int rc = ensure_pk(ctx); if (rc) return rc;
     const size_t bx3 = n_rows > 8192 && env_int("SML_FWD_BX3", 1) != 0 && env_int("SML_FWD_MT", 0) == 0 ? sml_bx3_bytes(ctx->d) : 0;
     if (bx3) {
-        HIPCHK(ctx->pkx.ensure(bx3 / sizeof(float) + 4));
-        ctx->prof.begin(PC_PACK, st); HIPCHK(sml_launch_theta_pack_bx3(ctx->d, theta, ctx->pkx.p, st)); ctx->prof.end(st);
+        if ((rc = pack_pkx(ctx, theta, st))) return rc;
         SmlFwdArgs a;
         memset(&a, 0, sizeof(a));
         SmlSeg& s = a.seg[0];
@@ -695,7 +737,7 @@
         ctx->prof.end(st);
         return SML_OK;
     }
-    ctx->prof.begin(PC_PACK, st); HIPCHK(sml_launch_theta_pack(ctx->d, theta, pk_cur(ctx), st)); ctx->prof.end(st);
+    if ((rc = pack_pk(ctx, theta, st))) return rc;
     SmlFwdArgs a;
     memset(&a, 0, sizeof(a));
     SmlSeg& s = a.seg[0];
@@ -747,13 +789,9 @@
     const int lstride = (wg_tiles(batch, 1) + wg_tiles(2 * batch, 1)) * (d / 16);
     const int64_t out_pstride = (int64_t)SML_R * (tiles_of(batch) + tiles_of(2 * batch)) * d;
     const int fns = fwd_split(wg_tiles(batch, 1) + wg_tiles(2 * batch, 1)), bsplit = bwd_split(wg_tiles(batch, 1) + wg_tiles(2 * batch, 1));
-    HIPCHK(ctx->loss_part.ensure((size_t)nb * lstride));
-    ctx->prof.begin(PC_PACK, st); HIPCHK(sml_launch_theta_pack(d, theta, pk_cur(ctx), st)); ctx->prof.end(st);
+    if ((rc = pack_pk(ctx, theta, st))) return rc;
     const bool mf_bx3 = fns == 1 && sml_bx3_bytes(d) > 0 && env_int("SML_MF_BX3", 1) != 0;
-    if (mf_bx3) {
-        HIPCHK(ctx->pkx.ensure(sml_bx3_bytes(d) / sizeof(float) + 4));
-        ctx->prof.begin(PC_PACK, st); HIPCHK(sml_launch_theta_pack_bx3(d, theta, ctx->pkx.p, st)); ctx->prof.end(st);
-    }
+    if (mf_bx3 && (rc = pack_pkx(ctx, theta, st))) return rc;
     const bool can_fuse = !xchg && !bsplit && d <= 64 && ctx->adaptive_beta <= 0.0f && env_int("SML_MF_FUSED_UPDATE", 1) != 0;
     const bool want_dense = can_fuse && fns == 1 && env_int("SML_MF_DISTINCT", 1) != 0;
     ctx->prof.begin(PC_SORT, st); rc = sort_epoch(&ctx->ix[0], triples, n, batch, 1, t->n_user, t->n_item, false, st, plan, nullptr, want_dense);
@@ -783,7 +821,8 @@
         HIPCHK(sml_launch_mark_runs(8, xchg->key_items, xchg->val_items, x_total, 32, ctx->rec_x.p, nullptr, nullptr, 0, 0, st));
     }
     ctx->prof.end(st); if (rc) return rc;
-    HIPCHK(hipMemsetAsync(ctx->loss_part.p, 0, (size_t)nb * lstride * sizeof(float), st));
+    const bool zfold = !xchg && hk_on("SML_HK_ZERO_FOLD");
+    if ((rc = loss_part_begin(ctx, (size_t)nb * lstride, zfold, st))) return rc;
     const int64_t ns = sml_net_size(d), ps = sml_pk_size(d);
     float* dx_buf = xchg ? xchg->dx_local : ctx->dx.p;
     const bool dense = want_dense && ctx->ix[0].by_hand && ctx->ix[0].dense;
@@ -917,7 +956,7 @@
         u.rep_x_stride = 3 * d; u.rep_x_off = d;
         ctx->prof.begin(PC_SEG_ADAM, st); HIPCHK(sml_launch_run_adam(d, u, (int64_t)u.n_u + u.n_i, st)); ctx->prof.end(st);
     }
-    ctx->prof.begin(PC_MISC, st); HIPCHK(sml_launch_loss_finalize(ctx->loss_part.p, (int)nb, lstride, nullptr, batch_loss, st)); ctx->prof.end(st);
+    if ((rc = loss_part_end(ctx, (int)nb, lstride, zfold, batch_loss, st))) return rc;
     *step += nb;
     return SML_OK;
 }
@@ -929,6 +968,14 @@
     hipStream_t st = (hipStream_t)stream;
     int rc;
     if ((rc = ensure_sched(ctx, lr, step + 1, st))) return rc;
+    if (hk_on("SML_HK_FLUSH_MERGE")) {
+        float* w[2] = {(float*)t->w_user, (float*)t->w_item}; float* m[2] = {t->m_user, t->m_item}; float* v[2] = {t->v_user, t->v_item};
+        int32_t* last[2] = {t->step_user, t->step_item}; const int64_t rows[2] = {t->n_user, t->n_item};
+        ctx->prof.begin(PC_FLUSH, st);
+        HIPCHK(sml_launch_adam_flush2(ctx->d, w, m, v, last, rows, ctx->sched.p, (int)step, replay_len(ctx, step), st));
+        ctx->prof.end(st);
+        return SML_OK;
+    }
     ctx->prof.begin(PC_FLUSH, st); HIPCHK(sml_launch_adam_flush(ctx->d, t->w_user, t->m_user, t->v_user, t->step_user, t->n_user, ctx->sched.p, (int)step, replay_len(ctx, step), st));
     HIPCHK(sml_launch_adam_flush(ctx->d, t->w_item, t->m_item, t->v_item, t->step_item, t->n_item, ctx->sched.p, (int)step, replay_len(ctx, step), st)); ctx->prof.end(st);
     return SML_OK;
@@ -963,12 +1010,13 @@
     const bool v2 = env_int("SML_TR_V2", 1) != 0;
     const int lstride = (wg_tiles(batch, 1) + wg_tiles(2 * batch, 1)) * (d / 16 > 4 ? d / 16 : 4);
     const int64_t out_pstride = (int64_t)SML_R * (tiles_of(batch) + tiles_of(2 * batch)) * d;
-    HIPCHK(ctx->loss_part.ensure((size_t)nb * lstride));
-    ctx->prof.begin(PC_PACK, st); HIPCHK(sml_launch_theta_pack(d, theta, pk_cur(ctx), st)); ctx->prof.end(st);
-    HIPCHK(hipMemsetAsync(ctx->loss_part.p, 0, (size_t)nb * lstride * sizeof(float), st));
-    HIPCHK(hipMemsetAsync(grad, 0, (size_t)2 * sml_net_size(d) * sizeof(float), st));
+    if ((rc = pack_pk(ctx, theta, st))) return rc;
+    ctx->theta_ver++;
     const int64_t ns = sml_net_size(d), ps = sml_pk_size(d);
     const bool fused_path = !clip && !grad_hook && ctx->peer.world <= 0 && ctx->comm == nullptr;
+    const bool zfold = fused_path && hk_on("SML_HK_ZERO_FOLD");
+    if ((rc = loss_part_begin(ctx, (size_t)nb * lstride, zfold, st))) return rc;
+    if (!(zfold && theta_grad == nullptr)) HIPCHK(hipMemsetAsync(grad, 0, (size_t)2 * sml_net_size(d) * sizeof(float), st));
     const bool defer = v2 && fns == 4 && fused_path && !plan && nb > 1 && env_int("SML_TR_DEFER", 1) != 0;
     const bool a2_recompute = v2 && env_int("SML_TR_A2_RECOMPUTE", 1) != 0;
     int prev_split = 0, prev_total = 0;
@@ -1077,7 +1125,7 @@
             HIPCHK(sml_launch_theta_adam(d, ad, st)); ctx->prof.end(st);
         }
     }
-    ctx->prof.begin(PC_MISC, st); HIPCHK(sml_launch_loss_finalize(ctx->loss_part.p, (int)nb, lstride, nullptr, batch_loss, st)); ctx->prof.end(st);
+    if ((rc = loss_part_end(ctx, (int)nb, lstride, zfold, batch_loss, st))) return rc;
     *step += nb;
     return SML_OK;
 }
@@ -1103,8 +1151,8 @@
     const int lstride = tiles * (d / 16 > 4 ? d / 16 : 4);
     const int64_t out_pstride = (int64_t)SML_R * (tiles_of(B) + tiles_of(2 * B)) * d;
     HIPCHK(ctx->loss_part.ensure((size_t)2 * lstride));
-    HIPCHK(hipMemsetAsync(ctx->loss_part.p, 0, (size_t)2 * lstride * sizeof(float), st));
-    HIPCHK(sml_launch_theta_pack(d, theta, pk_cur(ctx), st));
+    HIPCHK(hipMemsetAsync(ctx->loss_part.p, 0, (size_t)2 * lstride * sizeof(float), st)); ctx->loss_clean_p = nullptr;
+    if ((rc = pack_pk(ctx, theta, st, true))) return rc;
     SmlFwdArgs f;
     memset(&f, 0, sizeof(f));
     SmlBwdArgs w;
@@ -1230,7 +1278,7 @@
     } else if (X->n != n || X->batch != batch || X->triples != triples || X->world != (xchg ? xchg->world : 1)) {
         return fail(SML_ESTATE, "sml_embed_loss_sgd_epoch", "index set was prepared for other triples");
     }
-    HIPCHK(hipMemsetAsync(ctx->loss_part.p, 0, (size_t)nb * lstride * sizeof(float), st));
+    HIPCHK(hipMemsetAsync(ctx->loss_part.p, 0, (size_t)nb * lstride * sizeof(float), st)); ctx->loss_clean_p = nullptr;
     const int hot_cap = X->hot_cap;
     const bool known = hipEventQuery(X->ready) == hipSuccess;
     if ((rc = sort_order_check(X))) return rc;
@@ -1319,7 +1367,7 @@
     for (int q = 0; q < 8; ++q) inboxes[q] = q < W ? ctx->peer.inbox[q] : nullptr;
     HIPCHK(sml_launch_set_ptr_tab(ctx->ptr_tab.p, sh->item_shard, W, st));
     HIPCHK(sml_launch_set_ptr_tab(ctx->ptr_tab.p + 8, inboxes, W, st));
-    HIPCHK(hipMemsetAsync(ctx->loss_part.p, 0, (size_t)nb * lstride * sizeof(float), st));
+    HIPCHK(hipMemsetAsync(ctx->loss_part.p, 0, (size_t)nb * lstride * sizeof(float), st)); ctx->loss_clean_p = nullptr;
     IndexSet* A = &ctx->ix[0];
     IndexSet* Bs = &ctx->ix[1];
     for (int64_t b = 0; b < nb; ++b) {
@@ -1394,7 +1442,7 @@
     HIPCHK(ctx->loss_part.ensure((size_t)nb * lstride));
     ctx->prof.begin(PC_SORT, st); rc = sort_epoch(&ctx->ix[0], triples, n, batch, 0, t->n_user, t->n_item, false, st); ctx->prof.end(st);
     if (rc) return rc;
-    HIPCHK(hipMemsetAsync(ctx->loss_part.p, 0, (size_t)nb * lstride * sizeof(float), st));
+    HIPCHK(hipMemsetAsync(ctx->loss_part.p, 0, (size_t)nb * lstride * sizeof(float), st)); ctx->loss_clean_p = nullptr;
     for (int64_t b = 0; b < nb; ++b) {
         const int B = (int)((n - b * batch) < batch ? (n - b * batch) : batch);
         const int cur = (int)(*step + 1 + b);
@@ -2031,17 +2079,25 @@
     if (e != hipSuccess) return fail(SML_EHIP, "sml_stream_wait_stream", hipGetErrorString(e));
     return SML_OK;
 }
-int sml_copy_tables(int n, void* const* dst, const void* const* src, const int64_t* bytes, void* stream) {
-    if (n < 0 || n > 4 || (n && (!dst || !src || !bytes))) return fail(SML_EINVAL, "sml_copy_tables", "1..4 copies per call");
-    long long b[4] = {0, 0, 0, 0};
+static int copy_tables_impl(const char* what, int n, void* const* dst, const void* const* src, const int64_t* bytes, int32_t* flag, int value,
+                            void* stream) {
+    if (n < 0 || n > 8 || (n && (!dst || !src || !bytes))) return fail(SML_EINVAL, what, "0..8 copies per call");
+    long long b[8] = {0, 0, 0, 0, 0, 0, 0, 0};
     for (int q = 0; q < n; ++q) {
         if (bytes[q] == 0) continue;
         if (!dst[q] || !src[q] || bytes[q] < 0 || bytes[q] % 16 || ((uintptr_t)dst[q] | (uintptr_t)src[q]) % 16)
-            return fail(SML_EINVAL, "sml_copy_tables", "pointers and sizes must be multiples of 16 bytes");
+            return fail(SML_EINVAL, what, "pointers and sizes must be multiples of 16 bytes");
         b[q] = bytes[q];
     }
-    HIPCHK(sml_launch_copy_tables(n, dst, src, b, (hipStream_t)stream));
-    return SML_OK;
+    HIPCHK(sml_launch_copy_tables(n, dst, src, b, flag, value, (hipStream_t)stream));
+    return SML_OK;
+}
+int sml_copy_tables(int n, void* const* dst, const void* const* src, const int64_t* bytes, void* stream) {
+    return copy_tables_impl("sml_copy_tables", n, dst, src, bytes, nullptr, 0, stream);
+}
+int sml_copy_tables_signal(int n, void* const* dst, const void* const* src, const int64_t* bytes, int32_t* flag, int value, void* stream) {
+    if (!flag || value < 0) return fail(SML_EINVAL, "sml_copy_tables_signal", "bad argument");
+    return copy_tables_impl("sml_copy_tables_signal", n, dst, src, bytes, flag, value, stream);
 }
 int sml_debug_timeline(long long* buf) { return sml_debug_set_timeline(buf) == hipSuccess ? 0 : -1; }
 int sml_flag_set(int32_t* flag, int value, void* stream) {
diff --git a/sml_amd/csrc/mf_kernels.hip b/sml_amd/csrc/mf_kernels.hip
--- a/sml_amd/csrc/mf_kernels.hip
+++ b/sml_amd/csrc/mf_kernels.hip
@@ -144,12 +144,13 @@
     if (threadIdx.x == 0) { float s2 = 0.0f; for (int w = 0; w < 16; ++w) s2 += part[w]; *loss_slot += s2; }
 }
 
-__global__ __launch_bounds__(256) void k_loss_finalize(const float* __restrict__ part, int n_batches, int stride,
+template <bool ZERO>
+__global__ __launch_bounds__(256) void k_loss_finalize(std::conditional_t<ZERO, float*, const float* __restrict__> part, int n_batches, int stride,
                                                       float* __restrict__ out) {
     __shared__ float sh4[4];
     const int b = blockIdx.x;
     if (b >= n_batches) return;
-    const float* p = part + (int64_t)b * stride;
+    auto p = part + (int64_t)b * stride;
     float s = 0.0f;
     int i = threadIdx.x;
     for (; i + 7 * 256 < stride; i += 8 * 256) {
@@ -158,8 +159,12 @@
         for (int u = 0; u < 8; ++u) x[u] = p[i + u * 256];
 #pragma unroll
         for (int u = 0; u < 8; ++u) s += x[u];
-    }
-    for (; i < stride; i += 256) s += p[i];
+        if constexpr (ZERO) {
+#pragma unroll
+            for (int u = 0; u < 8; ++u) p[i + u * 256] = 0.0f;
+        }
+    }
+    for (; i < stride; i += 256) { s += p[i]; if constexpr (ZERO) p[i] = 0.0f; }
     const float tot = block_sum256(s, sh4);
     if (threadIdx.x == 0) out[b] = tot;
 }
@@ -666,19 +671,12 @@
 }
 
 template <int D>
-__global__ __launch_bounds__(256) void k_adam_flush(float* __restrict__ w, float* __restrict__ mt, float* __restrict__ vt,
-                                                    int32_t* __restrict__ last, int64_t rows,
-                                                    const SmlSched* __restrict__ sched, int cur_step, int sched_len) {
+__device__ __forceinline__ void adam_flush_rows(float* __restrict__ w, float* __restrict__ mt, float* __restrict__ vt,
+                                                int32_t* __restrict__ last, int64_t rows, const SmlSched* __restrict__ sched,
+                                                int cur_step, const SmlSched* swin, const SmlReplayEnt* tab, int64_t block, int64_t n_blocks) {
     constexpr int LPR = D / 4;
-    __shared__ SmlSched swin[SML_SW];
-    __shared__ SmlReplayEnt rtab[SML_RP_N];
-    sched_window_load(swin, sched, cur_step, threadIdx.x);
-    const bool closed = sched_len > 0;
-    if (closed) replay_table_build(rtab, sched, sched_len, cur_step, threadIdx.x);
-    __syncthreads();
-    const SmlReplayEnt* tab = closed ? rtab : nullptr;
     const int64_t total = rows * LPR;
-    for (int64_t gid = (int64_t)blockIdx.x * 256 + threadIdx.x; gid < total; gid += (int64_t)gridDim.x * 256) {
+    for (int64_t gid = block * 256 + threadIdx.x; gid < total; gid += n_blocks * 256) {
         const int64_t row = gid / LPR;
         const int sub = (int)(gid % LPR);
         const int from = last[row];
@@ -693,6 +691,33 @@
         RowVec<float>::store(vt + row * D + sub * 4, v);
         if (sub == 0) last[row] = cur_step;
     }
+}
+template <int D>
+__global__ __launch_bounds__(256) void k_adam_flush(float* __restrict__ w, float* __restrict__ mt, float* __restrict__ vt,
+                                                    int32_t* __restrict__ last, int64_t rows,
+                                                    const SmlSched* __restrict__ sched, int cur_step, int sched_len) {
+    __shared__ SmlSched swin[SML_SW];
+    __shared__ SmlReplayEnt rtab[SML_RP_N];
+    sched_window_load(swin, sched, cur_step, threadIdx.x);
+    const bool closed = sched_len > 0;
+    if (closed) replay_table_build(rtab, sched, sched_len, cur_step, threadIdx.x);
+    __syncthreads();
+    adam_flush_rows<D>(w, mt, vt, last, rows, sched, cur_step, swin, closed ? rtab : nullptr, blockIdx.x, gridDim.x);
+}
+struct SmlFlushTab { float* w; float* m; float* v; int32_t* last; long long rows; };
+template <int D>
+__global__ __launch_bounds__(256) void k_adam_flush2(SmlFlushTab t0, SmlFlushTab t1, int nb0, const SmlSched* __restrict__ sched,
+                                                     int cur_step, int sched_len) {
+    __shared__ SmlSched swin[SML_SW];
+    __shared__ SmlReplayEnt rtab[SML_RP_N];
+    sched_window_load(swin, sched, cur_step, threadIdx.x);
+    const bool closed = sched_len > 0;
+    if (closed) replay_table_build(rtab, sched, sched_len, cur_step, threadIdx.x);
+    __syncthreads();
+    const bool second = (int)blockIdx.x >= nb0;
+    const SmlFlushTab& t = second ? t1 : t0;
+    adam_flush_rows<D>(t.w, t.m, t.v, t.last, t.rows, sched, cur_step, swin, closed ? rtab : nullptr,
+                       second ? (int)blockIdx.x - nb0 : (int)blockIdx.x, second ? (int)gridDim.x - nb0 : nb0);
 }
 
 template <int D>
@@ -1201,7 +1226,11 @@
     return hipGetLastError();
 }
 hipError_t sml_launch_loss_finalize(const float* part, int n_batches, int stride, const int*, float* out, hipStream_t st) {
-    k_loss_finalize<<<dim3(n_batches), dim3(256), 0, st>>>(part, n_batches, stride, out);
+    k_loss_finalize<false><<<dim3(n_batches), dim3(256), 0, st>>>(part, n_batches, stride, out);
+    return hipGetLastError();
+}
+hipError_t sml_launch_loss_finalize_zero(float* part, int n_batches, int stride, float* out, hipStream_t st) {
+    k_loss_finalize<true><<<dim3(n_batches), dim3(256), 0, st>>>(part, n_batches, stride, out);
     return hipGetLastError();
 }
 hipError_t sml_launch_bare_grad(int d, int dtype_bytes, const SmlBareArgs& a, int* n_blocks, hipStream_t st) {
@@ -1290,6 +1319,20 @@
     SML_DISPATCH_D(d, k_adam_flush<DD><<<dim3((unsigned)nb), dim3(256), 0, st>>>(w, m, v, last, rows, sched, cur_step, sched_len));
     return hipGetLastError();
 }
+hipError_t sml_launch_adam_flush2(int d, float* const* w, float* const* m, float* const* v, int32_t* const* last, const int64_t* rows,
+                                  const SmlSched* sched, int cur_step, int sched_len, hipStream_t st) {
+    const int lpr = d / 4;
+    int64_t nb[2];
+    SmlFlushTab t[2];
+    for (int q = 0; q < 2; ++q) {
+        nb[q] = (rows[q] * lpr + 255) / 256;
+        if (sched_len > 0 && nb[q] > 2048) nb[q] = 2048;
+        t[q].w = w[q]; t[q].m = m[q]; t[q].v = v[q]; t[q].last = last[q]; t[q].rows = rows[q];
+    }
+    if (nb[0] + nb[1] == 0) return hipSuccess;
+    SML_DISPATCH_D(d, k_adam_flush2<DD><<<dim3((unsigned)(nb[0] + nb[1])), dim3(256), 0, st>>>(t[0], t[1], (int)nb[0], sched, cur_step, sched_len));
+    return hipGetLastError();
+}
 hipError_t sml_launch_mf_forward(int d, const float* wu, const float* wi, const int64_t* user, const int64_t* item,
                                  int64_t n, int norm, float* uemb, float* iemb, float* score, hipStream_t st) {
     const int lpr = d / 4;
@@ -1308,30 +1351,45 @@
     k_eval_bucketize<<<dim3((unsigned)((n + 3) / 4)), dim3(256), 0, st>>>(rows, n, n_cols, n_item, rows_out, bucket_off);
     return hipGetLastError();
 }
-struct SmlCopyJobs { f32x4* dst[4]; const f32x4* src[4]; long long n16[4]; int n_jobs; };
+struct SmlCopyJobs { f32x4* dst[8]; const f32x4* src[8]; long long n16[8]; int n_jobs; int* flag; int value; };
+template <bool SIGNAL>
 __global__ __launch_bounds__(256) void k_copy_tables(SmlCopyJobs j) {
     const long long stride = (long long)gridDim.x * 256;
     for (int q = 0; q < j.n_jobs; ++q) {
-        f32x4* __restrict__ d = j.dst[q];
-        const f32x4* __restrict__ s = j.src[q];
-        for (long long i = (long long)blockIdx.x * 256 + threadIdx.x; i < j.n16[q]; i += stride)
-            __builtin_nontemporal_store(__builtin_nontemporal_load(s + i), d + i);
-    }
-}
-hipError_t sml_launch_copy_tables(int n_jobs, void* const* dst, const void* const* src, const long long* bytes, hipStream_t st) {
+        f32x4* d = j.dst[q];
+        const f32x4* s = j.src[q];
+        for (long long i = (long long)blockIdx.x * 256 + threadIdx.x; i < j.n16[q]; i += stride) {
+            if constexpr (SIGNAL) peer_store16(reinterpret_cast<float*>(d + i), __builtin_nontemporal_load(s + i));
+            else __builtin_nontemporal_store(__builtin_nontemporal_load(s + i), d + i);
+        }
+    }
+    if constexpr (SIGNAL) {
+        asm volatile("s_waitcnt vmcnt(0)" ::: "memory");
+        __syncthreads();
+        if (threadIdx.x == 0 &&
+            __hip_atomic_fetch_add(j.flag + 2, 1, __ATOMIC_RELAXED, __HIP_MEMORY_SCOPE_AGENT) == (int)gridDim.x - 1) {
+            __hip_atomic_store(j.flag + 2, 0, __ATOMIC_RELAXED, __HIP_MEMORY_SCOPE_AGENT);
+            __hip_atomic_store(j.flag, j.value, __ATOMIC_RELAXED, __HIP_MEMORY_SCOPE_SYSTEM);
+        }
+    }
+}
+hipError_t sml_launch_copy_tables(int n_jobs, void* const* dst, const void* const* src, const long long* bytes, int* flag, int value,
+                                  hipStream_t st) {
     SmlCopyJobs j;
     long long most = 0;
-    j.n_jobs = n_jobs;
-    for (int q = 0; q < 4; ++q) {
+    j.n_jobs = n_jobs; j.flag = flag; j.value = value;
+    for (int q = 0; q < 8; ++q) {
         j.dst[q] = q < n_jobs ? reinterpret_cast<f32x4*>(dst[q]) : nullptr;
         j.src[q] = q < n_jobs ? reinterpret_cast<const f32x4*>(src[q]) : nullptr;
         j.n16[q] = q < n_jobs ? bytes[q] / 16 : 0;
         if (j.n16[q] > most) most = j.n16[q];
     }
-    if (most == 0) return hipSuccess;
+    if (most == 0 && !flag) return hipSuccess;
     long long nb = (most + 1023) / 1024;
     if (nb > 4096) nb = 4096;
-    k_copy_tables<<<dim3((unsigned)nb), dim3(256), 0, st>>>(j);
+    if (nb < 1) nb = 1;
+    if (flag) k_copy_tables<true><<<dim3((unsigned)nb), dim3(256), 0, st>>>(j);
+    else k_copy_tables<false><<<dim3((unsigned)nb), dim3(256), 0, st>>>(j);
     return hipGetLastError();
 }
 
diff --git a/sml_amd/csrc/sml_kernels.h b/sml_amd/csrc/sml_kernels.h
--- a/sml_amd/csrc/sml_kernels.h
+++ b/sml_amd/csrc/sml_kernels.h
@@ -160,6 +160,7 @@
 hipError_t sml_launch_adaptive_users(int d, const float* xin, float* dx, int B, float beta, float* loss_slot, hipStream_t st);
 hipError_t sml_launch_loss_finalize(const float* part, int n_batches, int stride, const int* counts,
                                     float* out, hipStream_t st);
+hipError_t sml_launch_loss_finalize_zero(float* part, int n_batches, int stride, float* out, hipStream_t st);
 
 
 struct SmlRunArgs {
@@ -246,6 +247,8 @@
 hipError_t sml_launch_run_sgd(int d, int dtype_bytes, const SmlRunArgs& a, int64_t max_records, hipStream_t st);
 hipError_t sml_launch_adam_flush(int d, float* w, float* m, float* v, int32_t* last, int64_t rows,
                                  const SmlSched* sched, int cur_step, int sched_len, hipStream_t st);
+hipError_t sml_launch_adam_flush2(int d, float* const* w, float* const* m, float* const* v, int32_t* const* last, const int64_t* rows,
+                                  const SmlSched* sched, int cur_step, int sched_len, hipStream_t st);
 hipError_t sml_launch_mark_runs(int key_bytes, const void* keys, const uint32_t* vals, int64_t n, int row_bits, SmlRun* rec,
                                 uint8_t* flag_dup, uint8_t* uniq, int64_t uniq_stride, int64_t uniq_item_base, hipStream_t st);
 hipError_t sml_launch_mark_unique(int key_bytes, const void* keys, const uint32_t* vals, int64_t n, int row_bits, uint8_t* uniq,
@@ -291,7 +294,8 @@
                                  int n_cols, int32_t* rank, hipStream_t st);
 hipError_t sml_launch_eval_bucketize(const int64_t* rows, int64_t n, int n_cols, int64_t n_item, int32_t* rows_out,
                                      int32_t* bucket_off, hipStream_t st);
-hipError_t sml_launch_copy_tables(int n_jobs, void* const* dst, const void* const* src, const long long* bytes, hipStream_t st);
+hipError_t sml_launch_copy_tables(int n_jobs, void* const* dst, const void* const* src, const long long* bytes, int* flag, int value,
+                                  hipStream_t st);
 hipError_t sml_debug_set_timeline(long long* buf);
 hipError_t sml_launch_flag_set(int* flag, int value, hipStream_t st);
 hipError_t sml_launch_flag_wait(int* flag, int value, long long timeout_ticks, hipStream_t st);
diff --git a/sml_amd/engine.py b/sml_amd/engine.py
--- a/sml_amd/engine.py
+++ b/sml_amd/engine.py
@@ -113,7 +113,30 @@
         if len(self._flat) >= 8:
             self._flat.pop(next(iter(self._flat)))
         self._flat[key] = (flat, views, transfer)
+        self.theta_written()
         return flat
+
+    def theta_written(self):
+        if getattr(self, "_theta_scoped", False):
+            check(self.lib.sml_ctx_theta_scope(self._ctx, 1), "sml_ctx_theta_scope")
+
+    def theta_scope(self, transfer):
+        import contextlib
+
+        @contextlib.contextmanager
+        def scope():
+            if self.dist is not None or getattr(self, "_theta_scoped", False):
+                yield
+                return
+            self._select(transfer)
+            check(self.lib.sml_ctx_theta_scope(self._ctx, 1), "sml_ctx_theta_scope")
+            self._theta_scoped = True
+            try:
+                yield
+            finally:
+                self._theta_scoped = False
+                check(self.lib.sml_ctx_theta_scope(self._ctx, 0), "sml_ctx_theta_scope")
+        return scope()
 
     def load_optimizer_state(self, mfbase=None, mf_state=None, transfer=None, tr_state=None):
         if mf_state is not None:
@@ -796,20 +819,33 @@
                 self._side = torch.cuda.Stream(device=self.device)
         return self._side
 
-    def copy_tables(self, pairs):
+    def copy_tables(self, pairs, signal=None):
         pairs = list(pairs)
-        for k in range(0, len(pairs), 4):
-            chunk = pairs[k:k + 4]
+        odd = [d.shape != s.shape or d.dtype != s.dtype or not (d.is_contiguous() and s.is_contiguous())
+               or (d.numel() * d.element_size()) % 16 or d.data_ptr() % 16 or s.data_ptr() % 16 or d.numel() == 0
+               for d, s in pairs]
+        if any(odd) and len({d.data_ptr() for d, _ in pairs if d.numel()} & {s.data_ptr() for _, s in pairs if s.numel()}):
+            for d, s in pairs:
+                d.copy_(s)
+            pairs, odd = [], []
+        for k in range(0, max(len(pairs), 1), 8):
+            chunk, codd = pairs[k:k + 8], odd[k:k + 8]
             n = len(chunk)
-            dst, src, nbytes = (ctypes.c_void_p * n)(), (ctypes.c_void_p * n)(), (ctypes.c_int64 * n)()
+            last = k + 8 >= len(pairs)
+            if n == 0 and not (last and signal is not None):
+                break
+            dst, src, nbytes = (ctypes.c_void_p * max(n, 1))(), (ctypes.c_void_p * max(n, 1))(), (ctypes.c_int64 * max(n, 1))()
             for q, (d, s) in enumerate(chunk):
-                if d.shape != s.shape or d.dtype != s.dtype or not (d.is_contiguous() and s.is_contiguous()) \
-                        or (d.numel() * d.element_size()) % 16 or d.data_ptr() % 16 or s.data_ptr() % 16 or d.numel() == 0:
+                if codd[q]:
                     d.copy_(s)
                     dst[q], src[q], nbytes[q] = None, None, 0
                     continue
                 dst[q], src[q], nbytes[q] = d.data_ptr(), s.data_ptr(), d.numel() * d.element_size()
-            check(self.lib.sml_copy_tables(n, dst, src, nbytes, self._stream()), "sml_copy_tables")
+            if last and signal is not None:
+                check(self.lib.sml_copy_tables_signal(n, dst, src, nbytes, _ptr(signal[0]), int(signal[1]), self._stream()),
+                      "sml_copy_tables_signal")
+            else:
+                check(self.lib.sml_copy_tables(n, dst, src, nbytes, self._stream()), "sml_copy_tables")
 
     def _snap_slot(self, cur):
         ring = self.__dict__.setdefault("_snap", [])
@@ -828,19 +864,27 @@
             slot[key] = torch.empty_like(like)
         return slot[key]
 
-    def _side_order(self, cur, side):
+    def _side_signal(self, force=False):
+        import os
+        if not force and (os.environ.get("SML_SIDE_SYNC", "flag") == "event" or os.environ.get("SML_HK_FLAG_TAIL", "0") != "1"):
+            return None
+        if getattr(self, "_sync_flag", None) is None:
+            self._sync_flag = torch.zeros(4, device=self.device, dtype=torch.int32)
+            self._sync_seq = 0
+            self._sync_seen = 0
+        self._sync_seq += 1
+        return (self._sync_flag, self._sync_seq)
+
+    def _side_order(self, cur, side, signal=None):
         mode = __import__("os").environ.get("SML_SIDE_SYNC", "flag")
         if mode == "event":
             check(self.lib.sml_stream_wait_stream(ctypes.c_void_p(side.cuda_stream), ctypes.c_void_p(cur.cuda_stream)),
                   "sml_stream_wait_stream")
             return
-        if getattr(self, "_sync_flag", None) is None:
-            self._sync_flag = torch.zeros(2, device=self.device, dtype=torch.int32)
-            self._sync_seq = 0
-            self._sync_seen = 0
-        self._sync_seq += 1
-        check(self.lib.sml_flag_set(_ptr(self._sync_flag), self._sync_seq, ctypes.c_void_p(cur.cuda_stream)), "sml_flag_set")
-        check(self.lib.sml_flag_wait(_ptr(self._sync_flag), self._sync_seq, self._flag_timeout(),
+        if signal is None:
+            signal = self._side_signal(force=True)
+            check(self.lib.sml_flag_set(_ptr(signal[0]), signal[1], ctypes.c_void_p(cur.cuda_stream)), "sml_flag_set")
+        check(self.lib.sml_flag_wait(_ptr(signal[0]), signal[1], self._flag_timeout(),
                                      ctypes.c_void_p(side.cuda_stream)), "sml_flag_wait")
 
     def eval_submit(self, user_tab, item_tab, rows):
@@ -850,8 +894,9 @@
         cur = torch.cuda.current_stream(self.device)
         slot = self._snap_slot(cur)
         su, si = self._snap_buf(slot, "u", wu), self._snap_buf(slot, "i", wi)
-        self.copy_tables([(su, wu), (si, wi)])
-        self._side_order(cur, side)
+        sig = self._side_signal()
+        self.copy_tables([(su, wu), (si, wi)], signal=sig)
+        self._side_order(cur, side, sig)
         with torch.cuda.stream(side):
             ranks = self.eval_ranks(su, si, rows, max_workgroups=self._side_eval_cap())
             ev = torch.cuda.Event()
@@ -888,14 +933,20 @@
         snaps = [self._snap_buf(slot, k, t) for k, t in zip(("lu", "hu", "li", "hi"), tabs)]
         su, si = self._snap_buf(slot, "u", tabs[0]), self._snap_buf(slot, "i", tabs[2])
         sth = self._snap_buf(slot, "theta", theta)
-        self.copy_tables(list(zip(snaps, tabs)))
-        sth.copy_(theta)
-        self._side_order(cur, side)
+        sig = self._side_signal()
+        if sig is not None:
+            self.copy_tables(list(zip(snaps, tabs)) + [(sth, theta)], signal=sig)
+        else:
+            self.copy_tables(list(zip(snaps, tabs)))
+            sth.copy_(theta)
+        self._side_order(cur, side, sig)
         ctx = self._side_ctx()
         with torch.cuda.stream(side):
+            check(self.lib.sml_ctx_theta_scope(ctx, 1), "sml_ctx_theta_scope")
             for net, (xt, xh, out) in enumerate(((snaps[0], snaps[1], su), (snaps[2], snaps[3], si))):
                 check(self.lib.sml_transfer_forward(ctx, _ptr(sth), net, _ptr(xt), _ptr(xh), _ptr(out), xt.shape[0],
                                                     self._stream()), "sml_transfer_forward")
+            check(self.lib.sml_ctx_theta_scope(ctx, 0), "sml_ctx_theta_scope")
             ranks = self.eval_ranks(su, si, rows, max_workgroups=self._side_eval_cap())
             ev = torch.cuda.Event()
             ev.record(side)
diff --git a/sml_amd/period.py b/sml_amd/period.py
--- a/sml_amd/period.py
+++ b/sml_amd/period.py
@@ -1,3 +1,6 @@
+import contextlib
+import os
+
 import numpy as np
 import torch
 
@@ -99,6 +102,12 @@
 
 
 def run_period(engine, st, plan, hp, record=None, overlap=True, exchanges=None):
+    scope = engine.theta_scope(st.transfer) if hasattr(engine, "theta_scope") else contextlib.nullcontext()
+    with scope:
+        return _run_period(engine, st, plan, hp, record, overlap, exchanges)
+
+
+def _run_period(engine, st, plan, hp, record, overlap, exchanges):
     mf, net = st.MFbase, st.transfer
     wu, wi = mf.user_laten.weight.data, mf.item_laten.weight.data
     state = {"version": 0, "cached": None}
@@ -158,8 +167,11 @@
             engine.mf_flush(mf)
             state["version"] += 1
             evaluate("MF epoch")
-        copy([(st.prev_hat_user, st.hat_user), (st.prev_hat_item, st.hat_item)])
-        copy([(st.hat_user, wu), (st.hat_item, wi)])
+        if hasattr(engine, "copy_tables") and os.environ.get("SML_HK_COPY_MERGE", "1") != "0":
+            copy([(st.prev_hat_user, st.hat_user), (st.prev_hat_item, st.hat_item), (st.hat_user, wu), (st.hat_item, wi)])
+        else:
+            copy([(st.prev_hat_user, st.hat_user), (st.prev_hat_item, st.hat_item)])
+            copy([(st.hat_user, wu), (st.hat_item, wi)])
         n_tr = len(plan.tr_triples[ph])
         if transferred_ok and n_tr > 0:
             evaluate_transferred("before TR")
```

Measured after the change: 16.05 million triples/s (median of 2 runs). Within noise of the previous version (+0.0%).
